# guy3540/Acoustic_Locating_VQ-VAE

Hardware: AMD Instinct MI355X
Metric: spectrograms/sec (train step), speech VQ-VAE default config (higher is better)
Workload: dtype x3mx_hb

## Files before the change

acoustic_locating_vq-vae_amd/csrc/alvq_common.h:

```cpp
#pragma once
#include <hip/hip_runtime.h>
#include <stdint.h>
#include <stdio.h>

#include "../../include/alvq.h"

namespace alvq {

void set_error(const char* fmt, ...);

enum Option { OPT_WIDE_MIN_TILES, OPT_FX_ROWS, OPT_FX_NARROW, OPT_CONV_V2, OPT_CONV_K3, OPT_WGRAD_V3, OPT_VQ_REG, OPT_COUNT };
long option(int id);

inline int check_launch(const char* what) {
  hipError_t e = hipGetLastError();
  if (e != hipSuccess) {
    set_error("%s: %s", what, hipGetErrorString(e));
    return (int)e;
  }
  return ALVQ_OK;
}

#define ALVQ_REQUIRE(cond, code, ...)  \
  do {                                 \
    if (!(cond)) {                     \
      alvq::set_error(__VA_ARGS__);    \
      return (code);                   \
    }                                  \
  } while (0)

struct DeviceOnce {
  bool done[64] = {};
  bool need() {
    int d = 0;
    if (hipGetDevice(&d) != hipSuccess || d < 0 || d >= 64) return true;
    if (done[d]) return false;
    done[d] = true;
    return true;
  }
};

constexpr int kWave = 64;
constexpr int kNumXcd = 8;

__device__ __forceinline__ int xcd_remap(int id, int n) {
  const int q = n / kNumXcd, r = n % kNumXcd;
  const int xcd = id % kNumXcd, local = id / kNumXcd;
  const int base = xcd < r ? xcd * (q + 1) : r * (q + 1) + (xcd - r) * q;
  return base + local;
}

typedef float f32x4 __attribute__((ext_vector_type(4)));
typedef float f32x16 __attribute__((ext_vector_type(16)));
typedef short bf16x8 __attribute__((ext_vector_type(8)));
typedef short bf16x4 __attribute__((ext_vector_type(4)));

int* fx_range_flag_ptr();
int* fx_range_sticky_ptr();

__device__ __forceinline__ float wave_sum(float v) {
#pragma unroll
  for (int o = 32; o > 0; o >>= 1) v += __shfl_xor(v, o, 64);
  return v;
}
// ... 9 lines not shown
```

acoustic_locating_vq-vae_amd/csrc/api.hip:

```cpp
#include <stdarg.h>
#include <stdlib.h>
#include <string.h>

#include <atomic>

#include "alvq_common.h"

namespace alvq {
static thread_local char g_err[512] = "";
void set_error(const char* fmt, ...) {
  va_list ap;
  va_start(ap, fmt);
  vsnprintf(g_err, sizeof(g_err), fmt, ap);
  va_end(ap);
}

struct OptionSpec { const char* name; const char* env; long def; };
static const OptionSpec kSpecs[OPT_COUNT] = {
    {"wide_min_tiles", "ALVQ_WIDE_MIN_TILES", 192},
    {"fx_rows", "ALVQ_FX_ROWS", 0},
    {"fx_narrow", "ALVQ_FX_NARROW", 1},
    {"conv_v2", "ALVQ_CONV_V2", 1},
    {"conv_k3", "ALVQ_CONV_K3", 1},
    {"wgrad_v3", "ALVQ_WGRAD_V3", 3},
    {"vq_reg", "ALVQ_VQ_REG", 1},
};
static std::atomic<long> g_opt[OPT_COUNT];
static std::atomic<int> g_opt_ready{0};
static void options_init() {
  if (g_opt_ready.load(std::memory_order_acquire)) return;
  for (int i = 0; i < OPT_COUNT; ++i) {
    const char* e = getenv(kSpecs[i].env);
    g_opt[i].store(e ? atol(e) : kSpecs[i].def, std::memory_order_relaxed);
  }
  g_opt_ready.store(1, std::memory_order_release);
}
long option(int id) {
  options_init();
  return g_opt[id].load(std::memory_order_relaxed);
}
}

extern "C" const char* alvq_version(void) { return "alvq 0.4.0 (gfx950)"; }
extern "C" const char* alvq_last_error(void) { return alvq::g_err; }

extern "C" int alvq_set_option(const char* name, int64_t value) {
  ALVQ_REQUIRE(name, ALVQ_EINVAL, "alvq_set_option: null name");
  alvq::options_init();
  for (int i = 0; i < alvq::OPT_COUNT; ++i)
    if (!strcmp(name, alvq::kSpecs[i].name)) {
      alvq::g_opt[i].store((long)value, std::memory_order_relaxed);
      return ALVQ_OK;
    }
  alvq::set_error("alvq_set_option: unknown option '%s'", name);
  return ALVQ_EINVAL;
}

extern "C" int64_t alvq_get_option(const char* name) {
  if (name) {
    alvq::options_init();
    for (int i = 0; i < alvq::OPT_COUNT; ++i)
      if (!strcmp(name, alvq::kSpecs[i].name)) return alvq::g_opt[i].load(std::memory_order_relaxed);
  }
  alvq::set_error("alvq_get_option: unknown option '%s'", name ? name : "(null)");
  return INT64_MIN;
}
```

acoustic_locating_vq-vae_amd/csrc/bf16_common.h:

```cpp
#pragma once
#include "alvq_common.h"

namespace alvq {

typedef __bf16 bf16;
typedef __bf16 bf16x8_t __attribute__((ext_vector_type(8)));
typedef unsigned short u16;
typedef unsigned short u16x8 __attribute__((ext_vector_type(8)));

constexpr int TB_R = 128;
constexpr int TB_M = 128;
constexpr int TB_K = 64;
constexpr int XROWS = TB_R + 8;
constexpr int XBYTES = XROWS * 128;
constexpr int WBYTES = TB_M * 128;
constexpr int CS = TB_M + 4;
constexpr int LDS_BYTES = 2 * XBYTES + 2 * WBYTES;
static_assert(LDS_BYTES >= TB_R * CS * 4, "C tile must fit");
constexpr int GUARD_ROWS = 8;

__device__ __forceinline__ float bf2f(u16 v) { return __uint_as_float(((unsigned)v) << 16); }
__device__ __forceinline__ u16 f2bf(float f) {
  unsigned u = __float_as_uint(f);
  if ((u & 0x7fffffffu) > 0x7f800000u) return (u16)((u >> 16) | 0x40);
  return (u16)((u + 0x7fffu + ((u >> 16) & 1u)) >> 16);
}

__device__ __forceinline__ void glds16(const void* gsrc, void* lds_dst) {
  __builtin_amdgcn_global_load_lds((const void __attribute__((address_space(1)))*)gsrc,
                                   (void __attribute__((address_space(3)))*)lds_dst, 16, 0, 0);
}

__device__ __forceinline__ bool row_valid(int row, int Lp1, int nrows_data, int* b, int* l) {
  const int v = row - 1;
  const int bb = v / Lp1, ll = v - bb * Lp1;
  *b = bb;
  *l = ll;
  return row >= 1 && v < nrows_data && ll < Lp1 - 1;
}

struct ConvBArgs {
  const u16* x;
  const u16* wp;
  const float* bias;
  const u16* skip1;
  const u16* skip2;
  const u16* mask;
  const u16* post;
  u16* y;
  u16* y2;
  float* y_ncl;
  int B, L, Cp, M, Mop, Mp128;
  int relu;
  int rtiles, mtiles;
  const unsigned char* mask_bits;
  unsigned char* bits_out;
  int elem;
  const float* out_scale;
  int* range_flag;
};

constexpr int WP_ROWS = 256;
constexpr int NLC_ROW_PAD = 256;

typedef __bf16 bf16x2_t __attribute__((ext_vector_type(2)));
typedef float f32x2 __attribute__((ext_vector_type(2)));
typedef unsigned u32x2 __attribute__((ext_vector_type(2)));
typedef unsigned u32x4 __attribute__((ext_vector_type(4)));

__device__ __forceinline__ unsigned f2bf_pk(float lo, float hi) {
  const f32x2 f = {lo, hi};
  return __builtin_bit_cast(unsigned, __builtin_convertvector(f, bf16x2_t));
}

typedef _Float16 h16x8_t __attribute__((ext_vector_type(8)));
typedef _Float16 h16x2_t __attribute__((ext_vector_type(2)));
template <int F16>
__device__ __forceinline__ float elem2f(u16 v) {
  if (F16) return (float)__builtin_bit_cast(_Float16, v);
  return bf2f(v);
}
template <int F16>
__device__ __forceinline__ unsigned elem_pk(float lo, float hi) {
  if (F16) {
    const f32x2 f = {lo, hi};
    return __builtin_bit_cast(unsigned, __builtin_convertvector(f, h16x2_t));
  }
  return f2bf_pk(lo, hi);
}
template <int F16>
__device__ __forceinline__ void elem_saturate() {
  if (F16) __builtin_amdgcn_s_setreg(1 | (23 << 6), 1);
}
template <int F16>
__device__ __forceinline__ f32x4 elem_mfma16(const bf16x8_t& a, const bf16x8_t& b, const f32x4& c) {
  if (F16) return __builtin_amdgcn_mfma_f32_16x16x32_f16(__builtin_bit_cast(h16x8_t, a), __builtin_bit_cast(h16x8_t, b), c, 0, 0, 0);
  return __builtin_amdgcn_mfma_f32_16x16x32_bf16(a, b, c, 0, 0, 0);
}

__device__ __forceinline__ void fp16_watch(unsigned& run, unsigned word) {
  const unsigned a = word & 0x7fff7fffu;
  asm("v_pk_max_u16 %0, %1, %2" : "=v"(run) : "v"(run), "v"(a));
}
__device__ __forceinline__ bool fp16_limit_reached(unsigned run) { return (run & 0xffffu) >= 0x7bffu || (run >> 16) >= 0x7bffu; }
__device__ __forceinline__ void fp16_report(unsigned run, int* flag) {
  if (flag && __any(fp16_limit_reached(run)) && (threadIdx.x & 63) == 0) atomicOr(flag, 4);
}

int conv1d_bf16_v2_launch(const ConvBArgs& a, int KW, hipStream_t stream);
int conv1d_bf16_k3_launch(const ConvBArgs& a, hipStream_t stream);
int64_t conv1d_wgrad_bf16_v2_workspace_bytes(int total_rows, int C, int M, int KW);
int conv1d_wgrad_bf16_v2_splits(int total_rows, int C, int M, int KW, int nseg, bool with_bias);
// ... 8 lines not shown
```

acoustic_locating_vq-vae_amd/csrc/conv1d_bf16.hip:

```cpp
#include <stdlib.h>

#include "alvq_common.h"
#include "bf16_common.h"
#include "conv1d_bf16_tile256.h"
#include "nlc_host.h"

namespace alvq {

template <int KW, int OUT, int F16 = 0>
__global__ __launch_bounds__(256, 2) void conv1d_bf16_kernel(ConvBArgs a) {
  constexpr int PAD = (KW - 1) / 2;
  extern __shared__ __attribute__((aligned(16))) unsigned char lds[];
  unsigned char* const Xb = lds;
  unsigned char* const Wb = lds + 2 * XBYTES;

  const int tid = threadIdx.x, lane = tid & 63;
  const int wave = __builtin_amdgcn_readfirstlane(tid >> 6);
  const int li = lane & 15, kq = lane >> 4;
  const int wm0 = (wave >> 1) * 64, wn0 = (wave & 1) * 64;

  const int tile = xcd_remap(blockIdx.x, a.mtiles * a.rtiles);
  const int m0 = (tile % a.mtiles) * TB_M;
  const int r0 = (tile / a.mtiles) * TB_R;
  const int Cp = a.Cp;
// ... 174 lines not shown
}

extern "C" int alvq_pack_weight_bf16(const float* w, void* wp, int M, int C, int KW, int w_layout, void* stream) {
  const alvq_pack_desc d{w, wp, M, C, KW, w_layout};
  return alvq_pack_weights_bf16_batch(&d, 1, 1, stream);
}

template <int F16>
static int ncl_to_nlc_16bit(const char* who, const float* x, void* y, int B, int C, int L, const float* scale, void* stream) {
  if (int rc = check_nlc_dims(who, x && y, B, C, L)) return rc;
  const NlcDims d(B, C, L);
  hipLaunchKernelGGL(ncl_to_nlc_kernel<F16>, d.grid32(), dim3(256), 0, (hipStream_t)stream, x, (u16*)y, B, C, L, d.Cp, d.rows, scale);
  return check_launch(who);
}
template <int F16>
static int nlc_to_ncl_16bit(const char* who, const void* x, float* y, int B, int C, int L, const float* scale, void* stream) {
  if (int rc = check_nlc_dims(who, x && y, B, C, L)) return rc;
  const NlcDims d(B, C, L);
  hipLaunchKernelGGL(nlc_to_ncl_kernel<F16>, d.grid32(), dim3(256), 0, (hipStream_t)stream, (const u16*)x, y, B, C, L, d.Cp, d.rows,
                     scale);
  return check_launch(who);
}

extern "C" int alvq_ncl_to_nlc_bf16(const float* x, void* y, int B, int C, int L, void* stream) {
  return ncl_to_nlc_16bit<0>("alvq_ncl_to_nlc_bf16", x, y, B, C, L, nullptr, stream);
}

extern "C" int alvq_nlc_to_ncl_f32(const void* x, float* y, int B, int C, int L, void* stream) {
  return nlc_to_ncl_16bit<0>("alvq_nlc_to_ncl_f32", x, y, B, C, L, nullptr, stream);
}

extern "C" int alvq_relu_mask_bf16(const void* dy, const void* t, void* out, int64_t n, void* stream) {
  ALVQ_REQUIRE(dy && t && out, ALVQ_EINVAL, "alvq_relu_mask_bf16: null pointer");
  ALVQ_REQUIRE(n > 0 && n % 8 == 0, ALVQ_EINVAL, "alvq_relu_mask_bf16: n must be a positive multiple of 8");
  long g = (n / 8 + 1023) / 1024;
  if (g > 2048) g = 2048;
  hipLaunchKernelGGL(relu_mask_bf16_kernel, dim3((int)g), dim3(256), 0, (hipStream_t)stream, (const u16*)dy, (const u16*)t,
                     (u16*)out, (long)(n / 8));
  return check_launch("alvq_relu_mask_bf16");
}

static constexpr int b16_slot(int KW, int OUT, int F16) { return ((KW == 3) * 2 + OUT) * 2 + F16; }
typedef KernelTable<void (*)(ConvBArgs), 8> B16Table;
static B16Table b16_table() {
  B16Table t;
  for_values<1, 3>([&](auto kw) { for_values<0, 1>([&](auto out) { for_values<0, 1>([&](auto f16) {
    t.put(b16_slot(kw, out, f16), conv1d_bf16_kernel<kw, out, f16>, LDS_BYTES);
  }); }); });
  return t;
}

static int conv1d_16bit(int elem, const float* out_scale, const void* x, const void* wp, const float* bias, const void* skip1,
                        const void* skip2, const void* mask, const void* post, void* y, void* y2, float* y_ncl, int B, int C, int M,
                        int L, int KW, int relu, const void* mask_bits, void* relu_bits_out, void* stream) {
  const char* const who = elem ? "alvq_conv1d_f16" : "alvq_conv1d_bf16";
  if (int rc = check_conv_args(who, x, wp, skip1, skip2, mask, post, y, y2, y_ncl, B, C, M, L, KW, relu, mask_bits, relu_bits_out))
    return rc;
  ConvBArgs a{(const u16*)x, (const u16*)wp, bias, (const u16*)skip1, (const u16*)skip2, (const u16*)mask, (const u16*)post,
              (u16*)y, (u16*)y2, y_ncl, B, L, pad_to(C, TB_K), M, pad_to(M, TB_K), pad_to(M, WP_ROWS), relu,
              (int)(alvq_nlc_rows(B, L) / TB_R), pad_to(M, TB_M) / TB_M, (const unsigned char*)mask_bits,
              (unsigned char*)relu_bits_out};
  hipStream_t s = (hipStream_t)stream;
  a.relu = relu ? 1 : 0;
  a.elem = elem;
  a.out_scale = out_scale;
  a.range_flag = elem ? fx_range_flag_ptr() : nullptr;
  const long use_v2 = option(OPT_CONV_V2), use_k3 = option(OPT_CONV_K3);
  const long tiles256 = (alvq_nlc_rows(B, L) / 256) * (pad_to(M, 256) / 256);
  const long min_tiles = option(OPT_WIDE_MIN_TILES);
  if (use_v2 && pad_to(M, 256) - M <= 32 && tiles256 >= min_tiles)
    return (KW == 3 && use_k3) ? conv1d_bf16_k3_launch(a, s) : conv1d_bf16_v2_launch(a, KW, s);
  static const B16Table table = b16_table();
  static DeviceOnce attr;
  if (attr.need()) table.raise_lds_limit();
  return table.launch(b16_slot(KW, y ? 0 : 1, elem ? 1 : 0), dim3(a.rtiles * a.mtiles), dim3(256), s, who, a);
}

extern "C" int alvq_conv1d_bf16(const void* x, const void* wp, const float* bias, const void* skip1, const void* skip2,
                                const void* mask, const void* post, void* y, void* y2, float* y_ncl, int B, int C, int M,
                                int L, int KW, int relu, const void* mask_bits, void* relu_bits_out, void* stream) {
  return conv1d_16bit(0, nullptr, x, wp, bias, skip1, skip2, mask, post, y, y2, y_ncl, B, C, M, L, KW, relu, mask_bits, relu_bits_out,
                      stream);
}

extern "C" int alvq_conv1d_f16(const void* x, const void* wp, const float* bias, const void* skip1, const void* skip2,
                               const void* mask, const void* post, void* y, void* y2, float* y_ncl, int B, int C, int M, int L,
                               int KW, int relu, const void* mask_bits, void* relu_bits_out, const float* out_scale, void* stream) {
  return conv1d_16bit(1, out_scale, x, wp, bias, skip1, skip2, mask, post, y, y2, y_ncl, B, C, M, L, KW, relu, mask_bits,
                      relu_bits_out, stream);
}

extern "C" int alvq_ncl_to_nlc_f16(const float* x, void* y, int B, int C, int L, const float* scale, void* stream) {
  return ncl_to_nlc_16bit<1>("alvq_ncl_to_nlc_f16", x, y, B, C, L, scale, stream);
}

extern "C" int alvq_nlc_to_ncl_f16(const void* x, float* y, int B, int C, int L, const float* scale, void* stream) {
  return nlc_to_ncl_16bit<1>("alvq_nlc_to_ncl_f16", x, y, B, C, L, scale, stream);
}

static int64_t wgrad_bias_offset(int rows, int C, int M, int KW) { return conv1d_wgrad_bf16_v2_workspace_bytes(rows, C, M, KW); }

extern "C" int64_t alvq_conv1d_wgrad_bf16_workspace_bytes(int B, int C, int M, int L, int KW) {
  if (!wgrad_shape_ok(B, C, M, L, KW)) return -1;
  return wgrad_bias_offset((int)alvq_nlc_rows(B, L), C, M, KW) + (int64_t)64 * pad_to(M, TB_K) * 4;
}

extern "C" int64_t alvq_conv1d_wgrad_bf16_bias_offset(int B, int C, int M, int L, int KW) {
  if (!wgrad_shape_ok(B, C, M, L, KW)) return -1;
  return wgrad_bias_offset((int)alvq_nlc_rows(B, L), C, M, KW);
}

extern "C" int alvq_conv1d_wgrad_bf16_splits(int B, int C, int M, int L, int KW, int nseg, int with_bias) {
  if (!wgrad_shape_ok(B, C, M, L, KW) || nseg < 1 || nseg > WGRAD_MAXSEG) return -1;
  return conv1d_wgrad_bf16_v2_splits((int)alvq_nlc_rows(B, L), C, M, KW, nseg, with_bias != 0);
}

static int wgrad_16bit(const char* who, int elem, const void* const* dy, const void* const* x, int nseg, bool multi, float* dw,
                       float* dbias, void* workspace, int B, int C, int M, int L, int KW, int w_layout, int accumulate,
                       const float* inv_scale, void* stream) {
  if (int rc = check_wgrad_args(who, dy, x, nseg, multi, dw, workspace, B, C, M, L, KW, w_layout, accumulate, true)) return rc;
  const int rows = (int)alvq_nlc_rows(B, L);
  float* const bias_partial = multi ? nullptr : (float*)((char*)workspace + wgrad_bias_offset(rows, C, M, KW));
  return conv1d_wgrad_bf16_v2_launch(dy, x, nseg, dw, workspace, rows, C, M, KW, w_layout, accumulate, (hipStream_t)stream, dbias,
                                     bias_partial, elem, inv_scale);
}

extern "C" int alvq_conv1d_wgrad_bf16(const void* dy, const void* x, float* dw, float* dbias, void* workspace, int B, int C,
                                      int M, int L, int KW, int w_layout, int accumulate, void* stream) {
  return wgrad_16bit("alvq_conv1d_wgrad_bf16", 0, &dy, &x, 1, false, dw, dbias, workspace, B, C, M, L, KW, w_layout, accumulate,
                     nullptr, stream);
}

extern "C" int alvq_conv1d_wgrad_f16(const void* dy, const void* x, float* dw, float* dbias, void* workspace, int B, int C, int M,
                                     int L, int KW, int w_layout, int accumulate, const float* inv_scale, void* stream) {
  return wgrad_16bit("alvq_conv1d_wgrad_f16", 1, &dy, &x, 1, false, dw, dbias, workspace, B, C, M, L, KW, w_layout, accumulate,
                     inv_scale, stream);
}

extern "C" int alvq_conv1d_wgrad_f16_multi(const void* const* dy, const void* const* x, int nseg, float* dw, void* workspace, int B,
                                           int C, int M, int L, int KW, int w_layout, int accumulate, const float* inv_scale,
                                           void* stream) {
  return wgrad_16bit("alvq_conv1d_wgrad_f16_multi", 1, dy, x, nseg, true, dw, nullptr, workspace, B, C, M, L, KW, w_layout,
// ... 9 lines not shown
```

acoustic_locating_vq-vae_amd/csrc/conv1d_bf16_tile256.h:

```cpp
#pragma once
#include "bf16_common.h"

namespace alvq {

constexpr int V2_M = 256, V2_R = 256, V2_K = 32;
constexpr int V2_HALF = V2_M * V2_K * 2;
constexpr int V2_CS = V2_M + 4;
constexpr int V2_EPI_LDS = 64 * V2_CS * 4;

struct FragSet {
  bf16x8_t a[8];
  bf16x8_t b[4];
};

template <int NMI, int NNI, int F16 = 0>
__device__ __forceinline__ void wave_epilogue_bf16(const ConvBArgs& a, const f32x4 (&acc)[NMI][NNI], int m0, int r0, int li,
                                                   int kq, int wm0, int wn0);

template <int OUT, int F16 = 0>
__device__ __forceinline__ void tile256_epilogue(const ConvBArgs& a, const f32x4 (&acc)[8][4], unsigned char* lds, int m0,
                                                 int r0, int wave, int tid, int li, int kq, int wm0) {
  if (OUT == 0) {
    wave_epilogue_bf16<8, 4, F16>(a, acc, m0, r0, li, kq, wm0, (wave & 3) * 64);
    return;
// ... 57 lines not shown
      float v[8];
#pragma unroll
      for (int e = 0; e < 4; ++e) {
        const u32x2 r = __builtin_amdgcn_permlane16_swap(__float_as_uint(acc[mp][ni][e]), __float_as_uint(acc[mp + 1][ni][e]),
                                                         false, false);
        v[e] = __uint_as_float(r[0]);
        v[e + 4] = __uint_as_float(r[1]);
      }
      if (a.bias) {
        if (m0 + wm0 + mp * 16 + 32 <= a.M) {
          const f32x4 b0 = *(const f32x4*)(a.bias + mb), b1 = *(const f32x4*)(a.bias + mb + 4);
#pragma unroll
          for (int e = 0; e < 4; ++e) {
            v[e] += b0[e];
            v[4 + e] += b1[e];
          }
        } else {
#pragma unroll
          for (int e = 0; e < 8; ++e) v[e] += (mb + e < a.M) ? a.bias[mb + e] : 0.f;
        }
      }
      if (a.skip1) {
#pragma unroll
        for (int e = 0; e < 8; ++e) v[e] += elem2f<F16>(s1[mp / 2][e]);
      }
      if (a.skip2) {
#pragma unroll
        for (int e = 0; e < 8; ++e) v[e] += elem2f<F16>(s2[mp / 2][e]);
      }
      if (a.relu & 1) {
#pragma unroll
        for (int e = 0; e < 8; ++e) v[e] = fmaxf(v[e], 0.f);
      }
      if (a.mask_bits) {
        const int bt = (int)a.mask_bits[o >> 3];
#pragma unroll
        for (int e = 0; e < 8; ++e) v[e] = __uint_as_float(__float_as_uint(v[e]) & (unsigned)((bt << (31 - e)) >> 31));
      } else if (a.mask) {
#pragma unroll
        for (int e = 0; e < 8; ++e) v[e] = (short)mk[mp / 2][e] > 0 ? v[e] : 0.f;
      }
      u32x4 out;
#pragma unroll
      for (int e = 0; e < 4; ++e) out[e] = elem_pk<F16>(v[2 * e], v[2 * e + 1]);
      if (gaps) {
#pragma unroll
        for (int e = 0; e < 4; ++e) out[e] = ok ? out[e] : 0u;
      }
      *(u32x4*)(a.y + o) = out;
      if (F16) {
#pragma unroll
        for (int e = 0; e < 4; ++e) fp16_watch(watch, out[e]);
      }
      if (a.y2) {
        const u16x8 ps = *(const u16x8*)(a.post + o);
        u32x4 out2;
#pragma unroll
        for (int e = 0; e < 4; ++e) out2[e] = elem_pk<F16>(v[2 * e] + elem2f<F16>(ps[2 * e]), v[2 * e + 1] + elem2f<F16>(ps[2 * e + 1]));
        if (gaps) {
#pragma unroll
          for (int e = 0; e < 4; ++e) out2[e] = ok ? out2[e] : 0u;
        }
        *(u32x4*)(a.y2 + o) = out2;
      }
      if (a.bits_out) {
        unsigned bt = 0;
#pragma unroll
        for (int e = 7; e >= 0; --e) {
          const int half = (int)((e & 1) ? (out[e >> 1] & 0xffff0000u) : (out[e >> 1] << 16));
          const int t = half > 0 ? half : 0;
          bt = __builtin_amdgcn_alignbit(bt, 0u - (unsigned)t, 31);
        }
        a.bits_out[o >> 3] = (unsigned char)bt;
      }
    }
  }
  if (F16) fp16_report(watch, a.range_flag);
}

}
```

acoustic_locating_vq-vae_amd/csrc/conv1d_wgrad_bf16_v2.hip:

```cpp
#include <stdlib.h>

#include "alvq_common.h"
#include "bf16_common.h"
#include "nlc_host.h"
#include "wgrad_reduce.h"

namespace alvq {

typedef short s16x4_t __attribute__((ext_vector_type(4)));
typedef short s16x8_t __attribute__((ext_vector_type(8)));

constexpr int WG_MAXSEG = 4;
struct WgradV2Args {
  const u16* dy[WG_MAXSEG];
  const u16* x[WG_MAXSEG];
  float* partial;
  float* bias_partial;
  int Mp, Cp, M, C;
  int mtiles, ctiles, splits, chunks_per_split, total_rows, nseg;
};

typedef unsigned long long u64;
template <int ROW_BYTES>
__device__ __forceinline__ void tr_pair_issue(unsigned lds_addr, u64& lo, u64& hi) {
// ... 397 lines not shown
#undef V3_TILE
#undef V3_TILE_K3
#undef V3_TILE_K1
#undef V3_SB
#undef V3_MM
#undef V3_RD_B
#undef V3_RD_A
#undef V3_TR16

  const int jc = lane & 31;
  float* out = a.partial + (long)split * KW * a.M * a.C;
#pragma unroll
  for (int t = 0; t < KW; ++t)
#pragma unroll
    for (int mi = 0; mi < MF; ++mi)
#pragma unroll
      for (int cf = 0; cf < NC; ++cf)
#pragma unroll
        for (int q = 0; q < 16; ++q) {
          const int m = m0 + wm0 + mi * 32 + (q & 3) + 8 * (q >> 2) + 4 * g;
          const int c = c0 + wc0 + cf * 32 + jc;
          if (m < a.M && c < a.C) out[((long)t * a.M + m) * a.C + c] = acc[t][mi][cf][q];
        }
}

template <int KW, int NC, int MF>
static constexpr int wgrad_v3_lds() {
  return 4 * (32 * (2 * MF * 32 * 2) + (KW == 1 ? 32 : 36) * (4 * NC * 32 * 2));
}

static __global__ __launch_bounds__(256) void wgrad_bias_reduce_kernel(const float* bp, float* dbias, int splits, int Mp, int M,
                                                                       int accumulate, const float* scale) {
  const int m = blockIdx.x * 256 + threadIdx.x;
  if (m >= M) return;
  float s = 0.f;
  for (int k = 0; k < splits; ++k) s += bp[(long)k * Mp + m];
  if (scale) s *= *scale;
  dbias[m] = accumulate ? dbias[m] + s : s;
}

template <int KW, int NCF>
static constexpr int wgrad_v2_lds() {
  return 4 * (32 * 256 + (KW == 1 ? 32 : 36) * (4 * NCF * 16 * 2));
}

static int wgrad_v3_select() { return (int)option(OPT_WGRAD_V3); }
static bool wgrad_uses_v3(int KW, bool with_bias) {
  return !with_bias && ((KW == 1 && (wgrad_v3_select() & 1)) || (KW == 3 && (wgrad_v3_select() & 2)));
}
static int wgrad_v2_tiles(int C, int M, int KW, bool v3) {
  return WgradTile{(v3 && KW == 1) ? 256 : 128, KW == 3 ? 128 : 256}.count(C, M);
}

static constexpr int wg_slot(int v3, int KW, int F16) { return (v3 * 2 + (KW == 3)) * 2 + F16; }
typedef KernelTable<void (*)(WgradV2Args), 8> WgTable;
static WgTable wg_table() {
  WgTable t;
  for_values<1, 3>([&](auto kw) { for_values<0, 1>([&](auto f16) {
    constexpr int NCF = kw == 3 ? 2 : 4, NC = kw == 3 ? 1 : 2, MF = kw == 3 ? 2 : 4;
    t.put(wg_slot(0, kw, f16), conv1d_wgrad_bf16_v2_kernel<kw, NCF, f16>, wgrad_v2_lds<kw, NCF>());
    t.put(wg_slot(1, kw, f16), conv1d_wgrad_bf16_v3_kernel<kw, NC, MF, f16>, wgrad_v3_lds<kw, NC, MF>());
  }); });
  return t;
}

int conv1d_wgrad_bf16_v2_splits(int total_rows, int C, int M, int KW, int nseg, bool with_bias) {
  int cps;
  return wgrad_split_plan(nseg * total_rows, wgrad_v2_tiles(C, M, KW, wgrad_uses_v3(KW, with_bias)), &cps);
}

int64_t conv1d_wgrad_bf16_v2_workspace_bytes(int total_rows, int C, int M, int KW) {
  const int s2 = wgrad_split_bound(total_rows, wgrad_v2_tiles(C, M, KW, false), WG_MAXSEG);
  const int s3 = wgrad_split_bound(total_rows, wgrad_v2_tiles(C, M, KW, true), WG_MAXSEG);
  return (int64_t)(s2 > s3 ? s2 : s3) * KW * M * C * 4;
}

int conv1d_wgrad_bf16_v2_launch(const void* const* dy, const void* const* x, int nseg, float* dw, void* workspace,
                                int total_rows, int C, int M, int KW, int w_layout, int accumulate, hipStream_t s,
                                float* dbias, float* bias_partial, int elem, const float* out_scale) {
  const int ct = KW == 3 ? 128 : 256;
  const int Mp = pad_to(M, 64), Cp = pad_to(C, 64);
  WgradV2Args a{};
  for (int i = 0; i < WG_MAXSEG; ++i) {
    a.dy[i] = (const u16*)dy[i < nseg ? i : 0];
    a.x[i] = (const u16*)x[i < nseg ? i : 0];
  }
  a.partial = (float*)workspace;
  a.bias_partial = dbias ? bias_partial : nullptr;
  a.Mp = Mp; a.Cp = Cp; a.M = M; a.C = C;
  a.mtiles = (M + 127) / 128; a.ctiles = (C + ct - 1) / ct;
  a.total_rows = total_rows; a.nseg = nseg;
  const bool v3 = wgrad_uses_v3(KW, dbias != nullptr);
  if (v3 && KW == 1) a.mtiles = (M + 255) / 256;
  a.splits = wgrad_split_plan(nseg * total_rows, a.mtiles * a.ctiles, &a.chunks_per_split);
  ALVQ_REQUIRE(a.mtiles * a.ctiles == wgrad_v2_tiles(C, M, KW, v3) &&
                   (int64_t)a.splits * KW * M * C * 4 <= conv1d_wgrad_bf16_v2_workspace_bytes(total_rows, C, M, KW),
               ALVQ_EINVAL, "alvq_conv1d_wgrad_bf16: %d splits exceed what alvq_conv1d_wgrad_bf16_workspace_bytes sizes", a.splits);
  static const WgTable table = wg_table();
  static DeviceOnce attr;
  if (attr.need()) table.raise_lds_limit();
  if (int rc = table.launch(wg_slot(v3, KW, elem ? 1 : 0), dim3(a.mtiles * a.ctiles * a.splits), dim3(512), s, "alvq_conv1d_wgrad_bf16(v2)", a))
    return rc;
  if (accumulate == ALVQ_WGRAD_DEFER) return ALVQ_OK;
  wgrad_reduce_launch((const float*)workspace, dw, a.splits, KW, M, C, w_layout, accumulate, s, out_scale);
  if (dbias)
    hipLaunchKernelGGL(wgrad_bias_reduce_kernel, dim3((M + 255) / 256), dim3(256), 0, s, (const float*)bias_partial, dbias,
                       a.splits, Mp, M, accumulate, out_scale);
  return check_launch("alvq_conv1d_wgrad_bf16(v2)/reduce");
}

}
```

acoustic_locating_vq-vae_amd/csrc/nlc_host.h:

```cpp
#pragma once
#include <type_traits>

#include "bf16_common.h"

namespace alvq {

inline int pad_to(int x, int q) { return (x + q - 1) / q * q; }
inline long nlc_plane_elems(int B, int L, int C) {
  return ((long)alvq_nlc_rows(B, L) + 2L * alvq_nlc_guard_rows()) * pad_to(C, TB_K);
}
struct NlcDims {
  int rows, Cp;
  long plane;
  NlcDims(int B, int C, int L) : rows((int)alvq_nlc_rows(B, L)), Cp(pad_to(C, TB_K)), plane(nlc_plane_elems(B, L, C)) {}
  dim3 grid32() const { return dim3((rows / 32) * (Cp / 32)); }
};

inline int check_nlc_dims(const char* who, bool pointers, int B, int C, int L) {
  ALVQ_REQUIRE(pointers, ALVQ_EINVAL, "%s: null pointer", who);
  ALVQ_REQUIRE(B > 0 && C > 0 && L > 0, ALVQ_EINVAL, "%s: bad dims", who);
  return ALVQ_OK;
}

inline int check_conv_args(const char* who, const void* x, const void* wp, const void* skip1, const void* skip2, const void* mask,
                           const void* post, const void* y, const void* y2, const void* y_ncl, int B, int C, int M, int L, int KW,
                           int relu, const void* mask_bits, const void* bits_out, const char* ncl_also = "") {
  ALVQ_REQUIRE(x && wp && (y || y_ncl), ALVQ_EINVAL, "%s: null x/wp/y", who);
  ALVQ_REQUIRE(!(y && y_ncl), ALVQ_EINVAL, "%s: choose one of y (NLC) and y_ncl (NCL fp32)", who);
  ALVQ_REQUIRE(B > 0 && C > 0 && M > 0 && L > 0, ALVQ_EINVAL, "%s: bad dims", who);
  ALVQ_REQUIRE(KW == 1 || KW == 3, ALVQ_EUNSUPPORTED, "%s: KW=%d (only 1 and 3)", who, KW);
  ALVQ_REQUIRE((y2 == nullptr) == (post == nullptr), ALVQ_EINVAL, "%s: y2 and post go together", who);
  ALVQ_REQUIRE(!y_ncl || (!skip1 && !skip2 && !mask && !post && !relu), ALVQ_EUNSUPPORTED,
               "%s: the NCL fp32 epilogue fuses bias%s only", who, ncl_also);
  ALVQ_REQUIRE((long)B * (L + 1) < (1L << 30), ALVQ_EUNSUPPORTED, "%s: problem too large", who);
  ALVQ_REQUIRE(!(mask && mask_bits), ALVQ_EINVAL, "%s: pass the mask as a tensor or as bits, not both", who);
  ALVQ_REQUIRE(!y_ncl || (!mask_bits && !bits_out), ALVQ_EUNSUPPORTED, "%s: sign bits go with the NLC output", who);
  return ALVQ_OK;
}

constexpr int WGRAD_MAXSEG = 4;

inline int check_wgrad_args(const char* who, const void* const* dy, const void* const* x, int nseg, bool multi, const void* dw,
                            const void* workspace, int B, int C, int M, int L, int KW, int w_layout, int accumulate,
                            bool dw_may_be_null) {
  ALVQ_REQUIRE(dy && x && (multi || (dy[0] && x[0])) && (dw || (dw_may_be_null && accumulate == ALVQ_WGRAD_DEFER)) && workspace,
               ALVQ_EINVAL, "%s: null pointer", who);
  if (multi) {
    ALVQ_REQUIRE(nseg >= 1 && nseg <= WGRAD_MAXSEG, ALVQ_EUNSUPPORTED, "%s: nseg=%d (1..4)", who, nseg);
    for (int i = 0; i < nseg; ++i) ALVQ_REQUIRE(dy[i] && x[i], ALVQ_EINVAL, "%s: null segment %d", who, i);
  }
  ALVQ_REQUIRE(B > 0 && C > 0 && M > 0 && L > 0, ALVQ_EINVAL, "%s: bad dims", who);
  ALVQ_REQUIRE(KW == 1 || KW == 3, ALVQ_EUNSUPPORTED, "%s: KW=%d (only 1 and 3)", who, KW);
  ALVQ_REQUIRE(w_layout == ALVQ_W_OIK || w_layout == ALVQ_W_IOK, ALVQ_EINVAL, "%s: w_layout", who);
  return ALVQ_OK;
}

template <int... V, class F>
inline void for_values(F f) {
  (f(std::integral_constant<int, V>{}), ...);
}

template <class Fn, int N>
struct KernelTable {
  Fn fn[N] = {};
  int lds[N] = {};
  void put(int slot, Fn f, int lds_bytes) {
    fn[slot] = f;
    lds[slot] = lds_bytes;
  }
  void raise_lds_limit() const {
    for (int i = 0; i < N; ++i)
      if (fn[i]) (void)hipFuncSetAttribute((const void*)fn[i], hipFuncAttributeMaxDynamicSharedMemorySize, lds[i]);
  }
  template <class... A>
  int launch(int slot, dim3 grid, dim3 block, hipStream_t s, const char* what, const A&... args) const {
    ALVQ_REQUIRE(slot >= 0 && slot < N && fn[slot], ALVQ_EUNSUPPORTED, "%s: no kernel is instantiated for this case (slot %d)", what,
                 slot);
    hipLaunchKernelGGL(fn[slot], grid, block, lds[slot], s, args...);
    return check_launch(what);
  }
};

inline int wgrad_split_plan(int total_rows, int tiles, int* chunks_per_split) {
  const int nchunks = total_rows / 64;
  int want = (256 + tiles - 1) / tiles;
  if (want < 1) want = 1;
  if (want > nchunks) want = nchunks;
  if (want > 64) want = 64;
  const int cps = (nchunks + want - 1) / want;
// ... 56 lines not shown
```

acoustic_locating_vq-vae_amd/csrc/pack_weights.hip:

```cpp
#include "alvq_common.h"
#include "bf16_common.h"
#include "f16mx_common.h"
#include "nlc_host.h"

namespace alvq {

constexpr int PB_MAX = 32;
struct PackDesc {
  const float* w;
  u16* wp;
  int M, C, KW, layout, Mp, Cp, blk0, ctiles;
};
struct PackBatch {
  PackDesc d[PB_MAX];
  int n;
  long plane[PB_MAX];
};

template <int PLANES>
__device__ __forceinline__ void pack_store8(u16* wp, long plane, long row_off, int c, const float (&v)[8]) {
  const long o = row_off + c;
  if (PLANES == 3) {
    unsigned h[4], qh[2], ql[2];
    fx_split<8>(v, fx_pow2(FX_E_W), fx_pow2(FX_E_W - FX_LO_SHIFT), h, qh, ql);
// ... 12 lines not shown
#pragma unroll
    for (int e = 0; e < 4; ++e) {
      const float h0 = __uint_as_float(hi[e] << 16), h1 = __uint_as_float(hi[e] & 0xffff0000u);
      lo[e] = f2bf_pk(v[2 * e] - h0, v[2 * e + 1] - h1);
    }
    *(u32x4*)(wp + plane + o) = lo;
  }
}

template <int PLANES>
__global__ __launch_bounds__(256) void pack_weights_batch_kernel(PackBatch b) {
  __shared__ float tile[3][32][65];
  if (PLANES == 3) fx_saturating_conversions();
  int di = 0;
  for (int i = 1; i < b.n; ++i)
    if ((int)blockIdx.x >= b.d[i].blk0) di = i;
  const PackDesc& d = b.d[di];
  const int lb = blockIdx.x - d.blk0;
  const int m0 = (lb / d.ctiles) * 32, c0 = (lb % d.ctiles) * 64;
  const int KW = d.KW, tid = threadIdx.x;
  if (d.layout == ALVQ_W_OIK) {
    const int run = 64 * KW;
#pragma unroll 4
    for (int e = tid; e < 32 * run; e += 256) {
      const int mr = e / run, j = e - mr * run, c = j / KW, t = j - c * KW;
      const int m = m0 + mr;
      tile[t][mr][c] = (m < d.M && c0 + c < d.C) ? d.w[((long)m * d.C + c0) * KW + j] : 0.f;
    }
  } else {
    const int run = 32 * KW;
#pragma unroll 4
    for (int e = tid; e < 64 * run; e += 256) {
      const int cc = e / run, j = e - cc * run, mr = j / KW, k = j - mr * KW;
      const int c = c0 + cc;
      tile[KW - 1 - k][mr][cc] = (c < d.C && m0 + mr < d.M) ? d.w[((long)c * d.M + m0) * KW + j] : 0.f;
    }
  }
  __syncthreads();
  const int mr = tid >> 3, cg = (tid & 7) * 8;
  for (int t = 0; t < KW; ++t) {
    float v[8];
#pragma unroll
    for (int e = 0; e < 8; ++e) v[e] = tile[t][mr][cg + e];
    pack_store8<PLANES>(d.wp, b.plane[di], ((long)t * d.Mp + m0 + mr) * d.Cp, c0 + cg, v);
  }
}

constexpr int AP_MAX = 24;
struct AdamPackDesc {
  float* w; const float* g; float* m; float* v;
  u16* oik; u16* iok;
  int dim0, dim1, KW, blk0, tiles1;
  int oik_Mp, oik_Cp, iok_Mp, iok_Cp;
};
struct AdamPackBatch {
  AdamPackDesc d[AP_MAX];
  int n;
  const float* sc;
  const float* skip;
  float beta1, beta2, eps;
};

template <int PLANES>
__global__ __launch_bounds__(256) void adam_pack_batch_kernel(AdamPackBatch b) {
  __shared__ float tile[3][32][65];
  if (b.skip && *b.skip != 0.f) return;
  if (PLANES == 3) fx_saturating_conversions();
  int di = 0;
  for (int i = 1; i < b.n; ++i)
    if ((int)blockIdx.x >= b.d[i].blk0) di = i;
  const AdamPackDesc& d = b.d[di];
  const int lb = blockIdx.x - d.blk0;
  const int r0 = (lb / d.tiles1) * 32, q0 = (lb % d.tiles1) * 64;
  const int KW = d.KW, tid = threadIdx.x;
  const float lr_bc1 = b.sc[0], bc2_sqrt = b.sc[1], gscale = b.sc[2];
  const float beta1 = b.beta1, beta2 = b.beta2, eps = b.eps;
  const int run = 64 * KW;
  if (q0 + 64 <= d.dim1 && ((d.dim1 * KW) & 3) == 0) {
#pragma unroll 2
    for (int e4 = tid; e4 < 8 * run; e4 += 256) {
      const int e = 4 * e4, rr = e / run, j = e - rr * run;
      f32x4 wn = {0.f, 0.f, 0.f, 0.f};
      if (r0 + rr < d.dim0) {
        const long i = ((long)(r0 + rr) * d.dim1 + q0) * KW + j;
        const f32x4 g4 = *(const f32x4*)(d.g + i), m4 = *(const f32x4*)(d.m + i), v4 = *(const f32x4*)(d.v + i), w4 = *(const f32x4*)(d.w + i);
        f32x4 mo, vo;
#pragma unroll
        for (int q = 0; q < 4; ++q) {
          const float gr = g4[q] * gscale;
          const float mm = m4[q] + (gr - m4[q]) * (1.f - beta1);
          const float vv = v4[q] * beta2 + (1.f - beta2) * gr * gr;
          const float denom = sqrtf(vv) / bc2_sqrt + eps;
          mo[q] = mm;
          vo[q] = vv;
          wn[q] = w4[q] - lr_bc1 * (mm / denom);
        }
        *(f32x4*)(d.m + i) = mo;
        *(f32x4*)(d.v + i) = vo;
        *(f32x4*)(d.w + i) = wn;
      }
#pragma unroll
      for (int q = 0; q < 4; ++q) {
        const int jj = j + q, qq = jj / KW, t = jj - qq * KW;
        tile[t][rr][qq] = wn[q];
      }
    }
  } else {
#pragma unroll 2
    for (int e = tid; e < 32 * run; e += 256) {
      const int rr = e / run, j = e - rr * run, qq = j / KW, t = j - qq * KW;
      float wn = 0.f;
      if (r0 + rr < d.dim0 && q0 + qq < d.dim1) {
        const long i = ((long)(r0 + rr) * d.dim1 + q0) * KW + j;
        const float gr = d.g[i] * gscale;
        const float m0 = d.m[i], v0 = d.v[i];
        const float mm = m0 + (gr - m0) * (1.f - beta1);
        const float vv = v0 * beta2 + (1.f - beta2) * gr * gr;
        const float denom = sqrtf(vv) / bc2_sqrt + eps;
        d.m[i] = mm;
        d.v[i] = vv;
        wn = d.w[i] - lr_bc1 * (mm / denom);
        d.w[i] = wn;
      }
      tile[t][rr][qq] = wn;
    }
  }
  __syncthreads();
  if (d.oik) {
    const int mr = tid >> 3, cg = (tid & 7) * 8;
    const long plane = (long)KW * d.oik_Mp * d.oik_Cp;
    for (int t = 0; t < KW; ++t) {
// ... 47 lines not shown

using namespace alvq;

extern "C" int alvq_pack_weights_bf16_batch(const alvq_pack_desc* descs, int n, int planes, void* stream) {
  ALVQ_REQUIRE(descs && n > 0, ALVQ_EINVAL, "alvq_pack_weights_bf16_batch: no descriptors");
  ALVQ_REQUIRE(planes >= 1 && planes <= 3, ALVQ_EINVAL, "alvq_pack_weights_bf16_batch: planes=%d (1, 2 or 3)", planes);
  for (int i = 0; i < n; ++i) {
    const alvq_pack_desc& s = descs[i];
    ALVQ_REQUIRE(s.w && s.wp, ALVQ_EINVAL, "alvq_pack_weights_bf16_batch: null pointer in descriptor %d", i);
    ALVQ_REQUIRE(s.M > 0 && s.C > 0 && (s.KW == 1 || s.KW == 3), ALVQ_EINVAL, "alvq_pack_weights_bf16_batch: bad dims in descriptor %d", i);
    ALVQ_REQUIRE(s.w_layout == ALVQ_W_OIK || s.w_layout == ALVQ_W_IOK, ALVQ_EINVAL, "alvq_pack_weights_bf16_batch: w_layout in descriptor %d", i);
  }
  for (int i0 = 0; i0 < n; i0 += PB_MAX) {
    PackBatch b{};
    b.n = n - i0 < PB_MAX ? n - i0 : PB_MAX;
    int blocks = 0;
    for (int i = 0; i < b.n; ++i) {
      const alvq_pack_desc& s = descs[i0 + i];
      PackDesc& d = b.d[i];
      d.w = s.w; d.wp = (u16*)s.wp; d.M = s.M; d.C = s.C; d.KW = s.KW; d.layout = s.w_layout;
      d.Mp = pad_to(s.M, WP_ROWS); d.Cp = pad_to(s.C, TB_K);
      d.blk0 = blocks; d.ctiles = d.Cp / 64;
      b.plane[i] = (long)s.KW * d.Mp * d.Cp;
      blocks += (d.Mp / 32) * d.ctiles;
    }
    if (planes == 1) hipLaunchKernelGGL(pack_weights_batch_kernel<1>, dim3(blocks), dim3(256), 0, (hipStream_t)stream, b);
    else if (planes == 2) hipLaunchKernelGGL(pack_weights_batch_kernel<2>, dim3(blocks), dim3(256), 0, (hipStream_t)stream, b);
    else hipLaunchKernelGGL(pack_weights_batch_kernel<3>, dim3(blocks), dim3(256), 0, (hipStream_t)stream, b);
    int rc = check_launch("alvq_pack_weights_bf16_batch");
    if (rc) return rc;
  }
  return ALVQ_OK;
}

extern "C" int alvq_adam_pack_batch(const alvq_adam_pack_desc* descs, int n, int planes, const float* scalars, float beta1,
                                    float beta2, float eps, const float* skip, void* stream) {
  ALVQ_REQUIRE(descs && n > 0 && scalars, ALVQ_EINVAL, "alvq_adam_pack_batch: no descriptors / scalars");
  ALVQ_REQUIRE(planes >= 1 && planes <= 3, ALVQ_EINVAL, "alvq_adam_pack_batch: planes=%d (1, 2 or 3)", planes);
  for (int i = 0; i < n; ++i) {
    const alvq_adam_pack_desc& s = descs[i];
    ALVQ_REQUIRE(s.w && s.g && s.m && s.v, ALVQ_EINVAL, "alvq_adam_pack_batch: null pointer in descriptor %d", i);
    ALVQ_REQUIRE(s.dim0 > 0 && s.dim1 > 0 && (s.KW == 1 || s.KW == 3), ALVQ_EINVAL, "alvq_adam_pack_batch: bad dims in descriptor %d", i);
  }
  for (int i0 = 0; i0 < n; i0 += AP_MAX) {
    AdamPackBatch b{};
    b.n = n - i0 < AP_MAX ? n - i0 : AP_MAX;
    b.sc = scalars; b.skip = skip; b.beta1 = beta1; b.beta2 = beta2; b.eps = eps;
    int blocks = 0;
    for (int i = 0; i < b.n; ++i) {
      const alvq_adam_pack_desc& s = descs[i0 + i];
      AdamPackDesc& d = b.d[i];
      d.w = s.w; d.g = s.g; d.m = s.m; d.v = s.v; d.oik = (u16*)s.wp_oik; d.iok = (u16*)s.wp_iok;
      d.dim0 = s.dim0; d.dim1 = s.dim1; d.KW = s.KW;
      d.oik_Mp = pad_to(s.dim0, WP_ROWS); d.oik_Cp = pad_to(s.dim1, TB_K);
      d.iok_Mp = pad_to(s.dim1, WP_ROWS); d.iok_Cp = pad_to(s.dim0, TB_K);
      d.blk0 = blocks; d.tiles1 = (s.dim1 + 63) / 64;
      blocks += ((s.dim0 + 31) / 32) * d.tiles1;
    }
    if (planes == 1) hipLaunchKernelGGL(adam_pack_batch_kernel<1>, dim3(blocks), dim3(256), 0, (hipStream_t)stream, b);
    else if (planes == 2) hipLaunchKernelGGL(adam_pack_batch_kernel<2>, dim3(blocks), dim3(256), 0, (hipStream_t)stream, b);
    else hipLaunchKernelGGL(adam_pack_batch_kernel<3>, dim3(blocks), dim3(256), 0, (hipStream_t)stream, b);
    int rc = check_launch("alvq_adam_pack_batch");
    if (rc) return rc;
  }
  return ALVQ_OK;
}

extern "C" int alvq_adam_segments_f32(float* param, const float* grad, float* exp_avg, float* exp_avg_sq, const int64_t* lo,
                                      const int64_t* hi, int nseg, const float* scalars, float beta1, float beta2, float eps,
                                      const float* skip, void* stream) {
  ALVQ_REQUIRE(param && grad && exp_avg && exp_avg_sq && scalars && lo && hi, ALVQ_EINVAL, "alvq_adam_segments_f32: null pointer");
  ALVQ_REQUIRE(nseg > 0, ALVQ_EINVAL, "alvq_adam_segments_f32: no segments");
  for (int i0 = 0; i0 < nseg; i0 += AS_MAX) {
    AdamSegs s{};
    s.n = nseg - i0 < AS_MAX ? nseg - i0 : AS_MAX;
    int blocks = 0;
    for (int i = 0; i < s.n; ++i) {
      ALVQ_REQUIRE(lo[i0 + i] >= 0 && hi[i0 + i] > lo[i0 + i], ALVQ_EINVAL, "alvq_adam_segments_f32: bad segment %d", i0 + i);
      s.lo[i] = lo[i0 + i]; s.hi[i] = hi[i0 + i];
      s.blk0[i] = blocks;
      blocks += (int)((hi[i0 + i] - lo[i0 + i] + 1023) / 1024);
    }
    hipLaunchKernelGGL(adam_segments_kernel, dim3(blocks), dim3(256), 0, (hipStream_t)stream, param, grad, exp_avg, exp_avg_sq, s, scalars,
                       beta1, beta2, eps, skip);
    int rc = check_launch("alvq_adam_segments_f32");
    if (rc) return rc;
  }
  return ALVQ_OK;
}
```

acoustic_locating_vq-vae_amd/csrc/wgrad_reduce.h:

```cpp
#pragma once
#include "alvq_common.h"

namespace alvq {

static __device__ __forceinline__ void wgrad_reduce_body(const float* partial, float* dw, int splits, int KW, int M, int C,
                                                         int w_layout, int accumulate, const float* scale, long stride, int bid,
                                                         int nblk) {
  const long total = (long)KW * M * C;
  const float sc = scale ? *scale : 1.f;
  if (w_layout == ALVQ_W_OIK && KW == 3) {
    const long pairs = (long)M * C;
    for (long q = bid * 256L + threadIdx.x; q < pairs; q += (long)nblk * 256) {
      float s0 = 0.f, s1 = 0.f, s2 = 0.f;
      const float* p = partial + q;
      int k = 0;
      for (; k + 2 <= splits; k += 2) {
        const float* pa = p + (long)k * stride;
        const float* pb = pa + stride;
        const float a0 = pa[0], a1 = pa[pairs], a2 = pa[2 * pairs], b0 = pb[0], b1 = pb[pairs], b2 = pb[2 * pairs];
        s0 = (s0 + a0) + b0;
        s1 = (s1 + a1) + b1;
        s2 = (s2 + a2) + b2;
      }
      for (; k < splits; ++k) {
        const float* pa = p + (long)k * stride;
        s0 += pa[0];
        s1 += pa[pairs];
        s2 += pa[2 * pairs];
      }
      if (scale) { s0 *= sc; s1 *= sc; s2 *= sc; }
      float* o = dw + 3 * q;
      if (accumulate) { s0 += o[0]; s1 += o[1]; s2 += o[2]; }
      o[0] = s0; o[1] = s1; o[2] = s2;
    }
    return;
  }
  for (long e = bid * 256L + threadIdx.x; e < total; e += (long)nblk * 256) {
    int m, c, t;
    if (w_layout == ALVQ_W_OIK) {
      t = (int)(e % KW);
      c = (int)((e / KW) % C);
      m = (int)(e / ((long)KW * C));
    } else {
      const int tt = (int)(e % KW);
      t = KW - 1 - tt;
      m = (int)((e / KW) % M);
      c = (int)(e / ((long)KW * M));
    }
    const long src = ((long)t * M + m) * C + c;
    float s = 0.f;
    int k = 0;
    for (; k + 4 <= splits; k += 4) {
      const float v0 = partial[(long)k * stride + src], v1 = partial[(long)(k + 1) * stride + src],
                  v2 = partial[(long)(k + 2) * stride + src], v3 = partial[(long)(k + 3) * stride + src];
      s = (((s + v0) + v1) + v2) + v3;
    }
    for (; k < splits; ++k) s += partial[(long)k * stride + src];
    if (scale) s *= sc;
    dw[e] = accumulate ? dw[e] + s : s;
  }
}
static __global__ void wgrad_reduce_kernel(const float* partial, float* dw, int splits, int KW, int M, int C, int w_layout,
                                    int accumulate, const float* scale) {
  wgrad_reduce_body(partial, dw, splits, KW, M, C, w_layout, accumulate, scale, (long)KW * M * C, blockIdx.x, gridDim.x);
}

template <int RB>
static __device__ __forceinline__ void wgrad_reduce_iok_body(float (&tile)[3][RB][65], const float* partial, float* dw, int splits,
                                                             int KW, int M, int C, int accumulate, const float* scale, int bid) {
  constexpr int RI = RB / 8;
  const int ctiles = (C + 63) / 64;
  const int m0 = (bid / ctiles) * RB, c0 = (bid % ctiles) * 64;
  const int tx = threadIdx.x & 31, ty = threadIdx.x >> 5;
  const long plane = (long)M * C, total = (long)KW * plane;
  const bool pair = (C % 2 == 0);
  float s0[3][RI], s1[3][RI];
#pragma unroll
  for (int t = 0; t < 3; ++t)
#pragma unroll
    for (int i = 0; i < RI; ++i) s0[t][i] = s1[t][i] = 0.f;
  const int c = c0 + 2 * tx;
  const bool full = pair && m0 + RB <= M && c0 + 64 <= C;
  if (full) {
    const float* p0 = partial + (long)(m0 + ty) * C + c;
    if (KW == 3) {
#pragma unroll 4
      for (int k = 0; k < splits; ++k) {
        float2 v[3][RI];
#pragma unroll
        for (int t = 0; t < 3; ++t)
#pragma unroll
          for (int i = 0; i < RI; ++i) v[t][i] = *(const float2*)(p0 + (long)k * total + (long)t * plane + (long)(8 * i) * C);
#pragma unroll
        for (int t = 0; t < 3; ++t)
#pragma unroll
          for (int i = 0; i < RI; ++i) {
            s0[t][i] += v[t][i].x;
            s1[t][i] += v[t][i].y;
          }
      }
    } else {
#pragma unroll 4
      for (int k = 0; k < splits; ++k) {
        float2 v[RI];
#pragma unroll
        for (int i = 0; i < RI; ++i) v[i] = *(const float2*)(p0 + (long)k * total + (long)(8 * i) * C);
#pragma unroll
        for (int i = 0; i < RI; ++i) {
          s0[0][i] += v[i].x;
          s1[0][i] += v[i].y;
        }
      }
    }
  } else
  for (int k = 0; k < splits; ++k) {
    const float* pk = partial + (long)k * total + c;
#pragma unroll
    for (int t = 0; t < 3; ++t) {
      if (t >= KW) break;
#pragma unroll
      for (int i = 0; i < RI; ++i) {
        const int m = m0 + ty + 8 * i;
        if (m >= M) continue;
        const float* p = pk + (long)t * plane + (long)m * C;
        if (pair && c + 1 < C) {
          const float2 v = *(const float2*)p;
          s0[t][i] += v.x;
          s1[t][i] += v.y;
        } else {
          if (c < C) s0[t][i] += p[0];
          if (c + 1 < C) s1[t][i] += p[1];
        }
      }
    }
  }
#pragma unroll
  for (int t = 0; t < 3; ++t) {
    if (t >= KW) break;
#pragma unroll
    for (int i = 0; i < RI; ++i) {
      tile[t][ty + 8 * i][2 * tx] = s0[t][i];
      tile[t][ty + 8 * i][2 * tx + 1] = s1[t][i];
    }
  }
  __syncthreads();
  const int run = RB * KW;
  for (int e = threadIdx.x; e < 64 * run; e += 256) {
    const int cc = e / run, j = e - cc * run, mr = j / KW, tt = j - mr * KW;
    if (c0 + cc >= C || m0 + mr >= M) continue;
    const long o = ((long)(c0 + cc) * M + m0) * KW + j;
    float v = tile[KW - 1 - tt][mr][cc];
    if (scale) v *= *scale;
    dw[o] = accumulate ? dw[o] + v : v;
  }
}
template <int RB>
static __global__ __launch_bounds__(256) void wgrad_reduce_iok_kernel(const float* partial, float* dw, int splits, int KW,
                                                                      int M, int C, int accumulate, const float* scale) {
  __shared__ float tile[3][RB][65];
  wgrad_reduce_iok_body<RB>(tile, partial, dw, splits, KW, M, C, accumulate, scale, blockIdx.x);
}

static inline void wgrad_reduce_launch(const float* partial, float* dw, int splits, int KW, int M, int C, int w_layout,
                                       int accumulate, hipStream_t s, const float* scale = nullptr) {
  if (w_layout == ALVQ_W_IOK) {
    const int grid = ((M + 15) / 16) * ((C + 63) / 64);
    hipLaunchKernelGGL(wgrad_reduce_iok_kernel<16>, dim3(grid), dim3(256), 0, s, partial, dw, splits, KW, M, C, accumulate, scale);
    return;
  }
  const long total = (long)KW * M * C;
  int rgrid = (int)((total + 255) / 256);
  if (rgrid > 2048) rgrid = 2048;
  hipLaunchKernelGGL(wgrad_reduce_kernel, dim3(rgrid), dim3(256), 0, s, partial, dw, splits, KW, M, C, w_layout, accumulate, scale);
}

}
```

acoustic_locating_vq-vae_amd/csrc/wgrad_reduce_batch.hip:

```cpp
#include "alvq_common.h"
#include "wgrad_reduce.h"

namespace alvq {

constexpr int RB_MAX = 40;
struct ReduceBatch {
  alvq_reduce_desc d[RB_MAX];
  int blk0[RB_MAX];
  int nblk[RB_MAX];
  int n;
};

__global__ __launch_bounds__(256) void wgrad_reduce_batch_kernel(ReduceBatch b) {
  __shared__ float tile[3][16][65];
  int di = 0;
  for (int i = 1; i < b.n; ++i)
    if ((int)blockIdx.x >= b.blk0[i]) di = i;
  const alvq_reduce_desc& d = b.d[di];
  const int lb = blockIdx.x - b.blk0[di];
  const int acc = d.accumulate;
  if (d.w_layout == ALVQ_W_IOK && d.stride == (int64_t)d.KW * d.M * d.C)
    wgrad_reduce_iok_body<16>(tile, d.partial, d.dst, d.splits, d.KW, d.M, d.C, acc, d.scale, lb);
  else
    wgrad_reduce_body(d.partial, d.dst, d.splits, d.KW, d.M, d.C, d.w_layout, acc, d.scale, (long)d.stride, lb, b.nblk[di]);
}

}

using namespace alvq;

extern "C" int alvq_wgrad_reduce_batch(const alvq_reduce_desc* descs, int n, void* stream) {
  ALVQ_REQUIRE(descs && n > 0, ALVQ_EINVAL, "alvq_wgrad_reduce_batch: no descriptors");
  for (int i = 0; i < n; ++i) {
    const alvq_reduce_desc& s = descs[i];
    ALVQ_REQUIRE(s.partial && s.dst, ALVQ_EINVAL, "alvq_wgrad_reduce_batch: null pointer in descriptor %d", i);
    ALVQ_REQUIRE(s.splits >= 1 && s.splits <= 64 && s.M > 0 && s.C > 0 && (s.KW == 1 || s.KW == 3), ALVQ_EINVAL,
                 "alvq_wgrad_reduce_batch: bad dims in descriptor %d", i);
    ALVQ_REQUIRE(s.w_layout == ALVQ_W_OIK || s.w_layout == ALVQ_W_IOK, ALVQ_EINVAL, "alvq_wgrad_reduce_batch: w_layout in descriptor %d", i);
    ALVQ_REQUIRE(s.stride >= (int64_t)s.KW * s.M * s.C, ALVQ_EINVAL, "alvq_wgrad_reduce_batch: stride in descriptor %d", i);
  }
  for (int i0 = 0; i0 < n; i0 += RB_MAX) {
    ReduceBatch b{};
    b.n = n - i0 < RB_MAX ? n - i0 : RB_MAX;
    int blocks = 0;
    for (int i = 0; i < b.n; ++i) {
      const alvq_reduce_desc& s = descs[i0 + i];
      b.d[i] = s;
      const long total = (long)s.KW * s.M * s.C;
      int nb;
      if (s.w_layout == ALVQ_W_IOK && s.stride == total) nb = ((s.M + 15) / 16) * ((s.C + 63) / 64);
      else {
        nb = (int)((total + 255) / 256);
        if (nb > 2048) nb = 2048;
      }
      b.blk0[i] = blocks;
      b.nblk[i] = nb;
      blocks += nb;
    }
    hipLaunchKernelGGL(wgrad_reduce_batch_kernel, dim3(blocks), dim3(256), 0, (hipStream_t)stream, b);
    int rc = check_launch("alvq_wgrad_reduce_batch");
    if (rc) return rc;
  }
  return ALVQ_OK;
}
```

acoustic_locating_vq-vae_amd/src/acoustic_locating_vq_vae/_native.py:

```python
from __future__ import annotations

import collections
import ctypes
import functools
import os

import torch

_LIB = None
_HERE = os.path.dirname(os.path.abspath(__file__))
_DEFAULT_LIB = os.path.normpath(os.path.join(_HERE, "..", "..", "lib", "libalvq.so"))

W_OIK = 0
W_IOK = 1
VQ_PARTIALS = 1024
EW_PARTIALS = 1024

_c_void_p = ctypes.c_void_p
_i32 = ctypes.c_int
_i64 = ctypes.c_int64
_f32 = ctypes.c_float

_SIGNATURES = {
    "alvq_version": (ctypes.c_char_p, []),
    "alvq_last_error": (ctypes.c_char_p, []),
    "alvq_set_option": (_i32, [ctypes.c_char_p, _i64]),
    "alvq_get_option": (_i64, [ctypes.c_char_p]),
    "alvq_conv1d_f32": (_i32, [_c_void_p] * 9 + [_i32] * 7 + [_c_void_p]),
    "alvq_conv1d_wgrad_workspace_bytes": (_i64, [_i32] * 5),
    "alvq_conv1d_wgrad_f32": (_i32, [_c_void_p] * 5 + [_i32] * 7 + [_c_void_p]),
    "alvq_vq_argmin_workspace_bytes": (_i64, [_i64, _i32, _i32]),
    "alvq_vq_argmin_f32": (_i32, [_c_void_p] * 5 + [_i64, _i32, _i32, _c_void_p]),
    "alvq_vq_gather_loss_f32": (_i32, [_c_void_p] * 6 + [_i64, _i32, _i32, _c_void_p]),
    "alvq_vq_finalize_f32": (_i32, [_c_void_p] * 3 + [_i64, _i32, _i32, _f32, _c_void_p]),
    "alvq_vq_finalize_ema_f32": (_i32, [_c_void_p] * 3 + [_i64, _i32, _i32, _f32, _c_void_p]),
    "alvq_vq_backward_workspace_bytes": (_i64, [_i32, _i32]),
    "alvq_vq_backward_f32": (_i32, [_c_void_p] * 8 + [_i64, _i32, _i32, _f32, _c_void_p]),
    "alvq_onehot_f32": (_i32, [_c_void_p, _c_void_p, _i64, _i32, _c_void_p]),
    "alvq_jitter_gather_f32": (_i32, [_c_void_p] * 3 + [_i64, _i32, _i32, _c_void_p]),
    "alvq_standardise_f32": (_i32, [_c_void_p, _c_void_p, _i32, _i32, _i32, _i32, _c_void_p]),
    "alvq_mse_f32": (_i32, [_c_void_p] * 4 + [_i64, _c_void_p]),
    "alvq_mse_backward_f32": (_i32, [_c_void_p] * 4 + [_i64, _c_void_p]),
    "alvq_fill_f32": (_i32, [_c_void_p, _f32, _i64, _c_void_p]),
    "alvq_add_f32": (_i32, [_c_void_p] * 3 + [_i64, _c_void_p]),
    "alvq_relu_mask_f32": (_i32, [_c_void_p] * 3 + [_i64, _c_void_p]),
    "alvq_row_mean_f32": (_i32, [_c_void_p] * 2 + [_i64, _i32, _c_void_p]),
    "alvq_row_mean_backward_f32": (_i32, [_c_void_p] * 2 + [_i64, _i32, _c_void_p]),
    "alvq_transpose_f32": (_i32, [_c_void_p, _c_void_p, _i32, _i32, _i32, _c_void_p]),
    "alvq_adam_f32": (_i32, [_c_void_p] * 4 + [_i64, _i32, _f32, _f32, _f32, _f32, _f32, _c_void_p]),
    "alvq_adam_dev_f32": (_i32, [_c_void_p] * 4 + [_i64, _c_void_p, _f32, _f32, _f32, _c_void_p, _c_void_p]),
    "alvq_adam_advance_f32": (_i32, [_c_void_p, ctypes.c_double, ctypes.c_double, ctypes.c_double, ctypes.c_double, _c_void_p, _c_void_p]),
    "alvq_range_flag_to_slot": (_i32, [_c_void_p, _c_void_p]),
    "alvq_stft_power_f32": (_i32, [_c_void_p, _c_void_p, _i32, _i32, _i32, _i32, _c_void_p]),
    "alvq_stft_power_f64": (_i32, [_c_void_p, _c_void_p, _i32, _i32, _i32, _i32, _c_void_p]),
    "alvq_stft_complex_f32": (_i32, [_c_void_p, _c_void_p, _i32, _i32, _i32, _i32, _c_void_p]),
    "alvq_stft_complex_f64": (_i32, [_c_void_p, _c_void_p, _i32, _i32, _i32, _i32, _c_void_p]),
    "alvq_fir_same_f64": (_i32, [_c_void_p, _c_void_p, _c_void_p, _i32, _i32, _i32, _i32, _c_void_p]),
    "alvq_spec_rir_wiener_f64": (_i32, [_c_void_p] * 7 + [_i32, _i32, _i32, _c_void_p]),
    "alvq_rows_to_nlc": (_i32, [_c_void_p, _c_void_p, _i32, _i32, _i32, _i32, _i32, _i32, _c_void_p]),
    "alvq_rows_to_nlc_max_std_rows": (_i32, []),
    "alvq_nlc_rows": (_i64, [_i32, _i32]),
    "alvq_nlc_channels": (_i32, [_i32]),
    "alvq_nlc_guard_rows": (_i32, []),
    "alvq_packed_weight_elems": (_i64, [_i32, _i32, _i32]),
    "alvq_pack_weight_bf16": (_i32, [_c_void_p, _c_void_p, _i32, _i32, _i32, _i32, _c_void_p]),
    "alvq_pack_weights_bf16_batch": (_i32, [_c_void_p, _i32, _i32, _c_void_p]),
    "alvq_adam_pack_batch": (_i32, [_c_void_p, _i32, _i32, _c_void_p, _f32, _f32, _f32, _c_void_p, _c_void_p]),
    "alvq_adam_segments_f32": (_i32, [_c_void_p] * 4 + [_c_void_p, _c_void_p, _i32, _c_void_p, _f32, _f32, _f32, _c_void_p, _c_void_p]),
    "alvq_ncl_to_nlc_bf16": (_i32, [_c_void_p, _c_void_p, _i32, _i32, _i32, _c_void_p]),
    "alvq_nlc_to_ncl_f32": (_i32, [_c_void_p, _c_void_p, _i32, _i32, _i32, _c_void_p]),
    "alvq_relu_mask_bf16": (_i32, [_c_void_p] * 3 + [_i64, _c_void_p]),
    "alvq_conv1d_bf16": (_i32, [_c_void_p] * 10 + [_i32] * 6 + [_c_void_p] * 3),
    "alvq_conv1d_wgrad_bf16_workspace_bytes": (_i64, [_i32] * 5),
    "alvq_conv1d_wgrad_bf16": (_i32, [_c_void_p] * 5 + [_i32] * 7 + [_c_void_p]),
    "alvq_conv1d_wgrad_bf16_multi": (_i32, [_c_void_p, _c_void_p, _i32, _c_void_p, _c_void_p] + [_i32] * 7 + [_c_void_p]),
    "alvq_nlc_plane_bytes": (_i64, [_i32, _i32, _i32]),
    "alvq_pack_weight_bf16x3": (_i32, [_c_void_p, _c_void_p, _i32, _i32, _i32, _i32, _c_void_p]),
    "alvq_ncl_to_nlc_bf16x3": (_i32, [_c_void_p, _c_void_p, _i32, _i32, _i32, _c_void_p]),
    "alvq_nlc_to_ncl_bf16x3": (_i32, [_c_void_p, _c_void_p, _i32, _i32, _i32, _c_void_p]),
    "alvq_relu_mask_bf16x3": (_i32, [_c_void_p] * 3 + [_i32, _i32, _i32, _c_void_p]),
    "alvq_conv1d_bf16x3": (_i32, [_c_void_p] * 10 + [_i32] * 6 + [_c_void_p]),
    "alvq_conv1d_wgrad_bf16x3_workspace_bytes": (_i64, [_i32] * 5),
    "alvq_conv1d_wgrad_bf16x3": (_i32, [_c_void_p] * 5 + [_i32] * 7 + [_c_void_p]),
    "alvq_grad_scale_f32": (_i32, [_c_void_p, _i64, _c_void_p, _c_void_p]),
    "alvq_f16mx_range_flag": (_i32, [_c_void_p, _i32, _c_void_p]),
    "alvq_ncl_to_nlc_f16mx": (_i32, [_c_void_p, _c_void_p, _i32, _i32, _i32, _c_void_p, _c_void_p]),
    "alvq_nlc_to_ncl_f16mx": (_i32, [_c_void_p, _c_void_p, _i32, _i32, _i32, _c_void_p, _c_void_p]),
    "alvq_relu_mask_f16mx": (_i32, [_c_void_p] * 3 + [_i32, _i32, _i32, _c_void_p]),
    "alvq_conv1d_f16mx": (_i32, [_c_void_p] * 10 + [_i32] * 6 + [_c_void_p] * 4),
    "alvq_conv1d_wgrad_f16mx_workspace_bytes": (_i64, [_i32] * 5),
    "alvq_conv1d_wgrad_f16mx": (_i32, [_c_void_p] * 5 + [_i32] * 7 + [_c_void_p, _c_void_p]),
    "alvq_conv1d_wgrad_bf16x3_multi": (_i32, [_c_void_p, _c_void_p, _i32, _c_void_p, _c_void_p] + [_i32] * 7 + [_c_void_p]),
    "alvq_conv1d_wgrad_f16mx_multi": (_i32, [_c_void_p, _c_void_p, _i32, _c_void_p, _c_void_p] + [_i32] * 7 + [_c_void_p, _c_void_p]),
    "alvq_conv1d_wgrad_bf16_splits": (_i32, [_i32] * 7),
    "alvq_conv1d_wgrad_bf16x3_splits": (_i32, [_i32] * 6),
    "alvq_conv1d_wgrad_f16mx_splits": (_i32, [_i32] * 6),
    "alvq_ncl_to_nlc_f16": (_i32, [_c_void_p, _c_void_p, _i32, _i32, _i32, _c_void_p, _c_void_p]),
    "alvq_nlc_to_ncl_f16": (_i32, [_c_void_p, _c_void_p, _i32, _i32, _i32, _c_void_p, _c_void_p]),
    "alvq_conv1d_f16": (_i32, [_c_void_p] * 10 + [_i32] * 6 + [_c_void_p] * 4),
    "alvq_conv1d_wgrad_f16": (_i32, [_c_void_p] * 5 + [_i32] * 7 + [_c_void_p, _c_void_p]),
    "alvq_conv1d_wgrad_f16_multi": (_i32, [_c_void_p, _c_void_p, _i32, _c_void_p, _c_void_p] + [_i32] * 7 + [_c_void_p, _c_void_p]),
    "alvq_conv1d_wgrad_bf16_bias_offset": (_i64, [_i32] * 5),
    "alvq_wgrad_reduce_batch": (_i32, [_c_void_p, _i32, _c_void_p]),
    "alvq_onehot_to_index_f32": (_i32, [_c_void_p] * 3 + [_i64, _i32, _c_void_p]),
    "alvq_indices_to_i32": (_i32, [_c_void_p] * 3 + [_i64, _i32, _c_void_p]),
    "alvq_embedding_bag_fwd_f32": (_i32, [_c_void_p] * 4 + [_i32] * 4 + [_c_void_p] * 2),
    "alvq_embedding_bag_bwd_f32": (_i32, [_c_void_p] * 4 + [_i32] * 5 + [_c_void_p] * 2),
    "alvq_istft_f32": (_i32, [_c_void_p] * 3 + [_i32] * 5 + [_c_void_p]),
    "alvq_istft_f64": (_i32, [_c_void_p] * 3 + [_i32] * 5 + [_c_void_p]),
    "alvq_griffin_lim_workspace_bytes": (_i64, [_i32] * 4),
    "alvq_griffin_lim_f32": (_i32, [_c_void_p] * 4 + [_i32] * 6 + [ctypes.c_double, _c_void_p]),
    "alvq_griffin_lim_f64": (_i32, [_c_void_p] * 4 + [_i32] * 6 + [ctypes.c_double, _c_void_p]),
    "alvq_rir_f64": (_i32, [_c_void_p] * 3 + [_i32] * 2 + [ctypes.c_double] * 3 + [_c_void_p] + [ctypes.c_double] * 2
                     + [_i32] * 2 + [_c_void_p]),
    "alvq_rir_rooms_f64": (_i32, [_c_void_p] * 6 + [_i32] * 2 + [ctypes.c_double] * 2 + [_i32] * 2 + [_c_void_p]),
    "alvq_edc_f32": (_i32, [_c_void_p] * 2 + [_i32] * 2 + [_c_void_p]),
    "alvq_edc_f64": (_i32, [_c_void_p] * 2 + [_i32] * 2 + [_c_void_p]),
    "alvq_room_acoustics_f32": (_i32, [_c_void_p] * 4 + [_i32] * 2 + [ctypes.c_double] + [_i32] * 3 + [_c_void_p]),
    "alvq_room_acoustics_f64": (_i32, [_c_void_p] * 4 + [_i32] * 2 + [ctypes.c_double] + [_i32] * 3 + [_c_void_p]),
    "alvq_tsne_code_sqdist_f32": (_i32, [_c_void_p] * 2 + [_i32] * 2 + [_c_void_p]),
    "alvq_tsne_affinities_workspace_bytes": (_i64, [_i32]),
    "alvq_tsne_affinities_f32": (_i32, [_c_void_p] * 4 + [_i32, ctypes.c_double, _c_void_p]),
    "alvq_tsne_descend_workspace_bytes": (_i64, [_i32]),
    "alvq_tsne_descend_f64": (_i32, [_c_void_p] * 7 + [_i32] * 2 + [ctypes.c_double] * 3 + [_c_void_p]),
    "alvq_kmeans_update_workspace_bytes": (_i64, [_i64, _i32, _i32]),
    "alvq_kmeans_update_f32": (_i32, [_c_void_p] * 9 + [_i64, _i32, _i32, ctypes.c_double, _c_void_p]),
    "alvq_kmeans_inertia_workspace_bytes": (_i64, [_i64]),
    "alvq_kmeans_inertia_f32": (_i32, [_c_void_p] * 5 + [_i64, _i32, _i32, _c_void_p]),
    "alvq_kmeans_col_stats_workspace_bytes": (_i64, [_i64, _i32]),
    "alvq_kmeans_col_stats_f32": (_i32, [_c_void_p] * 4 + [_i64, _i32, _c_void_p]),
    "alvq_kmeans_add_rows_f32": (_i32, [_c_void_p] * 3 + [_i64, _i32, _f32, _c_void_p]),
    "alvq_kmeans_plusplus_workspace_bytes": (_i64, [_i64, _i32]),
    "alvq_kmeans_plusplus_f32": (_i32, [_c_void_p] * 5 + [_i64, _i32, _i32, _i32, _i64, _c_void_p]),
    "alvq_vq_ema_stats_workspace_bytes": (_i64, [_i64, _i32, _i32]),
    "alvq_vq_ema_stats_f32": (_i32, [_c_void_p] * 5 + [_i64, _i32, _i32, _c_void_p]),
    "alvq_vq_ema_update_f32": (_i32, [_c_void_p] * 6 + [_i32, _i32, ctypes.c_double, ctypes.c_double, _c_void_p]),
    "alvq_vq_restart_gather_f32": (_i32, [_c_void_p] * 4 + [_i64, _i32, _i32, _i32, _i32, _c_void_p]),
    "alvq_vq_restart_dead_f32": (_i32, [_c_void_p] * 6 + [_i32, _i32, _i32, _f32, _c_void_p]),
    "alvq_adam_advance_sched_f32": (_i32, [_c_void_p, ctypes.c_double, ctypes.c_double, ctypes.c_double, ctypes.c_double, _c_void_p,
                                           _c_void_p, _i64, _i64, ctypes.c_double]),
    "alvq_grad_clip_workspace_bytes": (_i64, [_i64]),
    "alvq_grad_clip_f32": (_i32, [_c_void_p, _i64, _c_void_p, ctypes.c_double, _c_void_p, _c_void_p, _c_void_p]),
}

EXPORTS = tuple(_SIGNATURES)


def lib_path():
    return os.environ.get("ALVQ_LIB", _DEFAULT_LIB)


def lib():
# ... 117 lines not shown
    _check(rc, "alvq_conv1d_f32")
    return (y, y2) if post is not None else y


_WS = {}
_WS_RETIRED = []


def _workspace(nbytes, device):
    key = (device.type, device.index, torch.cuda.current_stream(device).cuda_stream)
    buf = _WS.get(key)
    if buf is None or buf.numel() < nbytes:
        if buf is not None:
            _WS_RETIRED.append(buf)
        buf = torch.empty(max(nbytes, 1 << 20), device=device, dtype=torch.uint8)
        _WS[key] = buf
    return buf


WGRAD_DEFER = 2
_ARENA = {}


class ReduceDesc(ctypes.Structure):
    _fields_ = [("partial", ctypes.c_void_p), ("dst", ctypes.c_void_p), ("scale", ctypes.c_void_p), ("splits", ctypes.c_int32),
                ("KW", ctypes.c_int32), ("M", ctypes.c_int32), ("C", ctypes.c_int32), ("w_layout", ctypes.c_int32),
                ("accumulate", ctypes.c_int32), ("stride", ctypes.c_int64)]


def arena_reset(device):
    key = (device.type, device.index, torch.cuda.current_stream(device).cuda_stream)
    st = _ARENA.get(key)
    if st is not None:
        st["chunk"], st["off"] = 0, 0


def arena_alloc(nbytes, device):
    key = (device.type, device.index, torch.cuda.current_stream(device).cuda_stream)
    st = _ARENA.setdefault(key, {"chunks": [], "chunk": 0, "off": 0})
    nbytes = (nbytes + 255) // 256 * 256
    while True:
        if st["chunk"] >= len(st["chunks"]):
            st["chunks"].append(torch.empty(max(nbytes, 256 << 20), device=device, dtype=torch.uint8))
            st["off"] = 0
        buf = st["chunks"][st["chunk"]]
        if st["off"] + nbytes <= buf.numel():
            ptr = buf.data_ptr() + st["off"]
            st["off"] += nbytes
            return ptr
        st["chunk"] += 1
        st["off"] = 0


class DeferredReductions(list):

    def __init__(self):
        super().__init__()
        self.keep = []


def wgrad_reduce_batch(descs):
    if not descs:
        return
    arr = (ReduceDesc * len(descs))(*descs)
    _check(lib().alvq_wgrad_reduce_batch(ctypes.addressof(arr), len(descs), _stream()), "alvq_wgrad_reduce_batch")
    if isinstance(descs, DeferredReductions):
        descs.keep.clear()


def _defer_descs(defer, ws_ptr, dw, dbias, scale, nseg, B, C, M, L, KW, w_layout):
    L_ = lib()
    scale_ptr = _sptr(scale, 1)
    dsts = {dw.data_ptr()} | ({dbias.data_ptr()} if dbias is not None else set())
    if any(d.dst in dsts for d in defer):
        wgrad_reduce_batch(defer)
        del defer[:]
    if scale is not None and hasattr(defer, "keep"):
        defer.keep.append(scale)
    splits = L_.alvq_conv1d_wgrad_bf16_splits(B, C, M, L, KW, nseg, int(dbias is not None))
    defer.append(ReduceDesc(ws_ptr, dw.data_ptr(), scale_ptr, splits, KW, M, C, w_layout, 1, KW * M * C))
    if dbias is not None:
        off = L_.alvq_conv1d_wgrad_bf16_bias_offset(B, C, M, L, KW)
        defer.append(ReduceDesc(ws_ptr + off, dbias.data_ptr(), scale_ptr, splits, 1, 1, M, W_OIK, 1, (M + 63) // 64 * 64))


def conv1d_wgrad(dy, x, KW, w_layout=W_OIK, want_bias=False, dw_out=None, dbias_out=None, accumulate=False):
    B, C, L = x.shape
    Bd, M, Ld = dy.shape
    if (Bd, Ld) != (B, L):
        raise RuntimeError("conv1d_wgrad: dy %s does not match x %s" % (tuple(dy.shape), tuple(x.shape)))
    shape = (M, C, KW) if w_layout == W_OIK else (C, M, KW)
    if dw_out is None:
        dw_out = torch.empty(shape, device=x.device, dtype=torch.float32)
        accumulate = False
    elif tuple(dw_out.shape) != shape:
        raise RuntimeError("conv1d_wgrad: dw_out has shape %s, expected %s" % (tuple(dw_out.shape), shape))
    if want_bias and dbias_out is None:
        dbias_out = torch.empty((M,), device=x.device, dtype=torch.float32)
    nbytes = lib().alvq_conv1d_wgrad_workspace_bytes(B, C, M, L, KW)
    if nbytes < 0:
        raise RuntimeError("conv1d_wgrad: unsupported shape")
    ws = _workspace(nbytes, x.device)
    with _timed("conv1d_wgrad_f32_kernel", 2.0 * B * L * M * C * KW):
        rc = lib().alvq_conv1d_wgrad_f32(_ptr(dy, name="dy"), _ptr(x, name="x"), _ptr(dw_out, name="dw"),
                                         _ptr(dbias_out, name="dbias") if want_bias else None, ws.data_ptr(),
                                         B, C, M, L, KW, w_layout, int(bool(accumulate)), _stream())
    _check(rc, "alvq_conv1d_wgrad_f32")
    return (dw_out, dbias_out) if want_bias else dw_out


def vq_argmin(flat, codebook, want_dist=False):
    N, D = flat.shape
    K, Dc = codebook.shape
    if D != Dc:
        raise RuntimeError("vq_argmin: row width %d != codebook dim %d" % (D, Dc))
    idx = torch.empty((N,), device=flat.device, dtype=torch.int64)
    dist = torch.empty((N,), device=flat.device, dtype=torch.float32) if want_dist else None
    ws = _workspace(lib().alvq_vq_argmin_workspace_bytes(N, K, D), flat.device)
    with _timed("vq_argmin_f32_kernel", 2.0 * N * K * D):
        rc = lib().alvq_vq_argmin_f32(_ptr(flat, name="x"), _ptr(codebook, name="codebook"), idx.data_ptr(),
                                      _ptr(dist), ws.data_ptr(), N, K, D, _stream())
    _check(rc, "alvq_vq_argmin_f32")
    return (idx, dist) if want_dist else idx


def vq_gather_loss(flat, codebook, idx, beta, ema=False):
    N, D = flat.shape
    K = codebook.shape[0]
    q_st = torch.empty_like(flat)
    partials = torch.empty((VQ_PARTIALS,), device=flat.device, dtype=torch.float32)
    hist = torch.empty((K,), device=flat.device, dtype=torch.float32)
    fill_(hist, 0.0)
    hist = hist.view(torch.int32)
    out = torch.empty((2,), device=flat.device, dtype=torch.float32)
    L = lib()
    _check(L.alvq_vq_gather_loss_f32(_ptr(flat, name="x"), _ptr(codebook, name="codebook"),
                                     _ptr(idx, torch.int64, "idx"), _ptr(q_st), _ptr(partials),
                                     _ptr(hist, torch.int32), N, K, D, _stream()), "alvq_vq_gather_loss_f32")
    fin = "alvq_vq_finalize_ema_f32" if ema else "alvq_vq_finalize_f32"
    _check(getattr(L, fin)(_ptr(partials), _ptr(hist, torch.int32), _ptr(out), N, K, D, float(beta), _stream()), fin)
    return q_st, out


def vq_ema_stats(flat, idx, counts, sums):
    N, D = flat.shape
    K = counts.numel()
    if idx.shape != (N,) or sums.shape != (K, D):
        raise RuntimeError("vq_ema_stats: idx must be (%d,) and sums (%d, %d)" % (N, K, D))
    nbytes = lib().alvq_vq_ema_stats_workspace_bytes(N, K, D)
    if nbytes < 0:
        raise RuntimeError("vq_ema_stats: N=%d, K=%d, D=%d out of range (N < 2^24, K <= 16384, D <= 512)" % (N, K, D))
    ws = _workspace(nbytes, flat.device)
    _check(lib().alvq_vq_ema_stats_f32(_ptr(flat, name="x"), _ptr(idx, torch.int64, "idx"), _ptr(counts, name="counts"),
                                       _ptr(sums, name="sums"), ws.data_ptr(), N, K, D, _stream()), "alvq_vq_ema_stats_f32")


def vq_ema_update(counts, sums, cluster_size, ema_w, codebook, decay, epsilon, skip=None):
    K, D = codebook.shape
    if counts.numel() != K or cluster_size.numel() != K or sums.shape != (K, D) or ema_w.shape != (K, D):
        raise RuntimeError("vq_ema_update: counts / cluster_size must be (%d,) and sums / ema_w (%d, %d)" % (K, K, D))
    _check(lib().alvq_vq_ema_update_f32(_ptr(counts, name="counts"), _ptr(sums, name="sums"),
                                        _ptr(cluster_size, name="cluster_size"), _ptr(ema_w, name="ema_w"),
                                        _ptr(codebook, name="codebook"), _ptr(skip, name="skip"), K, D, float(decay),
                                        float(epsilon), _stream()), "alvq_vq_ema_update_f32")


def vq_restart_gather(flat, rows, cand, status, first=0, stride=1):
    N, D = flat.shape
    R = cand.shape[0]
    if cand.shape != (R, D) or status.numel() != 1:
        raise RuntimeError("vq_restart_gather: cand must be (R, %d) and status one int32" % D)
    if not 0 <= first < stride or rows.numel() < len(range(first, R, stride)):
        raise RuntimeError("vq_restart_gather: first=%d, stride=%d need 0 <= first < stride and %d positions (got %d)"
                           % (first, stride, len(range(first, R, stride)), rows.numel()))
    _check(lib().alvq_vq_restart_gather_f32(_ptr(flat, name="x"), _ptr(rows, torch.int64, "rows"), _ptr(cand, name="cand"),
                                            _ptr(status, torch.int32, "status"), N, D, R, int(first), int(stride), _stream()),
           "alvq_vq_restart_gather_f32")


def vq_restart_dead(cand, cluster_size, ema_w, codebook, counters, threshold, skip=None):
    K, D = codebook.shape
    R = cand.shape[0]
    if cluster_size.numel() != K or ema_w.shape != (K, D) or cand.shape != (R, D) or counters.numel() != 2:
        raise RuntimeError("vq_restart_dead: cluster_size must be (%d,), ema_w (%d, %d), cand (R, %d) and counters int64[2]"
                           % (K, K, D, D))
    _check(lib().alvq_vq_restart_dead_f32(_ptr(cand, name="cand"), _ptr(cluster_size, name="cluster_size"),
                                          _ptr(ema_w, name="ema_w"), _ptr(codebook, name="codebook"), _ptr(skip, name="skip"),
                                          _ptr(counters, torch.int64, "counters"), K, D, R, float(threshold), _stream()),
           "alvq_vq_restart_dead_f32")


def vq_backward(g, grad_loss, flat, codebook, idx, beta, want_dx=True, want_dE=True, dE_out=None):
    N, D = flat.shape
    K = codebook.shape[0]
    dx = torch.empty_like(flat) if want_dx else None
    dE = (dE_out if dE_out is not None else torch.zeros_like(codebook)) if want_dE else None
    ws = _workspace(lib().alvq_vq_backward_workspace_bytes(K, D), flat.device).data_ptr() if want_dE else None
    _check(lib().alvq_vq_backward_f32(_ptr(g, name="g"), _ptr(grad_loss, name="grad_loss"), _ptr(flat, name="x"),
                                      _ptr(codebook, name="codebook"), _ptr(idx, torch.int64, "idx"), _ptr(dx), _ptr(dE),
                                      ws, N, K, D, float(beta), _stream()), "alvq_vq_backward_f32")
    return dx, dE


def onehot(idx, K):
    N = idx.numel()
    enc = torch.empty((N, K), device=idx.device, dtype=torch.float32)
    _check(lib().alvq_onehot_f32(_ptr(idx, torch.int64, "idx"), _ptr(enc), N, K, _stream()), "alvq_onehot_f32")
    return enc


def onehot_to_index(enc):
    rows, K = enc.shape
    idx = torch.empty((rows,), device=enc.device, dtype=torch.int32)
    flag = torch.empty((1,), device=enc.device, dtype=torch.float32)
    fill_(flag, 0.0)
    flag = flag.view(torch.int32)
    _check(lib().alvq_onehot_to_index_f32(_ptr(enc, name="encodings"), idx.data_ptr(), flag.data_ptr(), rows, K, _stream()),
           "alvq_onehot_to_index_f32")
    return idx, flag


BAG_MAX_INDICES = 16384


def device_flag(device):
    flag = torch.empty((1,), device=device, dtype=torch.float32)
    fill_(flag, 0.0)
    return flag.view(torch.int32)


def indices_to_i32(idx, K, flag):
    out = torch.empty(idx.shape, device=idx.device, dtype=torch.int32)
    _check(lib().alvq_indices_to_i32(_ptr(idx, torch.int64, "idx"), out.data_ptr(), flag.data_ptr(), idx.numel(), K, _stream()),
           "alvq_indices_to_i32")
    return out


def embedding_bag_fwd(W, bias, idx, L, K, flag=None):
    B = idx.shape[0]
    M = W.shape[0]
    if W.shape[1] != L * K or tuple(idx.shape) != (B, L):
        raise RuntimeError("embedding_bag_fwd: W %s / idx %s do not match L=%d, K=%d" % (tuple(W.shape), tuple(idx.shape), L, K))
    if L > BAG_MAX_INDICES:
        raise RuntimeError("embedding_bag_fwd: L = %d exceeds the %d-index table" % (L, BAG_MAX_INDICES))
    out = torch.empty((B, M), device=W.device, dtype=torch.float32)
    step = max(1, BAG_MAX_INDICES // L)
    for b0 in range(0, B, step):
        nb = min(step, B - b0)
        _check(lib().alvq_embedding_bag_fwd_f32(_ptr(W, name="W"), _ptr(bias, name="bias"), _ptr(idx[b0:b0 + nb], torch.int32, "idx"),
                                                _ptr(out[b0:b0 + nb]), nb, L, K, M, flag.data_ptr() if flag is not None else None,
                                                _stream()), "alvq_embedding_bag_fwd_f32")
    return out


def embedding_bag_bwd(dz, idx, L, K, want_bias=True, flag=None, dW_out=None, db_out=None):
    B, M = dz.shape
    if dW_out is not None:
        if tuple(dW_out.shape) != (M, L * K):
            raise RuntimeError("embedding_bag_bwd: dW_out has shape %s, expected %s" % (tuple(dW_out.shape), (M, L * K)))
        dW = dW_out
    else:
        dW = torch.empty((M, L * K), device=dz.device, dtype=torch.float32)
        fill_(dW, 0.0)
    db = None
    if want_bias:
        db = db_out if db_out is not None else torch.empty((M,), device=dz.device, dtype=torch.float32)
    step = max(1, BAG_MAX_INDICES // L)
    for b0 in range(0, B, step):
        nb = min(step, B - b0)
        _check(lib().alvq_embedding_bag_bwd_f32(_ptr(dz[b0:b0 + nb], name="dz"), _ptr(idx[b0:b0 + nb], torch.int32, "idx"), _ptr(dW), _ptr(db),
                                                nb, L, K, M, int(b0 > 0 or db_out is not None),
                                                flag.data_ptr() if flag is not None else None, _stream()),
               "alvq_embedding_bag_bwd_f32")
    return dW, db


def jitter_gather(x, src, backward=False):
    L = x.shape[-1]
    y = torch.empty_like(x)
    _check(lib().alvq_jitter_gather_f32(_ptr(x, name="x"), _ptr(src, torch.int32, "src"), _ptr(y), x.numel() // L, L,
                                        int(bool(backward)), _stream()), "alvq_jitter_gather_f32")
    return y


def standardise(x, take_abs=False):
    B, C, L = x.shape
    y = torch.empty_like(x)
    _check(lib().alvq_standardise_f32(_ptr(x, name="x"), _ptr(y), B, C, L, int(bool(take_abs)), _stream()),
           "alvq_standardise_f32")
    return y


def mse(a, b):
    if a.shape != b.shape:
        raise RuntimeError("mse: shapes differ %s vs %s" % (tuple(a.shape), tuple(b.shape)))
    loss = torch.empty((1,), device=a.device, dtype=torch.float32)
    ws = torch.empty((EW_PARTIALS,), device=a.device, dtype=torch.float32)
    _check(lib().alvq_mse_f32(_ptr(a, name="a"), _ptr(b, name="b"), _ptr(loss), _ptr(ws), a.numel(), _stream()), "alvq_mse_f32")
    return loss


def mse_backward(a, b, grad_loss):
    grad = torch.empty_like(a)
    _check(lib().alvq_mse_backward_f32(_ptr(a, name="a"), _ptr(b, name="b"), _ptr(grad_loss, name="grad_loss"), _ptr(grad),
                                       a.numel(), _stream()), "alvq_mse_backward_f32")
    return grad


def fill_(t, value=0.0):
    if t.numel():
        _check(lib().alvq_fill_f32(_ptr(t, name="t"), float(value), t.numel(), _stream()), "alvq_fill_f32")
    return t


def add(a, b):
    out = torch.empty_like(a)
    _check(lib().alvq_add_f32(_ptr(a, name="a"), _ptr(b, name="b"), _ptr(out), a.numel(), _stream()), "alvq_add_f32")
    return out

# ... 237 lines not shown


def tsne_affinities(P, perplexity):
    N = P.shape[0]
    if P.dim() != 2 or P.shape[1] != N:
        raise RuntimeError("tsne_affinities: P must be (N, N) (got %s)" % (tuple(P.shape),))
    nbytes = lib().alvq_tsne_affinities_workspace_bytes(N)
    if nbytes < 0:
        raise RuntimeError("tsne_affinities: N=%d out of range" % N)
    beta = torch.empty((N,), device=P.device, dtype=torch.float64)
    S = torch.empty((N,), device=P.device, dtype=torch.float64)
    ws = torch.empty((nbytes,), device=P.device, dtype=torch.uint8)
    _check(lib().alvq_tsne_affinities_f32(_ptr(P, name="P"), _ptr(beta, torch.float64), _ptr(S, torch.float64),
                                          _ptr(ws, torch.uint8), N, float(perplexity), _stream()), "alvq_tsne_affinities_f32")
    return beta, S


def tsne_descend(P, Y, update, gains, grad, stats, n_iter, exaggeration, momentum, learning_rate, workspace=None):
    N = Y.shape[0]
    for name, t in (("Y", Y), ("update", update), ("gains", gains), ("grad", grad)):
        if t.shape != (N, 2):
            raise RuntimeError("tsne_descend: %s must be (%d, 2) (got %s)" % (name, N, tuple(t.shape)))
    if P.shape != (N, N) or stats.numel() < 2:
        raise RuntimeError("tsne_descend: P must be (%d, %d) and stats hold 2 values" % (N, N))
    nbytes = lib().alvq_tsne_descend_workspace_bytes(N)
    if nbytes < 0:
        raise RuntimeError("tsne_descend: N=%d out of range" % N)
    if workspace is None or workspace.numel() < nbytes:
        workspace = torch.empty((nbytes,), device=Y.device, dtype=torch.uint8)
    f64 = torch.float64
    _check(lib().alvq_tsne_descend_f64(_ptr(P, name="P"), _ptr(Y, f64, "Y"), _ptr(update, f64, "update"),
                                       _ptr(gains, f64, "gains"), _ptr(grad, f64, "grad"), _ptr(stats, f64, "stats"),
                                       _ptr(workspace, torch.uint8, "workspace"), N, int(n_iter), float(exaggeration),
                                       float(momentum), float(learning_rate), _stream()), "alvq_tsne_descend_f64")
    return workspace


def _conv16_name(f16, out, KW, M, rows):
    min_tiles = get_option("wide_min_tiles")
    if ((M + 255) // 256 * 256 - M) <= 32 and (rows // 256) * ((M + 255) // 256) >= min_tiles:
        return ("conv1d_bf16_k3_kernel<%d, %d>" if KW == 3 else "conv1d_bf16_v2_kernel<%d, %d>") % (out, f16)
    return "conv1d_bf16_kernel<%d, %d, %d>" % (KW, out, f16)


def _wgrad16_name(KW, with_bias, f16):
    sel = get_option("wgrad_v3")
    if not with_bias and ((KW == 1 and sel & 1) or (KW == 3 and sel & 2)):
        return "conv1d_wgrad_bf16_v3_kernel<%s, %d>" % ("3, 1, 2" if KW == 3 else "1, 2, 4", f16)
    return "conv1d_wgrad_bf16_v2_kernel<%s, %d>" % ("3, 2" if KW == 3 else "1, 4", f16)


_Format = collections.namedtuple("_Format", (
    "name", "planes", "bits", "scaled", "defer", "wcode", "wreads", "operands", "rows_code", "to_nlc", "to_ncl", "relu",
    "relu_flat", "pack", "conv", "wgrad", "wgrad_multi", "wgrad_ws", "conv_family", "wgrad_family"))
_FORMATS = {f.name: f for f in (
    _Format("bf16", planes=1, bits=True, scaled=False, defer=True, wcode=1, wreads=(1, 2), operands=("bf16", "bf16x3"),
            rows_code=1, to_nlc="alvq_ncl_to_nlc_bf16", to_ncl="alvq_nlc_to_ncl_f32", relu="alvq_relu_mask_bf16",
            relu_flat=True, pack="alvq_pack_weight_bf16", conv="alvq_conv1d_bf16", wgrad="alvq_conv1d_wgrad_bf16",
            wgrad_multi="alvq_conv1d_wgrad_bf16_multi", wgrad_ws="alvq_conv1d_wgrad_bf16_workspace_bytes",
            conv_family=functools.partial(_conv16_name, 0),
            wgrad_family=lambda KW, with_bias: _wgrad16_name(KW, with_bias, 0)),
    _Format("bf16x3", planes=2, bits=False, scaled=False, defer=False, wcode=2, wreads=(2,), operands=("bf16x3",),
            rows_code=2, to_nlc="alvq_ncl_to_nlc_bf16x3", to_ncl="alvq_nlc_to_ncl_bf16x3", relu="alvq_relu_mask_bf16x3",
            relu_flat=False, pack="alvq_pack_weight_bf16x3", conv="alvq_conv1d_bf16x3", wgrad="alvq_conv1d_wgrad_bf16x3",
            wgrad_multi="alvq_conv1d_wgrad_bf16x3_multi", wgrad_ws="alvq_conv1d_wgrad_bf16x3_workspace_bytes",
            conv_family=lambda out, KW, M, rows: "conv1d_bf16x3_kernel<%d, %d, ...>" % (out, KW),
            wgrad_family=lambda KW, with_bias: "conv1d_wgrad_bf16x3_kernel"),
    _Format("f16mx", planes=2, bits=True, scaled=True, defer=False, wcode=3, wreads=(3,), operands=("f16mx",),
            rows_code=3, to_nlc="alvq_ncl_to_nlc_f16mx", to_ncl="alvq_nlc_to_ncl_f16mx", relu="alvq_relu_mask_f16mx",
            relu_flat=False, pack=None, conv="alvq_conv1d_f16mx", wgrad="alvq_conv1d_wgrad_f16mx",
            wgrad_multi="alvq_conv1d_wgrad_f16mx_multi", wgrad_ws="alvq_conv1d_wgrad_f16mx_workspace_bytes",
            conv_family=lambda out, KW, M, rows: "conv1d_f16mx_kernel<%d, %d, ...>" % (out, KW),
            wgrad_family=lambda KW, with_bias: "conv1d_wgrad_f16mx_kernel"),
    _Format("f16", planes=1, bits=True, scaled=True, defer=True, wcode=3, wreads=(3,), operands=("f16", "f16mx"),
            rows_code=None, to_nlc="alvq_ncl_to_nlc_f16", to_ncl="alvq_nlc_to_ncl_f16", relu="alvq_relu_mask_bf16",
            relu_flat=True, pack=None, conv="alvq_conv1d_f16", wgrad="alvq_conv1d_wgrad_f16",
            wgrad_multi="alvq_conv1d_wgrad_f16_multi", wgrad_ws="alvq_conv1d_wgrad_bf16_workspace_bytes",
            conv_family=functools.partial(_conv16_name, 1),
            wgrad_family=lambda KW, with_bias: _wgrad16_name(KW, with_bias, 1)))}
_PACKERS = {f.wcode: f.pack for f in _FORMATS.values()}


def _format(planes, fmt):
    f = _FORMATS[fmt or ("bf16x3" if planes == 2 else "bf16")]
    if f.planes != planes:
        raise ValueError("format %s has %d plane(s), not %d" % (f.name, f.planes, planes))
    return f


class NLC:
    __slots__ = ("storage", "B", "L", "C", "Cp", "rows", "guard", "planes", "has_bits", "fmt", "gscale")

    def _shape(self, B, L, C, planes, fmt):
        f = _format(planes, fmt)
        L_ = lib()
        self.B, self.L, self.C, self.planes, self.fmt = B, L, C, f.planes, f.name
        self.Cp, self.rows, self.guard = L_.alvq_nlc_channels(C), L_.alvq_nlc_rows(B, L), L_.alvq_nlc_guard_rows()
        return f, f.planes * (self.rows + 2 * self.guard) * self.Cp + (self.rows * self.Cp // 16 if f.bits else 0)

    def __init__(self, B, L, C, device, planes=1, fmt=None, gscale=None):
        _, n = self._shape(B, L, C, planes, fmt)
        self.gscale, self.has_bits = gscale, False
        self.storage = torch.empty((n,), device=device, dtype=torch.bfloat16)

    @classmethod
    def wrap(cls, storage, B, L, C, planes=1, has_bits=False, fmt=None):
        self = cls.__new__(cls)
        f, n = self._shape(B, L, C, planes, fmt)
        self.gscale, self.storage = None, storage
        self.has_bits = bool(has_bits) and f.bits and storage.numel() >= n
        return self

    @property
    def ptr(self):
        return self.storage.data_ptr() + self.guard * self.Cp * 2

    @property
    def bits_ptr(self):
        return self.storage.data_ptr() + self.planes * (self.rows + 2 * self.guard) * self.Cp * 2

    def matrix(self, plane=0):
        g = (self.guard + plane * (self.rows + 2 * self.guard)) * self.Cp
        return self.storage[g:g + self.rows * self.Cp].view(self.rows, self.Cp)

    def to_ncl(self):
        if self.fmt in ("f16mx", "f16"):
            return nlc_to_ncl(self)
        m = self.matrix(0).float()
        if self.planes == 2:
            m = m + self.matrix(1).float()
        m = m[1:1 + self.B * (self.L + 1)].view(self.B, self.L + 1, self.Cp)
        return m[:, :self.L, :self.C].permute(0, 2, 1).contiguous()
# ... 97 lines not shown
            M, C, KW = w.shape
        else:
            C, M, KW = w.shape
        need = min(planes, 2) * lib().alvq_packed_weight_elems(M, C, KW)
        if wp.numel() != need or wp.dtype != torch.bfloat16:
            raise RuntimeError("pack_weights_batch: packed image has %d elements, expected %d" % (wp.numel(), need))
        d.w, d.wp, d.M, d.C, d.KW, d.w_layout = _ptr(w, name="w"), wp.data_ptr(), M, C, KW, w_layout
    _check(lib().alvq_pack_weights_bf16_batch(ctypes.addressof(arr), len(entries), planes, _stream()),
           "alvq_pack_weights_bf16_batch")


class AdamPackDesc(ctypes.Structure):
    _fields_ = [("w", ctypes.c_void_p), ("g", ctypes.c_void_p), ("m", ctypes.c_void_p), ("v", ctypes.c_void_p),
                ("wp_oik", ctypes.c_void_p), ("wp_iok", ctypes.c_void_p), ("dim0", ctypes.c_int32), ("dim1", ctypes.c_int32),
                ("KW", ctypes.c_int32)]


def adam_pack_batch(entries, planes, scalars, beta1=0.9, beta2=0.999, eps=1e-8, skip=None):
    if not entries:
        return
    arr = (AdamPackDesc * len(entries))()
    for d, (w, g, m, v, oik, iok) in zip(arr, entries):
        d.w, d.g, d.m, d.v = _ptr(w, name="w"), _ptr(g, name="g"), _ptr(m, name="m"), _ptr(v, name="v")
        d.wp_oik = oik.data_ptr() if oik is not None else None
        d.wp_iok = iok.data_ptr() if iok is not None else None
        d.dim0, d.dim1, d.KW = w.shape
    _check(lib().alvq_adam_pack_batch(ctypes.addressof(arr), len(entries), planes, _ptr(scalars, name="scalars"), float(beta1),
                                      float(beta2), float(eps), _ptr(skip, name="skip"), _stream()), "alvq_adam_pack_batch")


def adam_segments(param, grad, exp_avg, exp_avg_sq, segments, scalars, beta1=0.9, beta2=0.999, eps=1e-8, skip=None):
    segments = [(int(a), int(b)) for a, b in segments if b > a]
    if not segments:
        return
    lo = (ctypes.c_int64 * len(segments))(*[a for a, _ in segments])
    hi = (ctypes.c_int64 * len(segments))(*[b for _, b in segments])
    _check(lib().alvq_adam_segments_f32(_ptr(param, name="param"), _ptr(grad, name="grad"), _ptr(exp_avg, name="exp_avg"),
                                        _ptr(exp_avg_sq, name="exp_avg_sq"), lo, hi, len(segments), _ptr(scalars, name="scalars"),
                                        float(beta1), float(beta2), float(eps), _ptr(skip, name="skip"), _stream()),
           "alvq_adam_segments_f32")


def relu_mask_bf16(dy, t):
    f = _FORMATS[dy.fmt]
    out = nlc_like(dy, dy.C)
    dims = (dy.rows * dy.Cp,) if f.relu_flat else (dy.B, dy.C, dy.L)
    _check(getattr(lib(), f.relu)(dy.ptr, _nlc_ptr(t, dy, dy.C, "t"), out.ptr, *dims, _stream()), f.relu)
    return out


USE_SIGN_BITS = os.environ.get("ALVQ_SIGN_BITS", "1") != "0"


def conv1d_bf16(x, packed, bias=None, skip1=None, skip2=None, mask=None, post=None, relu=False, out_ncl=False):
    f = _FORMATS[x.fmt]
    wp, (M, C, KW, wcode) = packed
    if C != x.C:
        raise RuntimeError("conv1d_bf16: weight expects %d input channels, x has %d" % (C, x.C))
    if wcode not in f.wreads:
        raise RuntimeError("conv1d_bf16: weight packed for format %d, activation is %s" % (wcode, x.fmt))
    if bias is not None and bias.numel() != M:
        raise RuntimeError("conv1d_bf16: bias has %d elements, expected %d" % (bias.numel(), M))
    y = y2 = y_ncl = None
    if out_ncl:
        y_ncl = torch.empty((x.B, M, x.L), device=wp.device, dtype=torch.float32)
    else:
        y = nlc_like(x, M)
        y2 = nlc_like(x, M) if post is not None else None
    family = f.conv_family(int(bool(out_ncl)), KW, M, x.rows)
    extra = ()
    mask_ptr = _nlc_ptr(mask, x, M, "mask")
    bits_out = f.bits and y is not None and relu and USE_SIGN_BITS
    if f.bits:
        mask_bits = None
        if mask is not None and mask.has_bits and USE_SIGN_BITS:
            mask_bits, mask_ptr = mask.bits_ptr, None
        extra = (mask_bits, y.bits_ptr if bits_out else None)
    if f.scaled:
        extra += (_sptr(x.gscale, 1) if out_ncl else None,)
    with _timed(family, 2.0 * x.B * x.L * M * C * KW):
        rc = getattr(lib(), f.conv)(x.ptr, wp.data_ptr(), _ptr(bias, name="bias"), _nlc_ptr(skip1, x, M, "skip1"),
                                    _nlc_ptr(skip2, x, M, "skip2"), mask_ptr, _nlc_ptr(post, x, M, "post"),
                                    y.ptr if y is not None else None, y2.ptr if y2 is not None else None, _ptr(y_ncl),
                                    x.B, C, M, x.L, KW, int(bool(relu)), *extra, _stream())
    if bits_out:
        y.has_bits = True
    _check(rc, f.conv)
    if out_ncl:
        return y_ncl
    return (y, y2) if post is not None else y


def _wgrad_out(who, dy, x, KW, w_layout, dw_out, accumulate):
    shape = (dy.C, x.C, KW) if w_layout == W_OIK else (x.C, dy.C, KW)
    if dw_out is None:
        return torch.empty(shape, device=x.storage.device, dtype=torch.float32), False
    if tuple(dw_out.shape) != shape:
        raise RuntimeError("%s: dw_out has shape %s, expected %s" % (who, tuple(dw_out.shape), shape))
    return dw_out, accumulate


def _wgrad_scratch(f, dy, x, KW, deferred):
    nbytes = getattr(lib(), f.wgrad_ws)(x.B, x.C, dy.C, x.L, KW)
    dev = x.storage.device
    return arena_alloc(nbytes, dev) if deferred else _workspace(nbytes, dev).data_ptr()


def _wgrad_launch(f, symbol, family, head, ws_ptr, nseg, dy, x, KW, w_layout, dw, dbias, accumulate, defer):
    B, C, M, L = x.B, x.C, dy.C, x.L
    scale = dy.gscale if f.scaled else None
    with _timed(family, 2.0 * nseg * B * L * M * C * KW):
        rc = getattr(lib(), symbol)(*head, ws_ptr, B, C, M, L, KW, w_layout,
                                    WGRAD_DEFER if defer is not None else int(bool(accumulate)),
                                    *((_sptr(scale, 1),) if f.scaled else ()), _stream())
    _check(rc, symbol)
    if defer is not None:
        _defer_descs(defer, ws_ptr, dw, dbias, scale, nseg, B, C, M, L, KW, w_layout)


def conv1d_wgrad_bf16(dy, x, KW, w_layout=W_OIK, want_bias=False, dw_out=None, dbias_out=None, accumulate=False, defer=None):
    f = _FORMATS[dy.fmt]
    dw_out, accumulate = _wgrad_out("conv1d_wgrad_bf16", dy, x, KW, w_layout, dw_out, accumulate)
    if want_bias and dbias_out is None:
        dbias_out = torch.empty((dy.C,), device=x.storage.device, dtype=torch.float32)
    if not _fmt_serves(x, dy):
        raise RuntimeError("conv1d_wgrad_bf16: dy and x differ in format")
    if not (accumulate and f.defer):
        defer = None
    family = f.wgrad_family(KW, want_bias)
    dbias = dbias_out if want_bias else None
    _wgrad_launch(f, f.wgrad, family, (dy.ptr, x.ptr, _ptr(dw_out, name="dw"), _ptr(dbias, name="dbias")),
                  _wgrad_scratch(f, dy, x, KW, defer is not None), 1, dy, x, KW, w_layout, dw_out, dbias, accumulate, defer)
    return (dw_out, dbias_out) if want_bias else dw_out


def conv1d_wgrad_bf16_multi(pairs, KW, w_layout=W_OIK, dw_out=None, accumulate=False, defer=None):
    dy0, x0 = pairs[0]
    f = _FORMATS[dy0.fmt]
    for dy, x in pairs:
        if (dy.B, dy.L, dy.C, dy.fmt, x.B, x.L, x.C) != (dy0.B, dy0.L, dy0.C, dy0.fmt, x0.B, x0.L, x0.C) or not _fmt_serves(x, dy):
            raise RuntimeError("conv1d_wgrad_bf16_multi: all segments must share one shape and format")
        if f.scaled and dy.gscale is not dy0.gscale:
            raise RuntimeError("conv1d_wgrad_bf16_multi: the segments belong to different loss-scale chains")
    dw_out, accumulate = _wgrad_out("conv1d_wgrad_bf16_multi", dy0, x0, KW, w_layout, dw_out, accumulate)
    n = len(pairs)
    dys = (ctypes.c_void_p * n)(*[dy.ptr for dy, _ in pairs])
    xs = (ctypes.c_void_p * n)(*[x.ptr for _, x in pairs])
    if not (accumulate and f.defer):
        defer = None
    ws_ptr = _wgrad_scratch(f, dy0, x0, KW, defer is not None)
    _wgrad_launch(f, f.wgrad_multi, f.wgrad_family(KW, False), (dys, xs, n, _ptr(dw_out, name="dw")), ws_ptr, n, dy0, x0, KW,
                  w_layout, dw_out, None, accumulate, defer)
    return dw_out


def _rows(x, name):
    if x.dim() != 2:
        raise RuntimeError("%s must be (N, D) (got %s)" % (name, tuple(x.shape)))
    return x.shape


def kmeans_update(x, labels, labels_old, centers_old, centers_new, counts, stats, flags, tol, workspace=None):
    N, D = _rows(x, "kmeans_update: x")
# ... 72 lines not shown
```

acoustic_locating_vq-vae_amd/src/acoustic_locating_vq_vae/_ops.py:

```python
from __future__ import annotations

import os

import numpy as np
import torch

from . import _native as N

OIK, IOK = N.W_OIK, N.W_IOK

DEFAULT_DTYPE = "x3mx_hb"
MODES = ("x3mx_hb", "f16mx_hb", "bf16x3_hb", "f32", "bf16")
INTERNAL_MODES = ("f16mx", "bf16x3", "f16mx_hd")
_DTYPE = os.environ.get("ALVQ_DTYPE", DEFAULT_DTYPE)
if _DTYPE not in MODES:
    raise ValueError("ALVQ_DTYPE must be one of %s, got %r" % (", ".join(repr(m) for m in MODES), _DTYPE))


def set_compute_dtype(name, internal=False):
    global _DTYPE
    if name not in MODES and not (internal and name in INTERNAL_MODES):
        raise ValueError("compute dtype must be one of %s, got %r" % (", ".join(repr(m) for m in MODES), name))
    _DTYPE = name


def has_fp16_range(mode=None):
    return any(f is not None and f.scaled for e in _MODE_ENGINES[mode or _DTYPE].values() for f in (e.fwd, e.grad))


def get_compute_dtype():
    return _DTYPE


import weakref

_GRAD_SINKS = weakref.WeakValueDictionary()


def register_grad_sinks(params):
    for p in params:
        if p.grad is not None:
            _GRAD_SINKS[p.data_ptr()] = p.grad


_SINKS_ACTIVE = 0


class use_grad_sinks:

    def __enter__(self):
        global _SINKS_ACTIVE
        _SINKS_ACTIVE += 1

    def __exit__(self, *exc):
        global _SINKS_ACTIVE
        _SINKS_ACTIVE -= 1


_DEFERRED = None


class deferred_reduce:
    def __enter__(self):
        global _DEFERRED
        self.prev, _DEFERRED = _DEFERRED, (N.DeferredReductions() if os.environ.get("ALVQ_DEFER_REDUCE", "1") != "0" else None)
        return _DEFERRED

    def __exit__(self, *exc):
        global _DEFERRED
        _DEFERRED = self.prev


_API_FORWARDS = 0


def note_training_forward(device):
    global _API_FORWARDS
    if device.type != "cuda" or _SINKS_ACTIVE or not has_fp16_range() or torch.cuda.is_current_stream_capturing():
        return
    every = int(os.environ.get("ALVQ_RANGE_CHECK_EVERY", "200"))
    _API_FORWARDS += 1
    if every <= 0 or _API_FORWARDS < every:
        return
    _API_FORWARDS = 0
    flag = N.f16mx_range_flag(reset=True, device=device)
    if flag:
        import warnings
        warnings.warn("acoustic_locating_vq_vae: fp16 range flag %d in mode %s -- a value entering or produced inside the "
                      "fp16-range formats reached 65504 (or was NaN) during the last %d forward / backward passes; those steps "
                      "are saturated.  ALVQ_DTYPE=bf16x3_hb or f32 have fp32 range; train_step.Trainer skips such steps."
                      % (flag, _DTYPE, every), RuntimeWarning)


def _sink(t):
    if t is None or not _SINKS_ACTIVE or not len(_GRAD_SINKS) or not t.requires_grad:
        return None
    return _GRAD_SINKS.get(t.data_ptr())


class PackPool:

    def __init__(self, params, dynamic=None):
        self._eligible = {p.data_ptr(): p for p in params if p.dim() == 3}
        self._dynamic = None if dynamic is None else {p.data_ptr() for p in dynamic}
        self._entries = {}
        self._static_version = {}
        self._adam_version = {}

    def _is_static(self, ptr):
        return self._dynamic is not None and ptr not in self._dynamic

    def lookup(self, w, layout, planes):
        key = (w.data_ptr(), layout, planes)
        hit = self._entries.get(key)
        if hit is not None:
            return hit
        p = self._eligible.get(key[0])
        if p is None or p.shape != w.shape:
            return None
        img, tag = N.packed_weight_alloc(p.detach(), layout, planes)
        N.pack_weights_batch([(p.detach(), img, layout)], planes)
        self._entries[key] = (img, tag)
        if self._is_static(key[0]):
            self._static_version[key] = p._version
        return self._entries[key]

    def _refresh(self, keys):
        by_planes = {}
        for key in keys:
            ptr, layout, planes = key
            by_planes.setdefault(planes, []).append((self._eligible[ptr].detach(), self._entries[key][0], layout))
        for planes, entries in by_planes.items():
            N.pack_weights_batch(entries, planes)

    def refresh(self):
        keys = [k for k in self._entries if not self._is_static(k[0]) and
                self._adam_version.get(k) != self._eligible[k[0]]._version]
        if keys:
            self._refresh(keys)
            for k in keys:
                self._adam_version.pop(k, None)

    def refresh_static(self):
        stale = [k for k, v in self._static_version.items() if self._eligible[k[0]]._version != v]
        if stale:
            self._refresh(stale)
            for k in stale:
                self._static_version[k] = self._eligible[k[0]]._version

    def stale_dynamic(self):
# ... 116 lines not shown

def dense(x):
    if isinstance(x, StandardisedT):
        return x.materialise()
    if x.dtype != torch.float32:
        x = x.float()
    if x.is_contiguous():
        return x
    if x.dim() == 3 and x.permute(0, 2, 1).is_contiguous():
        return N.transpose12(x.permute(0, 2, 1))
    return x.contiguous()


class StandardisedT:

    def __init__(self, raw):
        self.raw = raw
        b, f, t = raw.shape
        self.shape = torch.Size((b, t, f))
        self.device, self.is_cuda, self.dtype, self.requires_grad = raw.device, raw.is_cuda, raw.dtype, False

    def dim(self):
        return 3

    def size(self, i=None):
        return self.shape if i is None else self.shape[i]

    def materialise(self):
        return N.transpose12(N.standardise(self.raw))


def _as_blc(x):
    if torch.is_tensor(x) and x.dim() == 3 and x.dtype == torch.float32 and not x.is_contiguous():
        xt = x.permute(0, 2, 1)
        if xt.is_contiguous():
            return xt
    return None


def _need_gpu(x, who):
    if not x.is_cuda:
        raise RuntimeError("%s: input is on %s -- this build runs the HIP path only (no CPU fallback); "
                           "move the model and data to the GPU" % (who, x.device))
    if x.device.index is not None and x.device.index != torch.cuda.current_device():
        raise RuntimeError("%s: input is on %s but the current device is cuda:%d -- call torch.cuda.set_device(%d) "
                           "(one process per GPU)" % (who, x.device, torch.cuda.current_device(), x.device.index))


class _F32Engine:
    name = "f32"
    fwd = grad = None
    can_defer = False
    wgrad_multi = None

    def enter(self, x, grad=False):
        return dense(x)

    def leave(self, a):
        return a

    def conv(self, x, w, layout=OIK, bias=None, skip1=None, skip2=None, mask=None, post=None, relu=False, out_f32=False):
        return N.conv1d(x, w, bias, skip1, skip2, mask, post, relu, layout)

    def wgrad(self, dy, x, kw, layout, want_bias=False, dw_out=None, dbias_out=None, accumulate=False):
        return N.conv1d_wgrad(dy, x, kw, layout, want_bias=want_bias, dw_out=dw_out, dbias_out=dbias_out,
                              accumulate=accumulate)

    def relu_mask(self, dy, t):
        return N.relu_mask(dy, t)

    def pack(self, act):
        return act, None

    def unpack(self, tensor, meta):
        return tensor


class _NLCEngine:
    can_defer = True
    wgrad_multi = staticmethod(N.conv1d_wgrad_bf16_multi)

    def __init__(self, name, fwd, grad):
        self.name, self.fwd, self.grad = name, N._FORMATS[fwd], N._FORMATS[grad]

    def _w(self, w, layout):
        wcode = self.fwd.wcode
        if _ACTIVE_POOL is not None:
            hit = _ACTIVE_POOL.lookup(w, layout, wcode)
            if hit is not None:
                return hit
        if torch.cuda.is_current_stream_capturing():
            return N.pack_weight(w.detach(), layout, wcode)
        return _cached_pack(w, layout, wcode)

    def _enter_rows(self, x, f):
        if os.environ.get("ALVQ_ROWS_BOUNDARY", "1") == "0":
            return None
        if isinstance(x, StandardisedT):
            if N.rows_to_nlc_supported(f.name, x.raw.shape[1], True):
                return N.rows_to_nlc(x.raw, f.planes, f.name, standardise=True)
            return None
        blc = _as_blc(x)
        if blc is not None and blc.is_cuda and N.rows_to_nlc_supported(f.name, blc.shape[1]):
            return N.rows_to_nlc(blc, f.planes, f.name)
        return None

    def enter(self, x, grad=False):
        f = self.grad if grad else self.fwd
        if not grad:
            hit = self._enter_rows(x, f)
            if hit is not None:
                return hit
        x = dense(x)
        return N.ncl_to_nlc(x, f.planes, f.name, N.grad_scale(x) if grad and f.scaled else None)

    def leave(self, a):
        return N.nlc_to_ncl(a)

    def conv(self, x, w, layout=OIK, bias=None, skip1=None, skip2=None, mask=None, post=None, relu=False, out_f32=False):
        return N.conv1d_bf16(x, self._w(w, layout), bias, skip1, skip2, mask, post, relu, out_ncl=out_f32)

    def wgrad(self, dy, x, kw, layout, want_bias=False, dw_out=None, dbias_out=None, accumulate=False, defer=None):
        return N.conv1d_wgrad_bf16(dy, x, kw, layout, want_bias=want_bias, dw_out=dw_out, dbias_out=dbias_out,
                                   accumulate=accumulate, defer=defer)

    def relu_mask(self, dy, t):
        return N.relu_mask_bf16(dy, t)

    def pack(self, act):
        return act.storage, (act.B, act.L, act.C, act.planes, act.has_bits, act.fmt)

    def unpack(self, tensor, meta):
        return N.NLC.wrap(tensor, *meta)


_ENGINE_BY_NAME = {e.name: e for e in (
    _F32Engine(),
    _NLCEngine("bf16",      "bf16",   "bf16"),
    _NLCEngine("bf16x3",    "bf16x3", "bf16x3"),
    _NLCEngine("f16mx",     "f16mx",  "f16mx"),
    _NLCEngine("f16mx_hb",  "f16mx",  "f16"),
    _NLCEngine("bf16x3_hb", "bf16x3", "bf16"),
    _NLCEngine("f16dec",    "f16",    "f16"))}
_MODE_ENGINES = {m: {None: _ENGINE_BY_NAME[m]} for m in ("f32", "bf16", "bf16x3", "f16mx", "f16mx_hb", "bf16x3_hb")}
_MODE_ENGINES["x3mx_hb"] = {None: _ENGINE_BY_NAME["bf16x3_hb"], "decoder": _ENGINE_BY_NAME["f16mx_hb"]}
_MODE_ENGINES["f16mx_hd"] = {None: _ENGINE_BY_NAME["f16mx_hb"], "decoder": _ENGINE_BY_NAME["f16dec"]}


def _engine(name=None, role=None):
    if name is not None:
        return _ENGINE_BY_NAME[name]
    roles = _MODE_ENGINES[_DTYPE]
    return roles.get(role, roles[None])


_ACT_TAP = None


def _save(ctx, eng, tensors, acts):
    if _ACT_TAP is not None:
        _ACT_TAP.append((eng.name, list(acts)))
    packed = [eng.pack(a) for a in acts]
    ctx.eng_name = eng.name
    ctx.n_plain = len(tensors)
    ctx.act_meta = [m for _, m in packed]
    ctx.save_for_backward(*tensors, *[t for t, _ in packed])


def _load(ctx):
    eng = _engine(ctx.eng_name)
    saved = ctx.saved_tensors
    plain = saved[:ctx.n_plain]
    acts = [eng.unpack(t, m) for t, m in zip(saved[ctx.n_plain:], ctx.act_meta)]
# ... 3 lines not shown
def _stack_forward(eng, t1, w1, w2, R, post=None):
    ts, us = [t1], []
    out = None
    for r in range(R):
        u = eng.conv(ts[-1], w1, relu=True)
        us.append(u)
        if r == R - 1 and post is not None:
            t, out = eng.conv(u, w2, skip1=ts[-1], relu=True, post=post)
        else:
            t = eng.conv(u, w2, skip1=ts[-1], relu=True)
        ts.append(t)
    if out is None:
        out = ts[-1]
    return ts, us, out


def _stack_backward(eng, dh, ts, us, w1, w2, R, outer=None):
    dw1 = dw2 = None
    if w1.requires_grad != w2.requires_grad:
        raise RuntimeError("the two weights of the shared Residual must be frozen or trainable together")
    train = w1.requires_grad
    fused = train and eng.wgrad_multi is not None and 1 < R <= 4
    pairs1, pairs2 = [], []
    for r in range(R - 1, -1, -1):
        du = eng.conv(dh, w2, IOK, mask=us[r])
        if fused:
            pairs2.append((dh, us[r]))
            pairs1.append((du, ts[r]))
        elif train:
            dw2, _ = _wgrad(eng, dh, us[r], 1, OIK, w2, dw_prev=dw2)
            dw1, _ = _wgrad(eng, du, ts[r], 3, OIK, w1, dw_prev=dw1)
        dh = eng.conv(du, w1, IOK, skip1=dh, skip2=outer if r == 0 else None, mask=ts[r])
    if fused:
        s1, s2 = _sink(w1), _sink(w2)
        dw2 = eng.wgrad_multi(pairs2, 1, OIK, dw_out=s2, accumulate=s2 is not None, **_defer_kw(eng, s2))
        dw1 = eng.wgrad_multi(pairs1, 3, OIK, dw_out=s1, accumulate=s1 is not None, **_defer_kw(eng, s1))
        dw1, dw2 = (None if s1 is not None else dw1), (None if s2 is not None else dw2)
    return dh, dw1, dw2


def _check_layers(R):
    if R < 1:
        raise NotImplementedError("num_residual_layers=0 is not supported on the HIP path (no script uses it)")


def _encoder_forward(eng, x, wc, bc, w1, w2, R):
    _check_layers(R)
    xi = eng.enter(x)
    t1 = eng.conv(xi, wc, bias=bc, relu=True)
    ts, us, out = _stack_forward(eng, t1, w1, w2, R, post=t1)
    return xi, ts, us, out


def _encoder_backward(eng, d_out, xi, ts, us, wc, bc, w1, w2, R, need_dx):
    dh = eng.relu_mask(d_out, ts[R])
    dh0, dw1, dw2 = _stack_backward(eng, dh, ts, us, w1, w2, R, outer=d_out)
    dwc, dbc = _wgrad(eng, dh0, xi, 3, OIK, wc, bc)
    dx = eng.conv(dh0, wc, IOK, out_f32=True) if need_dx else None
    return dx, dwc, dbc, dw1, dw2


class EncoderFn(torch.autograd.Function):

    @staticmethod
    def forward(ctx, x, wc, bc, w1, w2, R):
        eng = _engine()
        xi, ts, us, out = _encoder_forward(eng, x, wc, bc, w1, w2, R)
        ctx.R = R
        _save(ctx, eng, (wc, bc, w1, w2), [xi, *ts, *us])
        return eng.leave(out)

    @staticmethod
    def backward(ctx, d_out):
        R = ctx.R
        eng, (wc, bc, w1, w2), acts = _load(ctx)
        xi, ts, us = acts[0], acts[1:R + 2], acts[R + 2:]
        dx, dwc, dbc, dw1, dw2 = _encoder_backward(eng, eng.enter(d_out, grad=True), xi, ts, us, wc, bc, w1, w2, R,
                                                   ctx.needs_input_grad[0])
        return dx, dwc, dbc, dw1, dw2, None


class LatentFn(torch.autograd.Function):

    @staticmethod
    def forward(ctx, x, wc, bc, w1, w2, wp, bp, R):
        eng = _engine()
        xi, ts, us, out = _encoder_forward(eng, x, wc, bc, w1, w2, R)
        z = eng.conv(out, wp, bias=bp, out_f32=True)
        ctx.R = R
        _save(ctx, eng, (wc, bc, w1, w2, wp, bp), [xi, out, *ts, *us])
        return z

    @staticmethod
    def backward(ctx, dz):
        R = ctx.R
        eng, (wc, bc, w1, w2, wp, bp), acts = _load(ctx)
        xi, out, ts, us = acts[0], acts[1], acts[2:R + 3], acts[R + 3:]
        dzi = eng.enter(dz, grad=True)
        d_out = eng.conv(dzi, wp, IOK)
        dwp, dbp = _wgrad(eng, dzi, out, 3, OIK, wp, bp)
        dx, dwc, dbc, dw1, dw2 = _encoder_backward(eng, d_out, xi, ts, us, wc, bc, w1, w2, R, ctx.needs_input_grad[0])
        return dx, dwc, dbc, dw1, dw2, dwp, dbp, None


class StackFn(torch.autograd.Function):

    @staticmethod
    def forward(ctx, h0, w1, w2, R):
        eng = _engine()
        _check_layers(R)
        hi = eng.enter(h0)
        t1 = eng.relu_mask(hi, hi)
        ts, us, out = _stack_forward(eng, t1, w1, w2, R)
        ctx.R = R
        _save(ctx, eng, (w1, w2), [*ts, *us])
        return eng.leave(out)

    @staticmethod
    def backward(ctx, d_out):
        R = ctx.R
        eng, (w1, w2), acts = _load(ctx)
        ts, us = acts[:R + 1], acts[R + 1:]
        dh = eng.relu_mask(eng.enter(d_out, grad=True), ts[R])
        dh0, dw1, dw2 = _stack_backward(eng, dh, ts, us, w1, w2, R)
        return eng.leave(dh0), dw1, dw2, None


class ResidualLayerFn(torch.autograd.Function):

    @staticmethod
    def forward(ctx, x, w1, w2):
        eng = _engine()
        xi = eng.enter(x)
        t = eng.relu_mask(xi, xi)
        u = eng.conv(t, w1, relu=True)
        _save(ctx, eng, (w1, w2), [t, u])
        return eng.leave(eng.conv(u, w2, skip1=t))

    @staticmethod
    def backward(ctx, dy):
        eng, (w1, w2), (t, u) = _load(ctx)
        dyi = eng.enter(dy, grad=True)
        du = eng.conv(dyi, w2, IOK, mask=u)
        dw2, _ = _wgrad(eng, dyi, u, 1, OIK, w2)
        dw1, _ = _wgrad(eng, du, t, 3, OIK, w1)
        dx = eng.conv(du, w1, IOK, skip1=dyi, mask=t)
        return eng.leave(dx), dw1, dw2


class ConvFn(torch.autograd.Function):

    @staticmethod
    def forward(ctx, x, w, b, layout):
        eng = _engine()
# ... 235 lines not shown
```

acoustic_locating_vq-vae_amd/src/acoustic_locating_vq_vae/train_step.py:

```python
from __future__ import annotations

import os

import torch
import torch.distributed as dist

from . import _native as N
from . import _ops

_ALIGN = 64


def _round_up(n):
    return (n + _ALIGN - 1) // _ALIGN * _ALIGN


def _world_rank(group=None, without=(1, 0)):
    if not (dist.is_available() and dist.is_initialized()):
        return without
    return dist.get_world_size(group), dist.get_rank(group)


def unique_trainable(params):
    seen, out = set(), []
    for p in params:
        if p.requires_grad and id(p) not in seen:
            seen.add(id(p))
            out.append(p)
    return out


class FlatBuffers:

    def __init__(self, params, extra=0):
        self.params = unique_trainable(params)
        if not self.params:
            raise ValueError("no trainable parameters")
        dev = self.params[0].device
        self.offsets, total = [], _ALIGN
        for p in self.params:
            if p.device != dev or p.dtype != torch.float32:
                raise ValueError("all parameters must be fp32 on one device")
            self.offsets.append(total)
            total += _round_up(p.numel())
        self.extra_span = (total, total + extra) if extra else None
        total += _round_up(extra)
        self.numel = sum(p.numel() for p in self.params)
        self.flat = torch.zeros(total, device=dev, dtype=torch.float32)
        self.grad = torch.zeros(total, device=dev, dtype=torch.float32)
        for p, off in zip(self.params, self.offsets):
            n = p.numel()
            self.flat[off:off + n].copy_(p.data.reshape(-1))
            p.data = self.flat[off:off + n].view(p.shape)
            p.grad = self.grad[off:off + n].view(p.shape)
        self.skip_slot = self.grad[0:1]

    def zero_grad(self):
        if self.grad.is_cuda:
            N.fill_(self.grad, 0.0)
        else:
            self.grad.zero_()
        for p, off in zip(self.params, self.offsets):
            if p.grad is None or p.grad.data_ptr() != self.grad.data_ptr() + 4 * off:
                p.grad = self.grad[off:off + p.numel()].view(p.shape)

    def sync_grads(self, group=None, force=False):
        world = _world_rank(group, without=(0, 0))[0]
        if world == 0 or (world == 1 and not force):
            return 1.0
        dist.all_reduce(self.grad, op=dist.ReduceOp.SUM, group=group)
        return 1.0 / world

    def span(self, params):
        ids = {id(p) for p in params}
        idx = [i for i, p in enumerate(self.params) if id(p) in ids]
        if not idx or idx != list(range(idx[0], idx[-1] + 1)) or len(idx) != len(ids):
            raise ValueError("bucket parameters are not a contiguous run of the flat buffer")
        last = idx[-1]
        hi = self.offsets[last + 1] if last + 1 < len(self.offsets) else self.grad.numel()
        return (0 if idx[0] == 0 else self.offsets[idx[0]]), hi

    def sync_span(self, lo, hi, group=None, force=False):
        world = _world_rank(group, without=(0, 0))[0]
        if world == 0 or (world == 1 and not force):
            return None
        return dist.all_reduce(self.grad[lo:hi], op=dist.ReduceOp.SUM, group=group, async_op=True)

    def broadcast_params(self, src=0, group=None):
        if _world_rank(group)[0] > 1:
            dist.broadcast(self.flat, src=src, group=group)


class WarmupCosine:

    __slots__ = ("warmup_steps", "total_steps", "lr_min")

    def __init__(self, warmup_steps, total_steps=None, lr_min=0.0):
        if int(warmup_steps) != warmup_steps or warmup_steps < 0:
            raise ValueError("WarmupCosine: warmup_steps=%r must be an integer >= 0" % (warmup_steps,))
        if total_steps is not None and (int(total_steps) != total_steps or total_steps <= warmup_steps):
            raise ValueError("WarmupCosine: total_steps=%r must be an integer beyond warmup_steps=%r" % (total_steps, warmup_steps))
        if not lr_min >= 0:
            raise ValueError("WarmupCosine: lr_min=%r must be >= 0" % (lr_min,))
        self.warmup_steps = int(warmup_steps)
        self.total_steps = None if total_steps is None else int(total_steps)
        self.lr_min = float(lr_min)

    def __repr__(self):
        return "WarmupCosine(warmup_steps=%d, total_steps=%r, lr_min=%g)" % (self.warmup_steps, self.total_steps, self.lr_min)


# ... 193 lines not shown
        if want_buckets >= 2 and kind != "echoed" and hasattr(model, "_encoder") and hasattr(model, "_pre_vq_conv"):
            late = unique_trainable(list(model._encoder.parameters()) + list(model._pre_vq_conv.parameters()))
            late_ids = {id(p) for p in late}
            early = [p for p in self.buffers.params if id(p) not in late_ids]
            if late and early:
                self._late_params, self._early_params = late, early
                self._buckets = (self.buffers.span(early), self.buffers.span(late))
                xs = self.buffers.extra_span
                if xs is not None and not any(lo <= xs[0] and xs[1] <= hi for lo, hi in self._buckets):
                    raise RuntimeError("the EMA statistics span (restart candidates included) is not inside one gradient bucket")

    def preprocess(self, raw, wiener=None):
        if self.kind == "speech":
            x = N.standardise(_ops.dense(raw), take_abs=True)
            return x, x
        if self.kind == "rir":
            x = _ops.StandardisedT(_ops.dense(raw))
            w = wiener.float()
            tgt = N.standardise(w.unsqueeze(2).contiguous()).view(w.shape[0], 1, w.shape[1])
            return x, tgt
        x = N.standardise(_ops.dense(raw))
        return x, x

    def forward_loss(self, x, target):
        if self.kind == "echoed":
            recon, sp_perp, _ = self.model(x, x.permute(0, 2, 1))
            recon_error = _ops.MSEFn.apply(recon, target)
            return recon_error, recon_error, sp_perp
        vq_loss, recon, perplexity = self.model(x)
        recon_error = _ops.MSEFn.apply(recon, target)
        return recon_error + vq_loss, recon_error, perplexity

    def _check_frozen(self):
        if [p.requires_grad for p in self.buffers.params] != self._trainable:
            raise RuntimeError("requires_grad of a parameter changed after the Trainer was built; build a new Trainer")
        if self.kind == "echoed" and bool(self.model.flag_train_encoder) != self._echoed_train_encoder:
            raise RuntimeError("set_train_encoder(%s) was called after the Trainer was built; build a new Trainer so "
                               "the encoders' parameters are (not) part of the optimiser" % self.model.flag_train_encoder)

    def _adam_skip(self):
        skip = [self.buffers.extra_span] if self.buffers.extra_span is not None else []
        ids = {id(p): i for i, p in enumerate(self.buffers.params)}
        for m in self.model.modules():
            if hasattr(m, "_train_vq") and not m._train_vq and id(m._embedding.weight) in ids:
                i = ids[id(m._embedding.weight)]
                skip.append((self.buffers.offsets[i], self.buffers.offsets[i] + m._embedding.weight.numel()))
        return skip

    def _body(self, raw, wiener):
        if self.buffers.flat.is_cuda:
            N.arena_reset(self.buffers.flat.device)
        for sink in self._ema_sinks.values():
            sink.written = False
        with _ops.use_pack_pool(self.pack_pool), _ops.use_grad_sinks(), _ops.deferred_reduce() as reductions, \
                _ops.use_ema_sinks(self._ema_sinks):
            x, target = self.preprocess(raw, wiener)
            self.buffers.zero_grad()
            if self._one is None or self._one.device != x.device:
                self._one = torch.ones((), device=x.device)
            if self._buckets is None:
                loss, recon_error, perplexity = self.forward_loss(x, target)
                loss.backward(self._one)
            else:
                with _ops.latent_tap() as tap:
                    loss, recon_error, perplexity = self.forward_loss(x, target)
                loss.backward(self._one)
                self._cut = tap[0] if tap else None
            if reductions:
                N.wgrad_reduce_batch(reductions)
            if self._cut is None:
                self._post_verdict()
        return loss.detach(), recon_error.detach(), perplexity.detach()

    def _post_verdict(self):
        if self.opt.guard and _ops.has_fp16_range():
            N.range_flag_to_slot(self.buffers.skip_slot)

    def _body_late(self):
        if self._cut is None:
            return
        z, leaf = self._cut
        self._cut = None
        with _ops.use_pack_pool(self.pack_pool, refresh=False), _ops.use_grad_sinks(), _ops.deferred_reduce() as reductions:
            z.backward(leaf.grad)
            if reductions:
                N.wgrad_reduce_batch(reductions)
            self._post_verdict()

    def _sync_early(self):
        return self.buffers.sync_span(*self._buckets[0], group=self.group, force=self.force_collective) if self._buckets else None

    def _finish(self, early_work=None):
        if self._buckets is None:
            self.buffers.sync_grads(self.group, force=self.force_collective)
        else:
            late_work = self.buffers.sync_span(*self._buckets[1], group=self.group, force=self.force_collective)
            for w in (early_work, late_work):
                if w is not None:
                    w.wait()
        if self.opt.max_grad_norm is not None:
            xs = self.buffers.extra_span
            self.opt.clip(_ALIGN, xs[0] if xs is not None else self.buffers.grad.numel())
        if self.pack_pool is not None:
            self.opt.apply(self._adam_skip(), pack_pool=self.pack_pool)
        else:
            self.opt.apply(self._adam_skip())
        for m in self._ema:
            sink = self._ema_sinks[id(m)]
            if sink.written:
                m.apply_update(sink, skip=self.opt._skip)

    def grad_norm(self):
        return self.opt.grad_norm()

    def clipped_steps(self, reset=True):
        return self.opt.clipped_steps(reset)

    def restarted_codes(self):
        return [m.restarted_codes() for m in self._ema]

    def _broadcast_ema(self):
        if not self._ema or _world_rank(self.group)[0] == 1:
            return
        src = dist.get_global_rank(self.group, 0) if self.group is not None else 0
        for m in self._ema:
            for t in (m._ema_cluster_size, m._ema_w.data, m._embedding.weight.data):
                dist.broadcast(t, src=src, group=self.group)

    def state_dict(self):
        state = {"model": self.model.state_dict(), "exp_avg": self.opt.exp_avg.clone(), "exp_avg_sq": self.opt.exp_avg_sq.clone(),
                 "step": self.opt.applied_steps(),
                 "numel": self.buffers.flat.numel(), "kind": self.kind}
        if self._restart:
            state["restart_rng"] = [m._restart_gen.get_state() for m in self._restart]
        return state

    def load_state_dict(self, state):
        if state["numel"] != self.buffers.flat.numel() or state["kind"] != self.kind:
            raise ValueError("checkpoint is for a different trainer (kind %s, %d flat elements)" % (state["kind"], state["numel"]))
# ... 147 lines not shown
```

include/alvq.h:

```cpp
#ifndef ALVQ_H
#define ALVQ_H

#include <stdint.h>

#ifdef __cplusplus
extern "C" {
#endif

#define ALVQ_OK 0
#define ALVQ_EINVAL (-1)
#define ALVQ_EUNSUPPORTED (-2)

#define ALVQ_W_OIK 0
#define ALVQ_W_IOK 1

#define ALVQ_F32 0
#define ALVQ_BF16 1

const char* alvq_version(void);
const char* alvq_last_error(void);

int alvq_set_option(const char* name, int64_t value);
int64_t alvq_get_option(const char* name);

// ... 126 lines not shown
                          int D, void* stream);

int alvq_vq_ema_update_f32(const float* counts, const float* sums, float* cluster_size, float* ema_w, float* codebook,
                           const float* skip, int K, int D, double decay, double epsilon, void* stream);

int alvq_vq_restart_gather_f32(const float* x, const int64_t* rows, float* cand, int* status, int64_t N, int D, int R, int first,
                               int stride, void* stream);

int alvq_vq_restart_dead_f32(const float* cand, float* cluster_size, float* ema_w, float* codebook, const float* skip,
                             int64_t* counters, int K, int D, int R, float threshold, void* stream);

int64_t alvq_kmeans_plusplus_workspace_bytes(int64_t N, int T);
int alvq_kmeans_plusplus_f32(const float* x, const double* uniforms, float* centers, int64_t* indices, void* workspace,
                             int64_t N, int K, int D, int T, int64_t first, void* stream);

int64_t alvq_nlc_rows(int B, int L);
int alvq_nlc_channels(int C);
int alvq_nlc_guard_rows(void);

int64_t alvq_packed_weight_elems(int M, int C, int KW);
int alvq_pack_weight_bf16(const float* w, void* wp, int M, int C, int KW, int w_layout, void* stream);

typedef struct alvq_pack_desc {
  const float* w;
  void* wp;
  int32_t M, C, KW, w_layout;
} alvq_pack_desc;
int alvq_pack_weights_bf16_batch(const alvq_pack_desc* descs, int n, int planes, void* stream);

typedef struct alvq_adam_pack_desc {
  float* w; const float* g; float* m; float* v;
  void* wp_oik; void* wp_iok;
  int32_t dim0, dim1, KW;
} alvq_adam_pack_desc;
int alvq_adam_pack_batch(const alvq_adam_pack_desc* descs, int n, int planes, const float* scalars,
                         float beta1, float beta2, float eps, const float* skip, void* stream);
int alvq_adam_segments_f32(float* param, const float* grad, float* exp_avg, float* exp_avg_sq,
                           const int64_t* lo, const int64_t* hi, int nseg, const float* scalars,
                           float beta1, float beta2, float eps, const float* skip, void* stream);

int alvq_rows_to_nlc(const float* x, void* y, int B, int C, int L, int fmt, int standardise, int take_abs, void* stream);
int alvq_rows_to_nlc_max_std_rows(void);

int alvq_ncl_to_nlc_bf16(const float* x, void* y, int B, int C, int L, void* stream);

int alvq_nlc_to_ncl_f32(const void* x, float* y, int B, int C, int L, void* stream);

int alvq_relu_mask_bf16(const void* dy, const void* t, void* out, int64_t n, void* stream);

int alvq_conv1d_bf16(const void* x, const void* wp, const float* bias, const void* skip1, const void* skip2,
                     const void* mask, const void* post, void* y, void* y2, float* y_ncl,
                     int B, int C, int M, int L, int KW, int relu, const void* mask_bits, void* relu_bits_out,
                     void* stream);

int64_t alvq_conv1d_wgrad_bf16_workspace_bytes(int B, int C, int M, int L, int KW);
int alvq_conv1d_wgrad_bf16(const void* dy, const void* x, float* dw, float* dbias, void* workspace,
                           int B, int C, int M, int L, int KW, int w_layout, int accumulate, void* stream);

int alvq_conv1d_wgrad_bf16_multi(const void* const* dy, const void* const* x, int nseg, float* dw, void* workspace,
                                 int B, int C, int M, int L, int KW, int w_layout, int accumulate, void* stream);
int alvq_conv1d_wgrad_bf16_splits(int B, int C, int M, int L, int KW, int nseg, int with_bias);

#define ALVQ_WGRAD_DEFER 2
int64_t alvq_conv1d_wgrad_bf16_bias_offset(int B, int C, int M, int L, int KW);
typedef struct alvq_reduce_desc {
  const float* partial;
  float* dst;
  const float* scale;
  int32_t splits, KW, M, C, w_layout, accumulate;
  int64_t stride;
} alvq_reduce_desc;
int alvq_wgrad_reduce_batch(const alvq_reduce_desc* descs, int n, void* stream);

int64_t alvq_nlc_plane_bytes(int B, int L, int C);
int alvq_pack_weight_bf16x3(const float* w, void* wp, int M, int C, int KW, int w_layout, void* stream);
int alvq_ncl_to_nlc_bf16x3(const float* x, void* y, int B, int C, int L, void* stream);
int alvq_nlc_to_ncl_bf16x3(const void* x, float* y, int B, int C, int L, void* stream);
int alvq_relu_mask_bf16x3(const void* dy, const void* t, void* out, int B, int C, int L, void* stream);
int alvq_conv1d_bf16x3(const void* x, const void* wp, const float* bias, const void* skip1, const void* skip2,
                       const void* mask, const void* post, void* y, void* y2, float* y_ncl,
                       int B, int C, int M, int L, int KW, int relu, void* stream);
int64_t alvq_conv1d_wgrad_bf16x3_workspace_bytes(int B, int C, int M, int L, int KW);
int alvq_conv1d_wgrad_bf16x3(const void* dy, const void* x, float* dw, float* dbias, void* workspace,
                             int B, int C, int M, int L, int KW, int w_layout, int accumulate, void* stream);
int alvq_conv1d_wgrad_bf16x3_multi(const void* const* dy, const void* const* x, int nseg, float* dw, void* workspace,
                                   int B, int C, int M, int L, int KW, int w_layout, int accumulate, void* stream);
int alvq_conv1d_wgrad_bf16x3_splits(int B, int C, int M, int L, int KW, int nseg);

int alvq_grad_scale_f32(const float* x, int64_t n, float* state, void* stream);
int alvq_f16mx_range_flag(int* out, int reset, void* stream);
int alvq_ncl_to_nlc_f16mx(const float* x, void* y, int B, int C, int L, const float* scale, void* stream);
int alvq_nlc_to_ncl_f16mx(const void* x, float* y, int B, int C, int L, const float* scale, void* stream);
int alvq_relu_mask_f16mx(const void* dy, const void* t, void* out, int B, int C, int L, void* stream);
int alvq_conv1d_f16mx(const void* x, const void* wp, const float* bias, const void* skip1, const void* skip2,
                      const void* mask, const void* post, void* y, void* y2, float* y_ncl,
                      int B, int C, int M, int L, int KW, int relu, const void* mask_bits, void* relu_bits_out,
                      const float* out_scale, void* stream);
int64_t alvq_conv1d_wgrad_f16mx_workspace_bytes(int B, int C, int M, int L, int KW);
int alvq_conv1d_wgrad_f16mx(const void* dy, const void* x, float* dw, float* dbias, void* workspace,
                            int B, int C, int M, int L, int KW, int w_layout, int accumulate,
                            const float* inv_scale, void* stream);
int alvq_conv1d_wgrad_f16mx_multi(const void* const* dy, const void* const* x, int nseg, float* dw, void* workspace,
                                  int B, int C, int M, int L, int KW, int w_layout, int accumulate,
                                  const float* inv_scale, void* stream);
int alvq_conv1d_wgrad_f16mx_splits(int B, int C, int M, int L, int KW, int nseg);

int alvq_ncl_to_nlc_f16(const float* x, void* y, int B, int C, int L, const float* scale, void* stream);
int alvq_nlc_to_ncl_f16(const void* x, float* y, int B, int C, int L, const float* scale, void* stream);
int alvq_conv1d_f16(const void* x, const void* wp, const float* bias, const void* skip1, const void* skip2,
                    const void* mask, const void* post, void* y, void* y2, float* y_ncl,
                    int B, int C, int M, int L, int KW, int relu, const void* mask_bits, void* relu_bits_out,
                    const float* out_scale, void* stream);
int alvq_conv1d_wgrad_f16(const void* dy, const void* x, float* dw, float* dbias, void* workspace,
                          int B, int C, int M, int L, int KW, int w_layout, int accumulate,
                          const float* inv_scale, void* stream);
int alvq_conv1d_wgrad_f16_multi(const void* const* dy, const void* const* x, int nseg, float* dw, void* workspace,
                                int B, int C, int M, int L, int KW, int w_layout, int accumulate,
                                const float* inv_scale, void* stream);

int alvq_onehot_to_index_f32(const float* encodings, int32_t* idx, int* not_onehot, int64_t rows, int K, void* stream);
int alvq_indices_to_i32(const int64_t* idx, int32_t* out, int* bad_index, int64_t n, int K, void* stream);
int alvq_embedding_bag_fwd_f32(const float* W, const float* bias, const int32_t* idx, float* out,
                               int B, int L, int K, int M, int* bad_index, void* stream);
int alvq_embedding_bag_bwd_f32(const float* dz, const int32_t* idx, float* dW, float* dbias,
                               int B, int L, int K, int M, int accumulate_bias, int* bad_index, void* stream);

#ifdef __cplusplus
}
#endif
#endif
```

Before: 7658.

## Fuse relu gating into conv epilogue, vectorize wgrad reduce, skip grad zero-fill

Adds a gated conv epilogue that writes a ReLU-masked copy of the output, so the encoder backward no longer runs a separate relu_mask kernel. It also vectorizes the OIK wgrad split reduction with float4 loads and an LDS transpose for KW=3. The zero-fill of the flat gradient buffer is replaced by first-touch writes, with only untouched spans filled at the end. Small wgrad problems get fewer splits through a new divisor option, and the Adam pack path checks pointer alignment before taking its vector path. Together these bring more bookkeeping and correctness risk around which gradients must be zeroed.

```diff
diff --git a/acoustic_locating_vq-vae_amd/csrc/alvq_common.h b/acoustic_locating_vq-vae_amd/csrc/alvq_common.h
--- a/acoustic_locating_vq-vae_amd/csrc/alvq_common.h
+++ b/acoustic_locating_vq-vae_amd/csrc/alvq_common.h
@@ -9,7 +9,7 @@
 
 void set_error(const char* fmt, ...);
 
-enum Option { OPT_WIDE_MIN_TILES, OPT_FX_ROWS, OPT_FX_NARROW, OPT_CONV_V2, OPT_CONV_K3, OPT_WGRAD_V3, OPT_VQ_REG, OPT_COUNT };
+enum Option { OPT_WIDE_MIN_TILES, OPT_FX_ROWS, OPT_FX_NARROW, OPT_CONV_V2, OPT_CONV_K3, OPT_WGRAD_V3, OPT_VQ_REG, OPT_WGRAD_SPLIT_DIV, OPT_COUNT };
 long option(int id);
 
 inline int check_launch(const char* what) {
diff --git a/acoustic_locating_vq-vae_amd/csrc/api.hip b/acoustic_locating_vq-vae_amd/csrc/api.hip
--- a/acoustic_locating_vq-vae_amd/csrc/api.hip
+++ b/acoustic_locating_vq-vae_amd/csrc/api.hip
@@ -24,6 +24,7 @@
     {"conv_k3", "ALVQ_CONV_K3", 1},
     {"wgrad_v3", "ALVQ_WGRAD_V3", 3},
     {"vq_reg", "ALVQ_VQ_REG", 1},
+    {"wgrad_split_div", "ALVQ_WGRAD_SPLIT_DIV", 1},
 };
 static std::atomic<long> g_opt[OPT_COUNT];
 static std::atomic<int> g_opt_ready{0};
diff --git a/acoustic_locating_vq-vae_amd/csrc/bf16_common.h b/acoustic_locating_vq-vae_amd/csrc/bf16_common.h
--- a/acoustic_locating_vq-vae_amd/csrc/bf16_common.h
+++ b/acoustic_locating_vq-vae_amd/csrc/bf16_common.h
@@ -58,6 +58,9 @@
   int elem;
   const float* out_scale;
   int* range_flag;
+  const u16* gate;
+  const unsigned char* gate_bits;
+  u16* yg;
 };
 
 constexpr int WP_ROWS = 256;
diff --git a/acoustic_locating_vq-vae_amd/csrc/conv1d_bf16.hip b/acoustic_locating_vq-vae_amd/csrc/conv1d_bf16.hip
--- a/acoustic_locating_vq-vae_amd/csrc/conv1d_bf16.hip
+++ b/acoustic_locating_vq-vae_amd/csrc/conv1d_bf16.hip
@@ -250,10 +250,13 @@
 
 static int conv1d_16bit(int elem, const float* out_scale, const void* x, const void* wp, const float* bias, const void* skip1,
                         const void* skip2, const void* mask, const void* post, void* y, void* y2, float* y_ncl, int B, int C, int M,
-                        int L, int KW, int relu, const void* mask_bits, void* relu_bits_out, void* stream) {
-  const char* const who = elem ? "alvq_conv1d_f16" : "alvq_conv1d_bf16";
+                        int L, int KW, int relu, const void* mask_bits, void* relu_bits_out, void* stream, bool gated = false,
+                        const void* gate = nullptr, const void* gate_bits = nullptr, void* y_gated = nullptr) {
+  const char* const who = elem ? (gated ? "alvq_conv1d_f16_gated" : "alvq_conv1d_f16") : (gated ? "alvq_conv1d_bf16_gated" : "alvq_conv1d_bf16");
   if (int rc = check_conv_args(who, x, wp, skip1, skip2, mask, post, y, y2, y_ncl, B, C, M, L, KW, relu, mask_bits, relu_bits_out))
     return rc;
+  if (gated)
+    if (int rc = check_conv_gate(who, y, gate, gate_bits, y_gated)) return rc;
   ConvBArgs a{(const u16*)x, (const u16*)wp, bias, (const u16*)skip1, (const u16*)skip2, (const u16*)mask, (const u16*)post,
               (u16*)y, (u16*)y2, y_ncl, B, L, pad_to(C, TB_K), M, pad_to(M, TB_K), pad_to(M, WP_ROWS), relu,
               (int)(alvq_nlc_rows(B, L) / TB_R), pad_to(M, TB_M) / TB_M, (const unsigned char*)mask_bits,
@@ -263,6 +266,9 @@
   a.elem = elem;
   a.out_scale = out_scale;
   a.range_flag = elem ? fx_range_flag_ptr() : nullptr;
+  a.gate = (const u16*)gate;
+  a.gate_bits = (const unsigned char*)gate_bits;
+  a.yg = (u16*)y_gated;
   const long use_v2 = option(OPT_CONV_V2), use_k3 = option(OPT_CONV_K3);
   const long tiles256 = (alvq_nlc_rows(B, L) / 256) * (pad_to(M, 256) / 256);
   const long min_tiles = option(OPT_WIDE_MIN_TILES);
@@ -281,11 +287,27 @@
                       stream);
 }
 
+extern "C" int alvq_conv1d_bf16_gated(const void* x, const void* wp, const float* bias, const void* skip1, const void* skip2,
+                                      const void* mask, const void* post, void* y, void* y2, float* y_ncl, int B, int C, int M,
+                                      int L, int KW, int relu, const void* mask_bits, void* relu_bits_out, const void* gate,
+                                      const void* gate_bits, void* y_gated, void* stream) {
+  return conv1d_16bit(0, nullptr, x, wp, bias, skip1, skip2, mask, post, y, y2, y_ncl, B, C, M, L, KW, relu, mask_bits, relu_bits_out,
+                      stream, true, gate, gate_bits, y_gated);
+}
+
 extern "C" int alvq_conv1d_f16(const void* x, const void* wp, const float* bias, const void* skip1, const void* skip2,
                                const void* mask, const void* post, void* y, void* y2, float* y_ncl, int B, int C, int M, int L,
                                int KW, int relu, const void* mask_bits, void* relu_bits_out, const float* out_scale, void* stream) {
   return conv1d_16bit(1, out_scale, x, wp, bias, skip1, skip2, mask, post, y, y2, y_ncl, B, C, M, L, KW, relu, mask_bits,
                       relu_bits_out, stream);
+}
+
+extern "C" int alvq_conv1d_f16_gated(const void* x, const void* wp, const float* bias, const void* skip1, const void* skip2,
+                                     const void* mask, const void* post, void* y, void* y2, float* y_ncl, int B, int C, int M, int L,
+                                     int KW, int relu, const void* mask_bits, void* relu_bits_out, const float* out_scale,
+                                     const void* gate, const void* gate_bits, void* y_gated, void* stream) {
+  return conv1d_16bit(1, out_scale, x, wp, bias, skip1, skip2, mask, post, y, y2, y_ncl, B, C, M, L, KW, relu, mask_bits,
+                      relu_bits_out, stream, true, gate, gate_bits, y_gated);
 }
 
 extern "C" int alvq_ncl_to_nlc_f16(const float* x, void* y, int B, int C, int L, const float* scale, void* stream) {
diff --git a/acoustic_locating_vq-vae_amd/csrc/conv1d_bf16_tile256.h b/acoustic_locating_vq-vae_amd/csrc/conv1d_bf16_tile256.h
--- a/acoustic_locating_vq-vae_amd/csrc/conv1d_bf16_tile256.h
+++ b/acoustic_locating_vq-vae_amd/csrc/conv1d_bf16_tile256.h
@@ -133,6 +133,21 @@
 #pragma unroll
         for (int e = 0; e < 4; ++e) fp16_watch(watch, out[e]);
       }
+      if (a.yg) {
+        u32x4 og;
+        if (a.gate_bits) {
+          const int bt = (int)a.gate_bits[o >> 3];
+#pragma unroll
+          for (int e = 0; e < 4; ++e)
+            og[e] = out[e] & ((((unsigned)((bt << (31 - 2 * e)) >> 31)) & 0xffffu) | (((unsigned)((bt << (30 - 2 * e)) >> 31)) & 0xffff0000u));
+        } else {
+          const u16x8 gt = *(const u16x8*)(a.gate + o);
+#pragma unroll
+          for (int e = 0; e < 4; ++e)
+            og[e] = out[e] & (((short)gt[2 * e] > 0 ? 0xffffu : 0u) | ((short)gt[2 * e + 1] > 0 ? 0xffff0000u : 0u));
+        }
+        *(u32x4*)(a.yg + o) = og;
+      }
       if (a.y2) {
         const u16x8 ps = *(const u16x8*)(a.post + o);
         u32x4 out2;
diff --git a/acoustic_locating_vq-vae_amd/csrc/conv1d_wgrad_bf16_v2.hip b/acoustic_locating_vq-vae_amd/csrc/conv1d_wgrad_bf16_v2.hip
--- a/acoustic_locating_vq-vae_amd/csrc/conv1d_wgrad_bf16_v2.hip
+++ b/acoustic_locating_vq-vae_amd/csrc/conv1d_wgrad_bf16_v2.hip
@@ -473,6 +473,18 @@
   return WgradTile{(v3 && KW == 1) ? 256 : 128, KW == 3 ? 128 : 256}.count(C, M);
 }
 
+static int wgrad_v2_plan(int total_rows, int tiles, long partial_bytes, int* chunks_per_split) {
+  const int splits = wgrad_split_plan(total_rows, tiles, chunks_per_split);
+  const long div = option(OPT_WGRAD_SPLIT_DIV);
+  if (div <= 1 || tiles > 16 || partial_bytes >= (4L << 20)) return splits;
+  const int nchunks = total_rows / 64;
+  int want = splits / (int)div;
+  if (want < 1) want = 1;
+  const int cps = (nchunks + want - 1) / want;
+  *chunks_per_split = cps;
+  return (nchunks + cps - 1) / cps;
+}
+
 static constexpr int wg_slot(int v3, int KW, int F16) { return (v3 * 2 + (KW == 3)) * 2 + F16; }
 typedef KernelTable<void (*)(WgradV2Args), 8> WgTable;
 static WgTable wg_table() {
@@ -487,7 +499,7 @@
 
 int conv1d_wgrad_bf16_v2_splits(int total_rows, int C, int M, int KW, int nseg, bool with_bias) {
   int cps;
-  return wgrad_split_plan(nseg * total_rows, wgrad_v2_tiles(C, M, KW, wgrad_uses_v3(KW, with_bias)), &cps);
+  return wgrad_v2_plan(nseg * total_rows, wgrad_v2_tiles(C, M, KW, wgrad_uses_v3(KW, with_bias)), 4L * KW * M * C, &cps);
 }
 
 int64_t conv1d_wgrad_bf16_v2_workspace_bytes(int total_rows, int C, int M, int KW) {
@@ -513,7 +525,7 @@
   a.total_rows = total_rows; a.nseg = nseg;
   const bool v3 = wgrad_uses_v3(KW, dbias != nullptr);
   if (v3 && KW == 1) a.mtiles = (M + 255) / 256;
-  a.splits = wgrad_split_plan(nseg * total_rows, a.mtiles * a.ctiles, &a.chunks_per_split);
+  a.splits = wgrad_v2_plan(nseg * total_rows, a.mtiles * a.ctiles, 4L * KW * M * C, &a.chunks_per_split);
   ALVQ_REQUIRE(a.mtiles * a.ctiles == wgrad_v2_tiles(C, M, KW, v3) &&
                    (int64_t)a.splits * KW * M * C * 4 <= conv1d_wgrad_bf16_v2_workspace_bytes(total_rows, C, M, KW),
                ALVQ_EINVAL, "alvq_conv1d_wgrad_bf16: %d splits exceed what alvq_conv1d_wgrad_bf16_workspace_bytes sizes", a.splits);
diff --git a/acoustic_locating_vq-vae_amd/csrc/nlc_host.h b/acoustic_locating_vq-vae_amd/csrc/nlc_host.h
--- a/acoustic_locating_vq-vae_amd/csrc/nlc_host.h
+++ b/acoustic_locating_vq-vae_amd/csrc/nlc_host.h
@@ -35,6 +35,13 @@
   ALVQ_REQUIRE((long)B * (L + 1) < (1L << 30), ALVQ_EUNSUPPORTED, "%s: problem too large", who);
   ALVQ_REQUIRE(!(mask && mask_bits), ALVQ_EINVAL, "%s: pass the mask as a tensor or as bits, not both", who);
   ALVQ_REQUIRE(!y_ncl || (!mask_bits && !bits_out), ALVQ_EUNSUPPORTED, "%s: sign bits go with the NLC output", who);
+  return ALVQ_OK;
+}
+
+inline int check_conv_gate(const char* who, const void* y, const void* gate, const void* gate_bits, const void* y_gated) {
+  ALVQ_REQUIRE(y_gated, ALVQ_EINVAL, "%s: null y_gated", who);
+  ALVQ_REQUIRE(y, ALVQ_EUNSUPPORTED, "%s: the gated output goes with the NLC output", who);
+  ALVQ_REQUIRE((gate != nullptr) != (gate_bits != nullptr), ALVQ_EINVAL, "%s: pass the gate as a tensor or as bits, one of them", who);
   return ALVQ_OK;
 }
 
diff --git a/acoustic_locating_vq-vae_amd/csrc/pack_weights.hip b/acoustic_locating_vq-vae_amd/csrc/pack_weights.hip
--- a/acoustic_locating_vq-vae_amd/csrc/pack_weights.hip
+++ b/acoustic_locating_vq-vae_amd/csrc/pack_weights.hip
@@ -88,6 +88,7 @@
   u16* oik; u16* iok;
   int dim0, dim1, KW, blk0, tiles1;
   int oik_Mp, oik_Cp, iok_Mp, iok_Cp;
+  int vec;
 };
 struct AdamPackBatch {
   AdamPackDesc d[AP_MAX];
@@ -112,7 +113,7 @@
   const float lr_bc1 = b.sc[0], bc2_sqrt = b.sc[1], gscale = b.sc[2];
   const float beta1 = b.beta1, beta2 = b.beta2, eps = b.eps;
   const int run = 64 * KW;
-  if (q0 + 64 <= d.dim1 && ((d.dim1 * KW) & 3) == 0) {
+  if (d.vec && q0 + 64 <= d.dim1) {
 #pragma unroll 2
     for (int e4 = tid; e4 < 8 * run; e4 += 256) {
       const int e = 4 * e4, rr = e / run, j = e - rr * run;
@@ -266,6 +267,7 @@
       AdamPackDesc& d = b.d[i];
       d.w = s.w; d.g = s.g; d.m = s.m; d.v = s.v; d.oik = (u16*)s.wp_oik; d.iok = (u16*)s.wp_iok;
       d.dim0 = s.dim0; d.dim1 = s.dim1; d.KW = s.KW;
+      d.vec = (((uintptr_t)s.w | (uintptr_t)s.g | (uintptr_t)s.m | (uintptr_t)s.v) & 15) == 0 && ((s.dim1 * s.KW) & 3) == 0;
       d.oik_Mp = pad_to(s.dim0, WP_ROWS); d.oik_Cp = pad_to(s.dim1, TB_K);
       d.iok_Mp = pad_to(s.dim1, WP_ROWS); d.iok_Cp = pad_to(s.dim0, TB_K);
       d.blk0 = blocks; d.tiles1 = (s.dim1 + 63) / 64;
diff --git a/acoustic_locating_vq-vae_amd/csrc/wgrad_reduce.h b/acoustic_locating_vq-vae_amd/csrc/wgrad_reduce.h
--- a/acoustic_locating_vq-vae_amd/csrc/wgrad_reduce.h
+++ b/acoustic_locating_vq-vae_amd/csrc/wgrad_reduce.h
@@ -2,6 +2,11 @@
 #include "alvq_common.h"
 
 namespace alvq {
+
+static __device__ __forceinline__ float wgrad_reduce_out(const float* old, float s, int accumulate) {
+  if (accumulate == 1) return *old + s;
+  return accumulate == ALVQ_REDUCE_FIRST_TOUCH ? 0.0f + s : s;
+}
 
 static __device__ __forceinline__ void wgrad_reduce_body(const float* partial, float* dw, int splits, int KW, int M, int C,
                                                          int w_layout, int accumulate, const float* scale, long stride, int bid,
@@ -30,8 +35,9 @@
       }
       if (scale) { s0 *= sc; s1 *= sc; s2 *= sc; }
       float* o = dw + 3 * q;
-      if (accumulate) { s0 += o[0]; s1 += o[1]; s2 += o[2]; }
-      o[0] = s0; o[1] = s1; o[2] = s2;
+      o[0] = wgrad_reduce_out(o, s0, accumulate);
+      o[1] = wgrad_reduce_out(o + 1, s1, accumulate);
+      o[2] = wgrad_reduce_out(o + 2, s2, accumulate);
     }
     return;
   }
@@ -57,12 +63,78 @@
     }
     for (; k < splits; ++k) s += partial[(long)k * stride + src];
     if (scale) s *= sc;
-    dw[e] = accumulate ? dw[e] + s : s;
+    dw[e] = wgrad_reduce_out(dw + e, s, accumulate);
   }
 }
 static __global__ void wgrad_reduce_kernel(const float* partial, float* dw, int splits, int KW, int M, int C, int w_layout,
                                     int accumulate, const float* scale) {
   wgrad_reduce_body(partial, dw, splits, KW, M, C, w_layout, accumulate, scale, (long)KW * M * C, blockIdx.x, gridDim.x);
+}
+
+static __host__ __device__ __forceinline__ bool wgrad_reduce_vec_ok(const float* partial, const float* dw, long pairs, long stride) {
+  return (((unsigned long long)partial | (unsigned long long)dw) & 15) == 0 && ((pairs | stride) & 3) == 0;
+}
+template <int KW, int NS>
+static __device__ __forceinline__ void wgrad_reduce_vec_splits(f32x4 (&s)[KW], const f32x4* p, long plane4, long stride4) {
+  f32x4 v[NS][KW];
+#pragma unroll
+  for (int i = 0; i < NS; ++i)
+#pragma unroll
+    for (int t = 0; t < KW; ++t) v[i][t] = p[i * stride4 + t * plane4];
+#pragma unroll
+  for (int i = 0; i < NS; ++i)
+#pragma unroll
+    for (int t = 0; t < KW; ++t) s[t] += v[i][t];
+}
+static __device__ __forceinline__ void wgrad_reduce_vec_store(f32x4* o, f32x4 v, int accumulate) {
+  if (accumulate == 1) v = *o + v;
+  else if (accumulate == ALVQ_REDUCE_FIRST_TOUCH) v = f32x4{0.f, 0.f, 0.f, 0.f} + v;
+  *o = v;
+}
+template <int KW>
+static __device__ __forceinline__ void wgrad_reduce_oik_vec_body(float* lds, const float* partial, float* dw, int splits, long pairs,
+                                                                 int accumulate, const float* scale, long stride, int bid, int nblk) {
+  const long quads = pairs / 4, plane4 = pairs / 4, stride4 = stride / 4;
+  const int tid = threadIdx.x;
+  for (long q0 = bid * 256L; q0 < quads; q0 += (long)nblk * 256) {
+    const long q = q0 + tid;
+    f32x4 s[KW];
+#pragma unroll
+    for (int t = 0; t < KW; ++t) s[t] = f32x4{0.f, 0.f, 0.f, 0.f};
+    if (q < quads) {
+      const f32x4* p = (const f32x4*)partial + q;
+      int k = 0;
+      for (; k + 8 <= splits; k += 8) wgrad_reduce_vec_splits<KW, 8>(s, p + k * stride4, plane4, stride4);
+      if (k + 4 <= splits) { wgrad_reduce_vec_splits<KW, 4>(s, p + k * stride4, plane4, stride4); k += 4; }
+      if (k + 2 <= splits) { wgrad_reduce_vec_splits<KW, 2>(s, p + k * stride4, plane4, stride4); k += 2; }
+      if (k < splits) wgrad_reduce_vec_splits<KW, 1>(s, p + k * stride4, plane4, stride4);
+      if (scale) {
+        const float sc = *scale;
+#pragma unroll
+        for (int t = 0; t < KW; ++t) s[t] *= sc;
+      }
+    }
+    if (KW == 1) {
+      if (q < quads) wgrad_reduce_vec_store((f32x4*)dw + q, s[0], accumulate);
+    } else {
+      if (q0 != bid * 256L) __syncthreads();
+      if (q < quads) {
+        f32x4* w = (f32x4*)lds + 3 * tid;
+        w[0] = f32x4{s[0][0], s[1][0], s[2][0], s[0][1]};
+        w[1] = f32x4{s[1][1], s[2][1], s[0][2], s[1][2]};
+        w[2] = f32x4{s[2][2], s[0][3], s[1][3], s[2][3]};
+      }
+      __syncthreads();
+      const long left = quads - q0;
+      const int n4 = 3 * (int)(left < 256 ? left : 256);
+      f32x4* o = (f32x4*)dw + 3 * q0;
+#pragma unroll
+      for (int r = 0; r < 3; ++r) {
+        const int i = tid + 256 * r;
+        if (i < n4) wgrad_reduce_vec_store(o + i, ((const f32x4*)lds)[i], accumulate);
+      }
+    }
+  }
 }
 
 template <int RB>
@@ -151,7 +223,7 @@
     const long o = ((long)(c0 + cc) * M + m0) * KW + j;
     float v = tile[KW - 1 - tt][mr][cc];
     if (scale) v *= *scale;
-    dw[o] = accumulate ? dw[o] + v : v;
+    dw[o] = wgrad_reduce_out(dw + o, v, accumulate);
   }
 }
 template <int RB>
diff --git a/acoustic_locating_vq-vae_amd/csrc/wgrad_reduce_batch.hip b/acoustic_locating_vq-vae_amd/csrc/wgrad_reduce_batch.hip
--- a/acoustic_locating_vq-vae_amd/csrc/wgrad_reduce_batch.hip
+++ b/acoustic_locating_vq-vae_amd/csrc/wgrad_reduce_batch.hip
@@ -12,16 +12,20 @@
 };
 
 __global__ __launch_bounds__(256) void wgrad_reduce_batch_kernel(ReduceBatch b) {
-  __shared__ float tile[3][16][65];
+  __shared__ __attribute__((aligned(16))) float tile[3][16][65];
   int di = 0;
   for (int i = 1; i < b.n; ++i)
     if ((int)blockIdx.x >= b.blk0[i]) di = i;
   const alvq_reduce_desc& d = b.d[di];
   const int lb = blockIdx.x - b.blk0[di];
   const int acc = d.accumulate;
+  const long pairs = (long)d.M * d.C;
   if (d.w_layout == ALVQ_W_IOK && d.stride == (int64_t)d.KW * d.M * d.C)
     wgrad_reduce_iok_body<16>(tile, d.partial, d.dst, d.splits, d.KW, d.M, d.C, acc, d.scale, lb);
-  else
+  else if (d.w_layout == ALVQ_W_OIK && wgrad_reduce_vec_ok(d.partial, d.dst, pairs, (long)d.stride)) {
+    if (d.KW == 3) wgrad_reduce_oik_vec_body<3>(&tile[0][0][0], d.partial, d.dst, d.splits, pairs, acc, d.scale, (long)d.stride, lb, b.nblk[di]);
+    else wgrad_reduce_oik_vec_body<1>(&tile[0][0][0], d.partial, d.dst, d.splits, pairs, acc, d.scale, (long)d.stride, lb, b.nblk[di]);
+  } else
     wgrad_reduce_body(d.partial, d.dst, d.splits, d.KW, d.M, d.C, d.w_layout, acc, d.scale, (long)d.stride, lb, b.nblk[di]);
 }
 
@@ -38,17 +42,25 @@
                  "alvq_wgrad_reduce_batch: bad dims in descriptor %d", i);
     ALVQ_REQUIRE(s.w_layout == ALVQ_W_OIK || s.w_layout == ALVQ_W_IOK, ALVQ_EINVAL, "alvq_wgrad_reduce_batch: w_layout in descriptor %d", i);
     ALVQ_REQUIRE(s.stride >= (int64_t)s.KW * s.M * s.C, ALVQ_EINVAL, "alvq_wgrad_reduce_batch: stride in descriptor %d", i);
+    ALVQ_REQUIRE(s.accumulate >= 0 && s.accumulate <= ALVQ_REDUCE_FIRST_TOUCH, ALVQ_EINVAL, "alvq_wgrad_reduce_batch: accumulate in descriptor %d", i);
   }
-  for (int i0 = 0; i0 < n; i0 += RB_MAX) {
+  for (int i0 = 0; i0 < n;) {
     ReduceBatch b{};
-    b.n = n - i0 < RB_MAX ? n - i0 : RB_MAX;
     int blocks = 0;
-    for (int i = 0; i < b.n; ++i) {
+    for (; i0 + b.n < n && b.n < RB_MAX; ++b.n) {
+      const int i = b.n;
       const alvq_reduce_desc& s = descs[i0 + i];
+      bool in_launch = false, earlier = false;
+      for (int j = 0; j < i0 + i; ++j)
+        if (descs[j].dst == s.dst) (j >= i0 ? in_launch : earlier) = true;
+      if (in_launch) break;
       b.d[i] = s;
+      if (s.accumulate == ALVQ_REDUCE_FIRST_TOUCH && earlier) b.d[i].accumulate = 1;
       const long total = (long)s.KW * s.M * s.C;
       int nb;
       if (s.w_layout == ALVQ_W_IOK && s.stride == total) nb = ((s.M + 15) / 16) * ((s.C + 63) / 64);
+      else if (s.w_layout == ALVQ_W_OIK && wgrad_reduce_vec_ok(s.partial, s.dst, (long)s.M * s.C, (long)s.stride))
+        nb = (int)(((long)s.M * s.C / 4 + 255) / 256);
       else {
         nb = (int)((total + 255) / 256);
         if (nb > 2048) nb = 2048;
@@ -60,6 +72,7 @@
     hipLaunchKernelGGL(wgrad_reduce_batch_kernel, dim3(blocks), dim3(256), 0, (hipStream_t)stream, b);
     int rc = check_launch("alvq_wgrad_reduce_batch");
     if (rc) return rc;
+    i0 += b.n;
   }
   return ALVQ_OK;
 }
diff --git a/acoustic_locating_vq-vae_amd/src/acoustic_locating_vq_vae/_native.py b/acoustic_locating_vq-vae_amd/src/acoustic_locating_vq_vae/_native.py
--- a/acoustic_locating_vq-vae_amd/src/acoustic_locating_vq_vae/_native.py
+++ b/acoustic_locating_vq-vae_amd/src/acoustic_locating_vq_vae/_native.py
@@ -71,6 +71,7 @@
     "alvq_nlc_to_ncl_f32": (_i32, [_c_void_p, _c_void_p, _i32, _i32, _i32, _c_void_p]),
     "alvq_relu_mask_bf16": (_i32, [_c_void_p] * 3 + [_i64, _c_void_p]),
     "alvq_conv1d_bf16": (_i32, [_c_void_p] * 10 + [_i32] * 6 + [_c_void_p] * 3),
+    "alvq_conv1d_bf16_gated": (_i32, [_c_void_p] * 10 + [_i32] * 6 + [_c_void_p] * 6),
     "alvq_conv1d_wgrad_bf16_workspace_bytes": (_i64, [_i32] * 5),
     "alvq_conv1d_wgrad_bf16": (_i32, [_c_void_p] * 5 + [_i32] * 7 + [_c_void_p]),
     "alvq_conv1d_wgrad_bf16_multi": (_i32, [_c_void_p, _c_void_p, _i32, _c_void_p, _c_void_p] + [_i32] * 7 + [_c_void_p]),
@@ -98,6 +99,7 @@
     "alvq_ncl_to_nlc_f16": (_i32, [_c_void_p, _c_void_p, _i32, _i32, _i32, _c_void_p, _c_void_p]),
     "alvq_nlc_to_ncl_f16": (_i32, [_c_void_p, _c_void_p, _i32, _i32, _i32, _c_void_p, _c_void_p]),
     "alvq_conv1d_f16": (_i32, [_c_void_p] * 10 + [_i32] * 6 + [_c_void_p] * 4),
+    "alvq_conv1d_f16_gated": (_i32, [_c_void_p] * 10 + [_i32] * 6 + [_c_void_p] * 7),
     "alvq_conv1d_wgrad_f16": (_i32, [_c_void_p] * 5 + [_i32] * 7 + [_c_void_p, _c_void_p]),
     "alvq_conv1d_wgrad_f16_multi": (_i32, [_c_void_p, _c_void_p, _i32, _c_void_p, _c_void_p] + [_i32] * 7 + [_c_void_p, _c_void_p]),
     "alvq_conv1d_wgrad_bf16_bias_offset": (_i64, [_i32] * 5),
@@ -321,6 +323,21 @@
         st["off"] = 0
 
 
+REDUCE_FIRST_TOUCH = 2
+_FIRST_TOUCH = None
+
+
+def _adds_into(*tensors):
+    if _FIRST_TOUCH is not None:
+        for t in tensors:
+            if t is not None:
+                _FIRST_TOUCH.adds(t.data_ptr())
+
+
+def _reduce_mode(dst):
+    return REDUCE_FIRST_TOUCH if _FIRST_TOUCH is not None and _FIRST_TOUCH.stores(dst.data_ptr()) else 1
+
+
 class DeferredReductions(list):
 
     def __init__(self):
@@ -347,10 +364,11 @@
     if scale is not None and hasattr(defer, "keep"):
         defer.keep.append(scale)
     splits = L_.alvq_conv1d_wgrad_bf16_splits(B, C, M, L, KW, nseg, int(dbias is not None))
-    defer.append(ReduceDesc(ws_ptr, dw.data_ptr(), scale_ptr, splits, KW, M, C, w_layout, 1, KW * M * C))
+    defer.append(ReduceDesc(ws_ptr, dw.data_ptr(), scale_ptr, splits, KW, M, C, w_layout, _reduce_mode(dw), KW * M * C))
     if dbias is not None:
         off = L_.alvq_conv1d_wgrad_bf16_bias_offset(B, C, M, L, KW)
-        defer.append(ReduceDesc(ws_ptr + off, dbias.data_ptr(), scale_ptr, splits, 1, 1, M, W_OIK, 1, (M + 63) // 64 * 64))
+        defer.append(ReduceDesc(ws_ptr + off, dbias.data_ptr(), scale_ptr, splits, 1, 1, M, W_OIK, _reduce_mode(dbias),
+                                (M + 63) // 64 * 64))
 
 
 def conv1d_wgrad(dy, x, KW, w_layout=W_OIK, want_bias=False, dw_out=None, dbias_out=None, accumulate=False):
@@ -370,6 +388,8 @@
     if nbytes < 0:
         raise RuntimeError("conv1d_wgrad: unsupported shape")
     ws = _workspace(nbytes, x.device)
+    if accumulate:
+        _adds_into(dw_out, dbias_out if want_bias else None)
     with _timed("conv1d_wgrad_f32_kernel", 2.0 * B * L * M * C * KW):
         rc = lib().alvq_conv1d_wgrad_f32(_ptr(dy, name="dy"), _ptr(x, name="x"), _ptr(dw_out, name="dw"),
                                          _ptr(dbias_out, name="dbias") if want_bias else None, ws.data_ptr(),
@@ -464,6 +484,8 @@
     K = codebook.shape[0]
     dx = torch.empty_like(flat) if want_dx else None
     dE = (dE_out if dE_out is not None else torch.zeros_like(codebook)) if want_dE else None
+    if want_dE:
+        _adds_into(dE_out)
     ws = _workspace(lib().alvq_vq_backward_workspace_bytes(K, D), flat.device).data_ptr() if want_dE else None
     _check(lib().alvq_vq_backward_f32(_ptr(g, name="g"), _ptr(grad_loss, name="grad_loss"), _ptr(flat, name="x"),
                                       _ptr(codebook, name="codebook"), _ptr(idx, torch.int64, "idx"), _ptr(dx), _ptr(dE),
@@ -534,6 +556,7 @@
     db = None
     if want_bias:
         db = db_out if db_out is not None else torch.empty((M,), device=dz.device, dtype=torch.float32)
+    _adds_into(dW_out, db_out if want_bias else None)
     step = max(1, BAG_MAX_INDICES // L)
     for b0 in range(0, B, step):
         nb = min(step, B - b0)
@@ -877,32 +900,32 @@
 
 _Format = collections.namedtuple("_Format", (
     "name", "planes", "bits", "scaled", "defer", "wcode", "wreads", "operands", "rows_code", "to_nlc", "to_ncl", "relu",
-    "relu_flat", "pack", "conv", "wgrad", "wgrad_multi", "wgrad_ws", "conv_family", "wgrad_family"))
+    "relu_flat", "pack", "conv", "wgrad", "wgrad_multi", "wgrad_ws", "conv_family", "wgrad_family", "conv_gated"))
 _FORMATS = {f.name: f for f in (
     _Format("bf16", planes=1, bits=True, scaled=False, defer=True, wcode=1, wreads=(1, 2), operands=("bf16", "bf16x3"),
             rows_code=1, to_nlc="alvq_ncl_to_nlc_bf16", to_ncl="alvq_nlc_to_ncl_f32", relu="alvq_relu_mask_bf16",
             relu_flat=True, pack="alvq_pack_weight_bf16", conv="alvq_conv1d_bf16", wgrad="alvq_conv1d_wgrad_bf16",
             wgrad_multi="alvq_conv1d_wgrad_bf16_multi", wgrad_ws="alvq_conv1d_wgrad_bf16_workspace_bytes",
             conv_family=functools.partial(_conv16_name, 0),
-            wgrad_family=lambda KW, with_bias: _wgrad16_name(KW, with_bias, 0)),
+            wgrad_family=lambda KW, with_bias: _wgrad16_name(KW, with_bias, 0), conv_gated="alvq_conv1d_bf16_gated"),
     _Format("bf16x3", planes=2, bits=False, scaled=False, defer=False, wcode=2, wreads=(2,), operands=("bf16x3",),
             rows_code=2, to_nlc="alvq_ncl_to_nlc_bf16x3", to_ncl="alvq_nlc_to_ncl_bf16x3", relu="alvq_relu_mask_bf16x3",
             relu_flat=False, pack="alvq_pack_weight_bf16x3", conv="alvq_conv1d_bf16x3", wgrad="alvq_conv1d_wgrad_bf16x3",
             wgrad_multi="alvq_conv1d_wgrad_bf16x3_multi", wgrad_ws="alvq_conv1d_wgrad_bf16x3_workspace_bytes",
             conv_family=lambda out, KW, M, rows: "conv1d_bf16x3_kernel<%d, %d, ...>" % (out, KW),
-            wgrad_family=lambda KW, with_bias: "conv1d_wgrad_bf16x3_kernel"),
+            wgrad_family=lambda KW, with_bias: "conv1d_wgrad_bf16x3_kernel", conv_gated=None),
     _Format("f16mx", planes=2, bits=True, scaled=True, defer=False, wcode=3, wreads=(3,), operands=("f16mx",),
             rows_code=3, to_nlc="alvq_ncl_to_nlc_f16mx", to_ncl="alvq_nlc_to_ncl_f16mx", relu="alvq_relu_mask_f16mx",
             relu_flat=False, pack=None, conv="alvq_conv1d_f16mx", wgrad="alvq_conv1d_wgrad_f16mx",
             wgrad_multi="alvq_conv1d_wgrad_f16mx_multi", wgrad_ws="alvq_conv1d_wgrad_f16mx_workspace_bytes",
             conv_family=lambda out, KW, M, rows: "conv1d_f16mx_kernel<%d, %d, ...>" % (out, KW),
-            wgrad_family=lambda KW, with_bias: "conv1d_wgrad_f16mx_kernel"),
+            wgrad_family=lambda KW, with_bias: "conv1d_wgrad_f16mx_kernel", conv_gated=None),
     _Format("f16", planes=1, bits=True, scaled=True, defer=True, wcode=3, wreads=(3,), operands=("f16", "f16mx"),
             rows_code=None, to_nlc="alvq_ncl_to_nlc_f16", to_ncl="alvq_nlc_to_ncl_f16", relu="alvq_relu_mask_bf16",
             relu_flat=True, pack=None, conv="alvq_conv1d_f16", wgrad="alvq_conv1d_wgrad_f16",
             wgrad_multi="alvq_conv1d_wgrad_f16_multi", wgrad_ws="alvq_conv1d_wgrad_bf16_workspace_bytes",
             conv_family=functools.partial(_conv16_name, 1),
-            wgrad_family=lambda KW, with_bias: _wgrad16_name(KW, with_bias, 1)))}
+            wgrad_family=lambda KW, with_bias: _wgrad16_name(KW, with_bias, 1), conv_gated="alvq_conv1d_f16_gated"))}
 _PACKERS = {f.wcode: f.pack for f in _FORMATS.values()}
 
 
@@ -1106,8 +1129,10 @@
 USE_SIGN_BITS = os.environ.get("ALVQ_SIGN_BITS", "1") != "0"
 
 
-def conv1d_bf16(x, packed, bias=None, skip1=None, skip2=None, mask=None, post=None, relu=False, out_ncl=False):
+def conv1d_bf16(x, packed, bias=None, skip1=None, skip2=None, mask=None, post=None, relu=False, out_ncl=False, gate=None):
     f = _FORMATS[x.fmt]
+    if gate is not None and (out_ncl or f.conv_gated is None):
+        raise RuntimeError("conv1d_bf16: no gated second output %s" % ("beside an fp32 output" if out_ncl else "in format " + x.fmt))
     wp, (M, C, KW, wcode) = packed
     if C != x.C:
         raise RuntimeError("conv1d_bf16: weight expects %d input channels, x has %d" % (C, x.C))
@@ -1132,17 +1157,24 @@
         extra = (mask_bits, y.bits_ptr if bits_out else None)
     if f.scaled:
         extra += (_sptr(x.gscale, 1) if out_ncl else None,)
+    symbol, yg = f.conv, None
+    if gate is not None:
+        symbol, yg = f.conv_gated, nlc_like(x, M)
+        gate_ptr = _nlc_ptr(gate, x, M, "gate")
+        as_bits = gate.has_bits and USE_SIGN_BITS
+        extra += (None, gate.bits_ptr, yg.ptr) if as_bits else (gate_ptr, None, yg.ptr)
     with _timed(family, 2.0 * x.B * x.L * M * C * KW):
-        rc = getattr(lib(), f.conv)(x.ptr, wp.data_ptr(), _ptr(bias, name="bias"), _nlc_ptr(skip1, x, M, "skip1"),
+        rc = getattr(lib(), symbol)(x.ptr, wp.data_ptr(), _ptr(bias, name="bias"), _nlc_ptr(skip1, x, M, "skip1"),
                                     _nlc_ptr(skip2, x, M, "skip2"), mask_ptr, _nlc_ptr(post, x, M, "post"),
                                     y.ptr if y is not None else None, y2.ptr if y2 is not None else None, _ptr(y_ncl),
                                     x.B, C, M, x.L, KW, int(bool(relu)), *extra, _stream())
     if bits_out:
         y.has_bits = True
-    _check(rc, f.conv)
+    _check(rc, symbol)
     if out_ncl:
         return y_ncl
-    return (y, y2) if post is not None else y
+    outs = (y,) + ((y2,) if post is not None else ()) + ((yg,) if gate is not None else ())
+    return outs if len(outs) > 1 else y
 
 
 def _wgrad_out(who, dy, x, KW, w_layout, dw_out, accumulate):
@@ -1163,6 +1195,8 @@
 def _wgrad_launch(f, symbol, family, head, ws_ptr, nseg, dy, x, KW, w_layout, dw, dbias, accumulate, defer):
     B, C, M, L = x.B, x.C, dy.C, x.L
     scale = dy.gscale if f.scaled else None
+    if defer is None and accumulate:
+        _adds_into(dw, dbias)
     with _timed(family, 2.0 * nseg * B * L * M * C * KW):
         rc = getattr(lib(), symbol)(*head, ws_ptr, B, C, M, L, KW, w_layout,
                                     WGRAD_DEFER if defer is not None else int(bool(accumulate)),
diff --git a/acoustic_locating_vq-vae_amd/src/acoustic_locating_vq_vae/_ops.py b/acoustic_locating_vq-vae_amd/src/acoustic_locating_vq_vae/_ops.py
--- a/acoustic_locating_vq-vae_amd/src/acoustic_locating_vq_vae/_ops.py
+++ b/acoustic_locating_vq-vae_amd/src/acoustic_locating_vq_vae/_ops.py
@@ -46,15 +46,74 @@
 _SINKS_ACTIVE = 0
 
 
+class GradTouch:
+
+    def __init__(self, grad, spans):
+        self.grad = grad
+        self.span = {grad.data_ptr() + 4 * lo: (lo, hi) for lo, hi in spans}
+        self.stored, self.promote = set(), set()
+        self.pending, self.written = set(), set()
+
+    def _fill(self, ranges):
+        run = None
+        for lo, hi in sorted(ranges) + [(None, None)]:
+            if run is not None and lo == run[1]:
+                run[1] = hi
+                continue
+            if run is not None and run[0] is not None:
+                N.fill_(self.grad[run[0]:run[1]], 0.0)
+            run = [lo, hi]
+
+    def begin(self):
+        self.stored |= self.promote
+        self.promote, self.written = set(), set()
+        keep = sorted(self.span[p] for p in self.stored)
+        fills, at = [], 0
+        for lo, hi in keep + [(self.grad.numel(), None)]:
+            if lo > at:
+                fills.append((at, lo))
+            at = hi
+        self._fill(fills)
+        self.pending = set(self.stored)
+
+    def stores(self, ptr):
+        if ptr in self.pending:
+            self.pending.discard(ptr)
+            self.written.add(ptr)
+            return True
+        if ptr in self.span and ptr not in self.written:
+            self.written.add(ptr)
+            self.promote.add(ptr)
+        return False
+
+    def adds(self, ptr):
+        if ptr in self.pending:
+            self.pending.discard(ptr)
+            self.stored.discard(ptr)
+            self._fill([self.span[ptr]])
+        self.written.add(ptr)
+
+    def finish(self, lo=0, hi=None):
+        late = [p for p in self.pending if lo <= self.span[p][0] and (hi is None or self.span[p][0] < hi)]
+        self._fill([self.span[p] for p in late])
+        self.pending.difference_update(late)
+        self.stored.difference_update(late)
+
+
 class use_grad_sinks:
+
+    def __init__(self, touch=None):
+        self.touch = touch
 
     def __enter__(self):
         global _SINKS_ACTIVE
         _SINKS_ACTIVE += 1
+        self.prev, N._FIRST_TOUCH = N._FIRST_TOUCH, self.touch
 
     def __exit__(self, *exc):
         global _SINKS_ACTIVE
         _SINKS_ACTIVE -= 1
+        N._FIRST_TOUCH = self.prev
 
 
 _DEFERRED = None
@@ -95,7 +154,10 @@
 def _sink(t):
     if t is None or not _SINKS_ACTIVE or not len(_GRAD_SINKS) or not t.requires_grad:
         return None
-    return _GRAD_SINKS.get(t.data_ptr())
+    hit = _GRAD_SINKS.get(t.data_ptr())
+    if hit is None and N._FIRST_TOUCH is not None and t.grad is not None:
+        N._FIRST_TOUCH.adds(t.grad.data_ptr())
+    return hit
 
 
 class PackPool:
@@ -318,6 +380,7 @@
     fwd = grad = None
     can_defer = False
     wgrad_multi = None
+    gates = False
 
     def enter(self, x, grad=False):
         return dense(x)
@@ -348,6 +411,7 @@
 
     def __init__(self, name, fwd, grad):
         self.name, self.fwd, self.grad = name, N._FORMATS[fwd], N._FORMATS[grad]
+        self.gates = self.grad.conv_gated is not None
 
     def _w(self, w, layout):
         wcode = self.fwd.wcode
@@ -383,8 +447,9 @@
     def leave(self, a):
         return N.nlc_to_ncl(a)
 
-    def conv(self, x, w, layout=OIK, bias=None, skip1=None, skip2=None, mask=None, post=None, relu=False, out_f32=False):
-        return N.conv1d_bf16(x, self._w(w, layout), bias, skip1, skip2, mask, post, relu, out_ncl=out_f32)
+    def conv(self, x, w, layout=OIK, bias=None, skip1=None, skip2=None, mask=None, post=None, relu=False, out_f32=False,
+             gate=None):
+        return N.conv1d_bf16(x, self._w(w, layout), bias, skip1, skip2, mask, post, relu, out_ncl=out_f32, gate=gate)
 
     def wgrad(self, dy, x, kw, layout, want_bias=False, dw_out=None, dbias_out=None, accumulate=False, defer=None):
         return N.conv1d_wgrad_bf16(dy, x, kw, layout, want_bias=want_bias, dw_out=dw_out, dbias_out=dbias_out,
@@ -494,8 +559,9 @@
     return xi, ts, us, out
 
 
-def _encoder_backward(eng, d_out, xi, ts, us, wc, bc, w1, w2, R, need_dx):
-    dh = eng.relu_mask(d_out, ts[R])
+def _encoder_backward(eng, d_out, xi, ts, us, wc, bc, w1, w2, R, need_dx, dh=None):
+    if dh is None:
+        dh = eng.relu_mask(d_out, ts[R])
     dh0, dw1, dw2 = _stack_backward(eng, dh, ts, us, w1, w2, R, outer=d_out)
     dwc, dbc = _wgrad(eng, dh0, xi, 3, OIK, wc, bc)
     dx = eng.conv(dh0, wc, IOK, out_f32=True) if need_dx else None
@@ -539,9 +605,9 @@
         eng, (wc, bc, w1, w2, wp, bp), acts = _load(ctx)
         xi, out, ts, us = acts[0], acts[1], acts[2:R + 3], acts[R + 3:]
         dzi = eng.enter(dz, grad=True)
-        d_out = eng.conv(dzi, wp, IOK)
+        d_out, dh = eng.conv(dzi, wp, IOK, gate=ts[R]) if eng.gates else (eng.conv(dzi, wp, IOK), None)
         dwp, dbp = _wgrad(eng, dzi, out, 3, OIK, wp, bp)
-        dx, dwc, dbc, dw1, dw2 = _encoder_backward(eng, d_out, xi, ts, us, wc, bc, w1, w2, R, ctx.needs_input_grad[0])
+        dx, dwc, dbc, dw1, dw2 = _encoder_backward(eng, d_out, xi, ts, us, wc, bc, w1, w2, R, ctx.needs_input_grad[0], dh=dh)
         return dx, dwc, dbc, dw1, dw2, dwp, dbp, None
 
 
diff --git a/acoustic_locating_vq-vae_amd/src/acoustic_locating_vq_vae/train_step.py b/acoustic_locating_vq-vae_amd/src/acoustic_locating_vq_vae/train_step.py
--- a/acoustic_locating_vq-vae_amd/src/acoustic_locating_vq_vae/train_step.py
+++ b/acoustic_locating_vq-vae_amd/src/acoustic_locating_vq_vae/train_step.py
@@ -54,9 +54,15 @@
             p.data = self.flat[off:off + n].view(p.shape)
             p.grad = self.grad[off:off + n].view(p.shape)
         self.skip_slot = self.grad[0:1]
-
-    def zero_grad(self):
-        if self.grad.is_cuda:
+        self.touch = None
+        if self.grad.is_cuda and os.environ.get("ALVQ_FIRST_TOUCH", "1") != "0":
+            ends = self.offsets[1:] + [self.extra_span[0] if extra else total]
+            self.touch = _ops.GradTouch(self.grad, list(zip(self.offsets, ends)))
+
+    def zero_grad(self, first_touch=False):
+        if self.grad.is_cuda and first_touch and self.touch is not None:
+            self.touch.begin()
+        elif self.grad.is_cuda:
             N.fill_(self.grad, 0.0)
         else:
             self.grad.zero_()
@@ -356,10 +362,11 @@
             N.arena_reset(self.buffers.flat.device)
         for sink in self._ema_sinks.values():
             sink.written = False
-        with _ops.use_pack_pool(self.pack_pool), _ops.use_grad_sinks(), _ops.deferred_reduce() as reductions, \
+        touch = self.buffers.touch
+        with _ops.use_pack_pool(self.pack_pool), _ops.use_grad_sinks(touch), _ops.deferred_reduce() as reductions, \
                 _ops.use_ema_sinks(self._ema_sinks):
             x, target = self.preprocess(raw, wiener)
-            self.buffers.zero_grad()
+            self.buffers.zero_grad(first_touch=True)
             if self._one is None or self._one.device != x.device:
                 self._one = torch.ones((), device=x.device)
             if self._buckets is None:
@@ -372,6 +379,8 @@
                 self._cut = tap[0] if tap else None
             if reductions:
                 N.wgrad_reduce_batch(reductions)
+            if touch is not None:
+                touch.finish(*(self._buckets[0] if self._cut is not None else ()))
             if self._cut is None:
                 self._post_verdict()
         return loss.detach(), recon_error.detach(), perplexity.detach()
@@ -385,10 +394,13 @@
             return
         z, leaf = self._cut
         self._cut = None
-        with _ops.use_pack_pool(self.pack_pool, refresh=False), _ops.use_grad_sinks(), _ops.deferred_reduce() as reductions:
+        touch = self.buffers.touch
+        with _ops.use_pack_pool(self.pack_pool, refresh=False), _ops.use_grad_sinks(touch), _ops.deferred_reduce() as reductions:
             z.backward(leaf.grad)
             if reductions:
                 N.wgrad_reduce_batch(reductions)
+            if touch is not None:
+                touch.finish()
             self._post_verdict()
 
     def _sync_early(self):
diff --git a/include/alvq.h b/include/alvq.h
--- a/include/alvq.h
+++ b/include/alvq.h
@@ -202,6 +202,10 @@
                      const void* mask, const void* post, void* y, void* y2, float* y_ncl,
                      int B, int C, int M, int L, int KW, int relu, const void* mask_bits, void* relu_bits_out,
                      void* stream);
+int alvq_conv1d_bf16_gated(const void* x, const void* wp, const float* bias, const void* skip1, const void* skip2,
+                           const void* mask, const void* post, void* y, void* y2, float* y_ncl,
+                           int B, int C, int M, int L, int KW, int relu, const void* mask_bits, void* relu_bits_out,
+                           const void* gate, const void* gate_bits, void* y_gated, void* stream);
 
 int64_t alvq_conv1d_wgrad_bf16_workspace_bytes(int B, int C, int M, int L, int KW);
 int alvq_conv1d_wgrad_bf16(const void* dy, const void* x, float* dw, float* dbias, void* workspace,
@@ -212,6 +216,7 @@
 int alvq_conv1d_wgrad_bf16_splits(int B, int C, int M, int L, int KW, int nseg, int with_bias);
 
 #define ALVQ_WGRAD_DEFER 2
+#define ALVQ_REDUCE_FIRST_TOUCH 2
 int64_t alvq_conv1d_wgrad_bf16_bias_offset(int B, int C, int M, int L, int KW);
 typedef struct alvq_reduce_desc {
   const float* partial;
@@ -261,6 +266,11 @@
                     const void* mask, const void* post, void* y, void* y2, float* y_ncl,
                     int B, int C, int M, int L, int KW, int relu, const void* mask_bits, void* relu_bits_out,
                     const float* out_scale, void* stream);
+int alvq_conv1d_f16_gated(const void* x, const void* wp, const float* bias, const void* skip1, const void* skip2,
+                          const void* mask, const void* post, void* y, void* y2, float* y_ncl,
+                          int B, int C, int M, int L, int KW, int relu, const void* mask_bits, void* relu_bits_out,
+                          const float* out_scale, const void* gate, const void* gate_bits, void* y_gated,
+                          void* stream);
 int alvq_conv1d_wgrad_f16(const void* dy, const void* x, float* dw, float* dbias, void* workspace,
                           int B, int C, int M, int L, int KW, int w_layout, int accumulate,
                           const float* inv_scale, void* stream);
```

Result: no change. 7675, median of 6 (+0.2%).
